# oleg-savchenko/jax_nbody_emulator_with_dj

Hardware: AMD Instinct MI355X
Metric: voxels/sec (disp+vel) on 512^3 box, ndiv=4 (higher is better)
Workload: dtype f32-equivalent: f16x3 split MFMA (3 f16 MFMAs per product, f32 accumulate)

## Files before the change

### include/nbe.h

```cpp
#ifndef NBE_H
#define NBE_H

#include <stddef.h>
#include <stdint.h>

#ifdef __cplusplus
extern "C" {
#endif

typedef struct nbe_ctx nbe_ctx;

typedef void (*nbe_progress_cb)(int done, int total, void* user);

typedef struct nbe_layer_desc {
    const char* block;
    const char* layer;
    int cout, cin, k;
    const float* weight;
    const float* bias;
    const float* style_weight;
    const float* style_bias;
    const float* dweight;
} nbe_layer_desc;

enum { NBE_F32 = 0, NBE_F16 = 1 };

const char* nbe_last_error(void);
int nbe_version(void);

int nbe_create(int device_id, nbe_ctx** out);
int nbe_destroy(nbe_ctx* ctx);
int nbe_set_stream(nbe_ctx* ctx, void* hip_stream);
int nbe_use_own_stream(nbe_ctx* ctx);
int nbe_synchronize(nbe_ctx* ctx);

int nbe_set_arch(nbe_ctx* ctx, int in_chan, int out_chan, int mid_chan, float eps, int compute_vel);

enum { NBE_PREC_F32 = 0, NBE_PREC_F16X3 = 1, NBE_PREC_F16 = 2 };
int nbe_set_precision(nbe_ctx* ctx, int precision);

enum { NBE_ERANGE = 2 };
int nbe_check_finite(nbe_ctx* ctx);
int nbe_set_input_range(nbe_ctx* ctx, float absmax);

enum { NBE_Q_GAUGE_ACTIVE = 0,
       NBE_Q_SLAB = 1,
       NBE_Q_PERIODIC_YX = 2,
       NBE_Q_PERIODIC_Z = 3,
       NBE_Q_RANGE_SHIFT = 4,
       NBE_Q_WORKSPACE_BYTES = 5,
       NBE_Q_HOST_PIPE = 6,
       NBE_Q_GRAPH_REPLAYS = 7,
       NBE_Q_PLAN_TILES = 8,
       NBE_Q_PLAN_SHORT_GB = 9 };
int nbe_query(nbe_ctx* ctx, int what, double* out);

int nbe_load_style_weights(nbe_ctx* ctx, const nbe_layer_desc* layers, int nlayers);
int nbe_load_premod_weights(nbe_ctx* ctx, const nbe_layer_desc* layers, int nlayers);

int nbe_set_cosmology(nbe_ctx* ctx, float Om, float Dz);

int nbe_forward(nbe_ctx* ctx, const void* x, int D, int H, int W, float Dz, float vel_fac,
                void* disp, void* vel);

int nbe_process_box(nbe_ctx* ctx, const void* box, const int64_t size[3], const int ndiv[3], const int pad[6],
                    float Dz, float vel_fac, void* disp, void* vel, int out_dtype,
                    nbe_progress_cb cb, void* user);

void* nbe_host_alloc(size_t bytes);
int nbe_host_free(void* p);
int nbe_host_trim(void);

int nbe_process_region(nbe_ctx* ctx, const void* box, const int64_t box_size[3], const int64_t origin[3],
                       const int64_t region[3], const int ndiv[3], const int* order, int norder,
                       float Dz, float vel_fac, void* disp, void* vel, int out_dtype,
                       const int64_t out_size[3], const int64_t out_origin[3]);

int64_t nbe_brick_halo_bytes(nbe_ctx* ctx, const int64_t brick_size[3], int which);
int nbe_brick_plan(nbe_ctx* ctx, const int64_t brick_size[3]);
int nbe_brick_encode(nbe_ctx* ctx, const void* haloed_brick, const int64_t brick_size[3], float Dz, float vel_fac,
                     void* send_lo, void* send_hi, void* skip_send_lo, void* skip_send_hi);
int nbe_brick_interior(nbe_ctx* ctx);
int nbe_brick_exchange(nbe_ctx* ctx, const void* recv_lo, const void* recv_hi, void* send2_lo, void* send2_hi);
int nbe_brick_finish(nbe_ctx* ctx, const void* recv2_lo, const void* recv2_hi, const void* skip_recv_lo, const void* skip_recv_hi,
                     void* skip_ready_event , float Dz, float vel_fac, void* disp, void* vel, int out_dtype);

int nbe_plan_tiles(const int64_t region[3], const int ndiv[3], int max_tile, int out_ndiv[3]);
int nbe_set_max_tile(nbe_ctx* ctx, int max_tile);
int nbe_plan_tiles_ctx(nbe_ctx* ctx, const int64_t region[3], const int ndiv[3], int periodic_box, int out_ndiv[3]);
int nbe_set_slab(nbe_ctx* ctx, int slab);
int nbe_set_periodic(nbe_ctx* ctx, int on);

double nbe_growth_factor(double z, double Om);
double nbe_vel_norm(double z, double Om);


int nbe_paint_mesh(const void* disp, int disp_dtype, const int64_t n[3], const double boxsize[3], const int64_t res[3],
                   int worder, int count_atomics, void* mesh, void* stats, void* stream);
int nbe_mesh_to_delta(const void* mesh, const int64_t res[3], int64_t nparticles, void* delta, void* stream);

#define NBE_PAINT_MAX_CHANNELS 4
#define NBE_FIELD_DENSITY 0
#define NBE_FIELD_MEAN 1
int nbe_quantity_range(const void* quantity, int dtype, int nchan, int64_t count, void* range, void* stream);
int nbe_paint_fields(const void* disp, int disp_dtype, const void* quantity, int quantity_dtype, int nchan,
                     const int exponents[], const void* shift, int shift_dtype, int shift_axis, double shift_scale,
                     const int64_t n[3], const double boxsize[3], const int64_t res[3], int worder, void* mesh,
                     void* qmesh, void* stats, void* stream);
int nbe_mesh_to_field(const void* mesh, const void* qmesh, int nchan, const int exponents[], const int64_t res[3],
                      int64_t nparticles, int mode, double fill, void* field, void* stats, void* stream);
int nbe_deconvolve_mas(void* field, const int64_t res[3], int worder, void* stream);
int nbe_power_spectrum(const void* a, const void* b, int64_t n, void* binmax, void* sums, void* stream);
#define NBE_PK_ANISO_MAX_N 2048
#define NBE_PK_MAX_MU 64
int nbe_power_multipoles(const void* a, const void* b, int64_t n, int los, void* binmax, void* sums, void* stream);
int nbe_power_wedges(const void* a, const void* b, int64_t n, int los, int nmu, int max_bins, void* binmax, void* sums,
                     void* stream);

#define NBE_MF_MAX_N 2048
#define NBE_MF_MAX_THRESHOLDS 1024
#define NBE_MOMENTS_WORDS 2050
int nbe_field_moments(const void* field, int64_t n, void* moments, void* stream);
int nbe_minkowski_counts(const void* field, int64_t n, const void* thresholds, int nthresholds, const void* moments,
                         void* counts, void* stream);

#define NBE_BK_MIN_N 4
#define NBE_BK_MAX_N 2048
#define NBE_BK_MAX_SHELLS 258
#define NBE_BK_MAX_EDGES 512
#define NBE_BK_PARTIALS 2048
int nbe_shell_filter(const void* spectrum, int64_t n, const void* shells, int nshells, void* filtered, void* binmax,
                     void* sums, void* stream);
int nbe_triple_sums(const void* f1, const void* f2, const void* f3, int nfields, int64_t n, void* partials, void* out,
                    void* stream);
int nbe_triangle_counts(const void* modes1, int64_t count1, const void* modes2, int64_t count2, const void* edges,
                        int nedges, void* hist, void* stream);

#define NBE_MOMENTS4_WORDS 6148
#define NBE_PDF_MAX_BINS 4096
#define NBE_ONEPOINT_MAX_VOXELS (1LL << 40)
int nbe_field_moments4(const void* field, int64_t count, void* moments, void* stream);
int nbe_field_histogram(const void* field, int64_t count, double lo, double hi, const void* edges, int nbins,
                        void* counts, void* stream);

#define NBE_LPT_MIN_N 2
#define NBE_LPT_MAX_N 2048
int nbe_zeldovich_spectrum(const void* spectrum, int64_t n, double boxsize, double scale, void* psi_spectrum,
                           void* stream);
int nbe_divergence_spectrum(const void* spectra, int64_t n, double boxsize, void* out, void* stream);
int nbe_spectrum_resize(const void* src, int64_t n_in, void* dst, int64_t n_out, int sphere, void* stream);
int nbe_spectrum_inject(const void* src, int64_t n_in, void* dst, int64_t n_out, const void* k_table,
                        const void* pk_table, int ntable, double tail_slope, double tail_intercept, double boxsize,
                        uint64_t seed, void* stream);
int nbe_gaussian_filter(void* spectrum, int64_t n, double sigma_over_L, void* stream);
int nbe_block_average(const void* src, int64_t n_in, void* dst, int64_t n_out, void* stream);
int nbe_trilinear_upsample(const void* src, int64_t n_in, void* dst, int64_t n_out, void* stream);


int nbe_test_layer(nbe_ctx* ctx, int kind, int crop, int flags, const float* x, const float* dx, int cin,
                   int D, int H, int W, const float* w, const float* dw, const float* bias, int cout,
                   const float* res, const float* dres, float* y, float* dy);
int nbe_test_layer_gauged(nbe_ctx* ctx, int flags, const float* x, const float* dx, int cin, int D, int H, int W,
                          const float* w, const float* beta, const float* bias, int cout, float* y, float* dy);
int nbe_test_layer_gauged_res(nbe_ctx* ctx, int flags, const float* x, const float* dx, int cin, int D, int H, int W,
                              const float* w, const float* beta, const float* bias, int cout, const float* res,
                              const float* dres, float* y, float* dy);
enum { NBE_PATH_SKIP_FUSED = 1,
       NBE_PATH_TWO_SOURCE = 2,
       NBE_PATH_WINO_0 = 4,
       NBE_PATH_WINO_1 = 8,
       NBE_PATH_NARROW = 16,
       NBE_PATH_UP8 = 32,
       NBE_PATH_SKIP_NODX = 64,
       NBE_PATH_TWO_SOURCE_SKIP = 128   };
int nbe_test_block(nbe_ctx* ctx, const char* block, int pad, int two_source, const float* x, const float* dx, int D, int H, int W,
                   const float* x2, const float* dx2, float* y, float* dy, float* h, float* dh, float* gauges, int* paths);
int nbe_test_modulate(nbe_ctx* ctx, const float* weight, const float* style_weight, const float* style_bias,
                      int cout, int cin, int k, float s0, float s1, float eps, int first_layer,
                      float* w_n, float* dw_tot);

int nbe_probe_begin(nbe_ctx* ctx, const int64_t origin[3], int nout);
int nbe_probe_slots(nbe_ctx* ctx);
int nbe_probe_layout(nbe_ctx* ctx, int slot, char* name, int name_cap, int dims[3], int64_t* word_offset);
int nbe_probe_read(nbe_ctx* ctx, void* words, int64_t nwords);
int nbe_probe_end(nbe_ctx* ctx);

int nbe_profile_enable(nbe_ctx* ctx, int on);
int nbe_profile_reset(nbe_ctx* ctx);
int nbe_profile_count(nbe_ctx* ctx);
int nbe_profile_entry(nbe_ctx* ctx, int i, char* name, int name_cap, double* ms, int64_t* launches, double* flops);
int64_t nbe_workspace_bytes(nbe_ctx* ctx);
int nbe_debug_phase_cycles(nbe_ctx* ctx, double* out16);

#ifdef __cplusplus
}
#endif
#endif
```

### jax_nbody_emulator_with_dj_amd/csrc/nbe_engine.cpp

```cpp
#include "nbe_engine_internal.h"

static thread_local std::string g_err;

int fail(const char* fmt, ...) {
    char buf[1024];
    va_list ap;
    va_start(ap, fmt);
    vsnprintf(buf, sizeof buf, fmt, ap);
    va_end(ap);
    g_err = buf;
    return 1;
}

namespace nbe { int api_fail(const char* msg) { g_err = msg; return 1; } }

bool is_device_ptr(const void* p) {
    hipPointerAttribute_t at;
    if (hipPointerGetAttributes(&at, p) != hipSuccess) { (void)hipGetLastError(); return false; }
    return at.type == hipMemoryTypeDevice;
}

int require_ready(nbe_ctx* c) {
    if (!c->have_weights) return fail("No parameters loaded. Call nbe_load_style_weights / nbe_load_premod_weights first.");
    if (c->style && !c->modulated) return fail("style weights are loaded but nbe_set_cosmology(Om, Dz) has not been called");
// ... 232 lines not shown
    }
    char *dd = (char*)disp, *vd = (char*)vel;
    if (!out_dev) {
        const int64_t need = out_bytes * 2;
        if (need > c->box_out_bytes) { (void)hipFree(c->box_out); HIPCHK(hipMalloc((void**)&c->box_out, need)); c->box_out_bytes = need; }
        dd = c->box_out; vd = c->box_out + out_bytes;
    }
    if (prepare_range(c, xd, (int64_t)c->in_chan * D * H * W, Dz)) return 1;
    if (c->probe.on) {
        const int oe[3] = {OD, OH, OW};
        c->probe.tile = true;
        for (int d = 0; d < 3; ++d) {
            c->probe.o[d] = c->probe.p[d];
            if (c->probe.p[d] < 0 || c->probe.p[d] + c->probe.nout > oe[d]) return fail("branch probe: the block does not fit the output of this input");
        }
    }
    if (run_subbox(c, xd, D, H, W, 0, 0, 0, D, H, W, Dz, vel_fac, dd, vd, NBE_F32, OD, OH, OW, 0, 0, 0)) return 1;
    HIPCHK(hipGetLastError());
    if (!out_dev) {
        HIPCHK(hipMemcpyAsync(disp, dd, out_bytes, hipMemcpyDeviceToHost, c->stream));
        if (c->vel) HIPCHK(hipMemcpyAsync(vel, vd, out_bytes, hipMemcpyDeviceToHost, c->stream));
    }
    if (!out_dev || !xin_dev) {
        HIPCHK(hipStreamSynchronize(c->stream));
        return check_range(c);
    }
    return 0;
}

int nbe_set_precision(nbe_ctx* c, int prec) {
    if (!c) return fail("null context");
    if (prec != PREC_F32 && prec != PREC_F16X3 && prec != PREC_F16) return fail("precision must be NBE_PREC_F32 (0), NBE_PREC_F16X3 (1) or NBE_PREC_F16 (2)");
    if (c->have_weights && prec != c->prec)
        return fail("nbe_set_precision must be called before the weights are loaded (they are packed per precision)");
    c->prec = prec;
    return 0;
}

int nbe_set_periodic(nbe_ctx* c, int on) {
    if (!c) return fail("null context");
    c->pyx_allowed = on != 0;
    return 0;
}

int nbe_set_slab(nbe_ctx* c, int slab) {
    if (!c) return fail("null context");
    if (slab > 0 && (slab & 1)) return fail("slab must be even");
    c->slab_forced = slab < 0 ? -1 : slab;
    return 0;
}

int nbe_set_max_tile(nbe_ctx* c, int max_tile) {
    if (!c) return fail("null context");
    if (max_tile < 0) return fail("max_tile must be >= 0 (0 = keep the caller's sub-box grid)");
    c->max_tile = max_tile;
    return 0;
}

int nbe_check_finite(nbe_ctx* c) {
    if (!c) return fail("null context");
    HIPCHK(hipSetDevice(c->device));
    return check_range(c);
}

int nbe_set_input_range(nbe_ctx* c, float absmax) {
    if (!c) return fail("null context");
    c->preset_absmax = (absmax >= 0.f || std::isnan(absmax)) ? absmax : -1.f;
    return 0;
}

int nbe_query(nbe_ctx* c, int what, double* out) {
    if (!c || !out) return fail("null argument");
    switch (what) {
    case NBE_Q_GAUGE_ACTIVE: *out = c->gauge_active ? 1 : 0; break;
    case NBE_Q_SLAB: *out = c->slab; break;
    case NBE_Q_PERIODIC_YX: *out = c->pyx ? 1 : 0; break;
    case NBE_Q_PERIODIC_Z: *out = c->pz ? 1 : 0; break;
    case NBE_Q_RANGE_SHIFT: *out = std::log2((double)c->act_scale); break;
    case NBE_Q_WORKSPACE_BYTES: *out = (double)c->ws_bytes; break;
    case NBE_Q_HOST_PIPE: *out = c->last_piped ? 1 : 0; break;
    case NBE_Q_GRAPH_REPLAYS: *out = (double)c->graph_replays; break;
    case NBE_Q_PLAN_TILES: *out = (double)c->plan_tiles; break;
    case NBE_Q_PLAN_SHORT_GB: *out = c->plan_short_gb; break;
    default: return fail("nbe_query: unknown item %d", what);
    }
    return 0;
}

int64_t nbe_workspace_bytes(nbe_ctx* c) { return c ? c->ws_bytes : 0; }

}
```

### jax_nbody_emulator_with_dj_amd/csrc/nbe_engine_box.cpp

```cpp
#include "nbe_engine_internal.h"

#include <sched.h>

static int host_threads() {
    static const int n = [] {
        if (const char* e = getenv("NBE_HOST_THREADS")) return std::max(1, atoi(e));
        unsigned hw = std::thread::hardware_concurrency();
        cpu_set_t set;
        if (sched_getaffinity(0, sizeof set, &set) == 0) hw = std::min<unsigned>(hw ? hw : 64, (unsigned)CPU_COUNT(&set));
        return (int)std::max(1u, std::min(hw ? hw : 4u, 16u));
    }();
    return n;
}
template <typename F>
static void parallel_for(int nt, F&& fn) {
    std::vector<std::thread> th;
    for (int i = 1; i < nt; ++i) th.emplace_back([&fn, i, nt] { fn(i, nt); });
    fn(0, nt);
    for (auto& t : th) t.join();
}
static void parallel_memcpy(void* dst, const void* src, size_t bytes) {
    const int nt = bytes < (size_t(8) << 20) ? 1 : host_threads();
    parallel_for(nt, [&](int i, int n) {
        const size_t per = ((bytes + n - 1) / n + 4095) & ~size_t(4095), b = std::min(bytes, per * i), e = std::min(bytes, b + per);
// ... 69 lines not shown
    }
    return 0;
}

int pipe_input(nbe_ctx* c, const Tensor& tin, int t0, int t1, int look, float scale) {
    auto& P = c->pipe;
    if (P.gz < t0) P.gz = t0;
    if (t1 > P.gz) {
        if (pipe_upload(c, P.gz, t1)) return 1;
        HIPCHK(hipEventRecord(c->ev_up, c->up_stream));
        HIPCHK(hipStreamWaitEvent(c->stream, c->ev_up, 0));
        const Tensor v = zview(tin, P.gz, t1 - P.gz);
        const int h = tin.pad ? 1 : 48;
        launch_gather(c->box_in, P.C, P.S0, P.S1, P.S2, P.o0 + P.gz, P.slabwise ? P.o1 : -h, P.slabwise ? P.o2 : -h, v.p, scale,
                      c->prec, c->stream);
        P.gz = t1;
    }
    return look > 0 ? pipe_upload(c, t1, t1 + look) : 0;
}

int pipe_output(nbe_ctx* c, int z, int n, int a1, int a2, int e1, int e2) {
    auto& P = c->pipe;
    if (e1 < 0) e1 = P.O1;
    if (e2 < 0) e2 = P.O2;
    HIPCHK(hipEventRecord(c->ev_down, c->stream));
    HIPCHK(hipStreamWaitEvent(c->down_stream, c->ev_down, 0));
    const int64_t plane = (int64_t)P.O1 * P.O2 * P.esz;
    const bool whole = a1 == 0 && a2 == 0 && e1 == P.O1 && e2 == P.O2;
    for (int f = 0; f < (P.hvel ? 2 : 1); ++f) {
        char* h = f ? P.hvel : P.hdisp;
        char* d = f ? P.dvel : P.ddisp;
        for (int ch = 0; ch < c->out_chan; ++ch) {
            if (whole) {
                const int64_t off = ((int64_t)ch * P.O0 + z) * plane;
                HIPCHK(hipMemcpyAsync(h + off, d + off, (size_t)n * plane, hipMemcpyDeviceToHost, c->down_stream));
            } else {
                hipMemcpy3DParms mp;
                memset(&mp, 0, sizeof mp);
                mp.srcPtr = make_hipPitchedPtr(d, (size_t)P.O2 * P.esz, (size_t)P.O2 * P.esz, (size_t)P.O1);
                mp.dstPtr = make_hipPitchedPtr(h, (size_t)P.O2 * P.esz, (size_t)P.O2 * P.esz, (size_t)P.O1);
                mp.srcPos = make_hipPos((size_t)a2 * P.esz, (size_t)a1, (size_t)ch * P.O0 + z);
                mp.dstPos = mp.srcPos;
                mp.extent = make_hipExtent((size_t)e2 * P.esz, (size_t)e1, (size_t)n);
                mp.kind = hipMemcpyDeviceToHost;
                HIPCHK(hipMemcpy3DAsync(&mp, c->down_stream));
            }
        }
    }
    return 0;
}

static int64_t workspace_need(nbe_ctx* c, int D, int H, int W, int slab, bool pyx, bool pz) {
    const int keep_slab = c->slab; const bool keep_pyx = c->pyx, keep_pz = c->pz;
    c->slab = slab; c->pyx = pyx; c->pz = pz;
    c->dry = true;
    c->arena.reset();
    Tensor tin = talloc(c, c->in_chan, D, H, W), y;
    tin.pad = c->pyx ? 1 : 0;
    HeadOut ho{};
    const int rc = c->slab > 0 ? network_stream(c, tin, ho, c->slab) : network(c, tin, &y);
    c->dry = false;
    c->slab = keep_slab; c->pyx = keep_pyx; c->pz = keep_pz;
    return rc ? -1 : c->arena.high;
}

int ensure_workspace(nbe_ctx* c, int D, int H, int W) {
    const int64_t need = workspace_need(c, D, H, W, c->slab, c->pyx, c->pz);
    if (need < 0) return 1;
    if (need > c->ws_bytes) {
        c->sst.valid = false;
        if (c->ws) { HIPCHK(hipStreamSynchronize(c->stream)); HIPCHK(hipFree(c->ws)); c->ws = nullptr; c->ws_bytes = 0; }
        HIPCHK(hipMalloc((void**)&c->ws, need));
        HIPCHK(hipMemsetAsync(c->ws, 0, need, c->stream));
        c->ws_bytes = need;
    }
    return 0;
}

int run_subbox(nbe_ctx* c, const float* box, int Db, int Hb, int Wb, int o0, int o1, int o2,
                      int D, int H, int W, float Dz, float vel_fac, void* disp, void* velo, int out_dtype,
                      int OD, int OH, int OW, int a0, int a1, int a2) {
    c->sst.valid = false;
    c->arena.reset();
    Tensor tin = talloc(c, c->in_chan, D, H, W), y;
    tin.pad = c->pyx ? 1 : 0;
    if (tin.pad) set_org(tin, 0, 48, 48);
    if (!c->pipe.active && !c->pipe.slabwise)
        launch_gather(box, c->in_chan, Db, Hb, Wb, o0, o1, o2, tin.p, Dz / 6.0f * c->act_scale, c->prec, c->stream);
    const HeadOut ho{disp, velo, out_dtype, OD, OH, OW, a0, a1, a2, Dz, vel_fac};
    if (c->slab > 0) return network_stream(c, tin, ho, c->slab);
    if (network(c, tin, &y)) return 1;
    run_head(c, y, tin, ho, 0);
    return 0;
}

void drop_graphs(nbe_ctx* c) {
    for (auto& kv : c->graphs) {
        if (kv.second.exec) (void)hipGraphExecDestroy(kv.second.exec);
        if (kv.second.graph) (void)hipGraphDestroy(kv.second.graph);
    }
    c->graphs.clear();
}

static int run_tile(nbe_ctx* c, const float* box, int Db, int Hb, int Wb, int o0, int o1, int o2,
                    int D, int H, int W, float Dz, float vel_fac, void* disp, void* velo, int out_dtype,
                    int OD, int OH, int OW, int a0, int a1, int a2) {
    const bool off = getenv("NBE_GRAPH") && atoi(getenv("NBE_GRAPH")) == 0;
    if (off || c->prof || c->prog_cb || c->pipe.active || c->pipe.slabwise || c->dry || c->probe.on)
        return run_subbox(c, box, Db, Hb, Wb, o0, o1, o2, D, H, W, Dz, vel_fac, disp, velo, out_dtype, OD, OH, OW, a0, a1, a2);
    nbe_ctx::GraphKey k;
    memset(&k, 0, sizeof k);
    k.box = box; k.disp = disp; k.velo = velo; k.ws = c->ws;
    const int geo[18] = {Db, Hb, Wb, o0, o1, o2, D, H, W, out_dtype, OD, OH, OW, a0, a1, a2, c->slab, c->prec};
    memcpy(k.geo, geo, sizeof geo);
    k.f[0] = Dz; k.f[1] = vel_fac; k.f[2] = c->act_scale;
    k.epoch = c->epoch; k.flags = (c->pyx ? 1 : 0) | (c->pz ? 2 : 0) | (c->gauge_active ? 4 : 0) | (c->fuse ? 8 : 0) | (wino_env_off() ? 16 : 0);
    nbe_ctx::GraphVal& g = c->graphs[k];
    g.used = ++c->graph_clock;
    if (!g.exec && g.seen++ == 0) {
        if (c->graphs.size() > 16) {
            auto lru = c->graphs.begin();
            for (auto it = c->graphs.begin(); it != c->graphs.end(); ++it) if (it->second.used < lru->second.used) lru = it;
            if (lru->second.exec) (void)hipGraphExecDestroy(lru->second.exec);
            if (lru->second.graph) (void)hipGraphDestroy(lru->second.graph);
            c->graphs.erase(lru);
        }
        return run_subbox(c, box, Db, Hb, Wb, o0, o1, o2, D, H, W, Dz, vel_fac, disp, velo, out_dtype, OD, OH, OW, a0, a1, a2);
    }
    if (!c->ev_g0) { HIPCHK(hipEventCreateWithFlags(&c->ev_g0, hipEventDisableTiming)); HIPCHK(hipEventCreateWithFlags(&c->ev_g1, hipEventDisableTiming)); }
    hipStream_t user = c->stream;
    if (!g.exec) {
        c->stream = c->own_stream;
        hipError_t e = hipStreamBeginCapture(c->own_stream, hipStreamCaptureModeThreadLocal);
        int rc = 0;
        if (e == hipSuccess) {
            rc = run_subbox(c, box, Db, Hb, Wb, o0, o1, o2, D, H, W, Dz, vel_fac, disp, velo, out_dtype, OD, OH, OW, a0, a1, a2);
            e = hipStreamEndCapture(c->own_stream, &g.graph);
            if (e == hipSuccess && !rc) e = hipGraphInstantiate(&g.exec, g.graph, nullptr, nullptr, 0);
        }
        c->stream = user;
        if (rc || e != hipSuccess || !g.exec) {
            (void)hipGetLastError();
            if (g.graph) { (void)hipGraphDestroy(g.graph); g.graph = nullptr; }
            g.exec = nullptr; g.seen = -1000000;
            return run_subbox(c, box, Db, Hb, Wb, o0, o1, o2, D, H, W, Dz, vel_fac, disp, velo, out_dtype, OD, OH, OW, a0, a1, a2);
        }
    }
    if (user != c->own_stream) { HIPCHK(hipEventRecord(c->ev_g0, user)); HIPCHK(hipStreamWaitEvent(c->own_stream, c->ev_g0, 0)); }
    HIPCHK(hipGraphLaunch(g.exec, c->own_stream));
    if (user != c->own_stream) { HIPCHK(hipEventRecord(c->ev_g1, c->own_stream)); HIPCHK(hipStreamWaitEvent(user, c->ev_g1, 0)); }
    ++c->graph_replays;
    return 0;
}

extern "C" {

int nbe_plan_tiles(const int64_t region[3], const int ndiv[3], int max_tile, int out_ndiv[3]) {
    if (!region || !ndiv || !out_ndiv) return fail("null argument");
    bool ok = max_tile > 0;
    for (int a = 0; a < 3 && ok; ++a) {
        if (ndiv[a] < 1 || region[a] < 1) return fail("sizes and ndiv must be positive");
        const int64_t crop = region[a] / ndiv[a];
        if (crop % 8 != 0 || crop * ndiv[a] != region[a]) ok = false;
    }
    for (int a = 0; a < 3; ++a) {
        out_ndiv[a] = ndiv[a];
        if (!ok) continue;
        const int64_t crop = region[a] / ndiv[a];
        int best = 1;
        for (int m = 1; m <= ndiv[a]; ++m)
            if (ndiv[a] % m == 0 && crop * m <= max_tile) best = m;
        out_ndiv[a] = ndiv[a] / best;
    }
    return 0;
}

}

int choose_slab(nbe_ctx* c, int D, int H, int W, int64_t budget, int64_t* need_out, bool pyx, bool pz) {
    const int forced = c->slab_forced;
    int result = -1;
    const int cand[4] = {0, 128, 64, 32};
    for (int i = 0; i < 4 && result < 0; ++i) {
        int S = cand[i];
        if (pyx && S == 0) { if (forced == 0) break; continue; }
        if (forced == 0 && S != 0) break;
        if (forced > 0) { if (i > (pyx ? 1 : 0)) break; S = forced & ~1; }
        if (!pyx && S > 0 && D - 8 <= S) continue;
        const int64_t need = workspace_need(c, D, H, W, S, pyx, pyx && pz);
        if (need >= 0 && need <= budget) { result = S; if (need_out) *need_out = need; }
    }
    return result;
}

static bool choose_schedule(nbe_ctx* c, int e0, int e1, int e2, bool spans_yx, bool whole_z, int64_t budget, bool fallback32) {
    const int D = e0 + 96;
    if (spans_yx && !check_dims_pyx(D, e1 + 2, e2 + 2)) {
        const int sl = choose_slab(c, D, e1 + 2, e2 + 2, budget, nullptr, true, whole_z);
        if (sl > 0) { c->slab = sl; c->pyx = true; c->pz = whole_z; return true; }
// ... 391 lines not shown
```

### jax_nbody_emulator_with_dj_amd/csrc/nbe_engine_internal.h

```cpp
#pragma once

#include "../../include/nbe.h"
#include "nbe_kernels.h"

#include <cmath>
#include <cstdarg>
#include <cstdio>
#include <cstdlib>
#include <cstring>
#include <algorithm>
#include <atomic>
#include <chrono>
#include <condition_variable>
#include <deque>
#include <functional>
#include <map>
#include <memory>
#include <mutex>
#include <string>
#include <thread>
#include <vector>

#pragma GCC visibility push(hidden)

using namespace nbe;

int fail(const char* fmt, ...);

#define HIPCHK(expr)                                                                        \
    do {                                                                                    \
        hipError_t e_ = (expr);                                                             \
        if (e_ != hipSuccess) return fail("%s failed: %s (%s:%d)", #expr, hipGetErrorString(e_), __FILE__, __LINE__); \
    } while (0)

static inline int roundup(int v, int m) { return (v + m - 1) / m * m; }

struct Arena {
    struct Blk { int64_t off, size; bool used; };
    std::vector<Blk> blks;
    int64_t high = 0;
    void reset() { blks.clear(); blks.push_back({0, INT64_MAX / 2, false}); high = 0; }
    int64_t alloc(int64_t bytes) {
        bytes = (bytes + 255) & ~int64_t(255);
        for (size_t i = 0; i < blks.size(); ++i) {
            if (!blks[i].used && blks[i].size >= bytes) {
                Blk rest{blks[i].off + bytes, blks[i].size - bytes, false};
                blks[i].size = bytes; blks[i].used = true;
                if (rest.size > 0) blks.insert(blks.begin() + i + 1, rest);
                if (blks[i].off + bytes > high) high = blks[i].off + bytes;
                return blks[i].off;
            }
        }
        return -1;
    }
    void release(int64_t off) {
        for (size_t i = 0; i < blks.size(); ++i) {
            if (blks[i].off == off && blks[i].used) {
                blks[i].used = false;
                if (i + 1 < blks.size() && !blks[i + 1].used) { blks[i].size += blks[i + 1].size; blks.erase(blks.begin() + i + 1); }
                if (i > 0 && !blks[i - 1].used) { blks[i - 1].size += blks[i].size; blks.erase(blks.begin() + i); }
                return;
            }
        }
    }
};

struct Layer {
    std::string block, layer;
    int cout = 0, cin = 0, k = 0, kind = 0;
    bool first = false;
    float *weight = nullptr, *sw = nullptr, *sb = nullptr;
    float *wn = nullptr, *dwn = nullptr;
    PackedW pw;
    PackedW pwn;
    float* bias0 = nullptr;
    float *alpha = nullptr, *beta = nullptr;
    const float* gout = nullptr;
    const float* a_in = nullptr;
    bool g6 = false;
    const Layer* fskip = nullptr;
    const float* b_sub = nullptr;
    float* bias_f = nullptr;
    float* dwn_f = nullptr;
};

struct Tensor { Planes p; int64_t off = -1; int pad = 0; int org[3] = {0, 0, 0}; };

struct ProfEntry { std::string name; double ms = 0; int64_t launches = 0; double flops = 0; };

struct Progress {
    struct Item { hipEvent_t ev; int done, total; };
    nbe_progress_cb cb; void* user; int device;
    std::thread th; std::mutex mu; std::condition_variable cv; std::deque<Item> q; bool stop = false;
    Progress(nbe_progress_cb cb_, void* user_, int dev) : cb(cb_), user(user_), device(dev) {
        th = std::thread([this] {
            (void)hipSetDevice(device);
            for (;;) {
                Item it;
                {
                    std::unique_lock<std::mutex> lk(mu);
                    cv.wait(lk, [this] { return stop || !q.empty(); });
                    if (q.empty()) return;
                    it = q.front(); q.pop_front();
                }
                (void)hipEventSynchronize(it.ev);
                (void)hipEventDestroy(it.ev);
                cb(it.done, it.total, user);
            }
        });
    }
    void post(hipStream_t s, int done, int total) {
        hipEvent_t ev;
        if (hipEventCreateWithFlags(&ev, hipEventDisableTiming) != hipSuccess) return;
        (void)hipEventRecord(ev, s);
        { std::lock_guard<std::mutex> lk(mu); q.push_back({ev, done, total}); }
        cv.notify_one();
    }
    ~Progress() {
        { std::lock_guard<std::mutex> lk(mu); stop = true; }
        cv.notify_one();
        if (th.joinable()) th.join();
    }
};

struct nbe_ctx {
    int device = 0;
    hipStream_t own_stream = nullptr, stream = nullptr;
    int in_chan = 3, out_chan = 3, mid = 64;
    float eps = 1e-8f;
    bool vel = true;
    bool have_weights = false, style = false, modulated = false;
    float mod_Om = NAN, mod_Dz = NAN;
    std::map<std::string, Layer> layers;
    Arena arena;
    char* ws = nullptr;
    int64_t ws_bytes = 0;
    bool dry = false;
    int slab = 0;
    int slab_forced = -1;
    bool pyx = false;
    bool pyx_allowed = true;
    bool pz = false;
    bool zx = false;
    int phase = 0;
    struct BrickIO { void *send_lo = nullptr, *send_hi = nullptr; const void *recv_lo = nullptr, *recv_hi = nullptr;
                     void *skip_send_lo = nullptr, *skip_send_hi = nullptr; const void *skip_recv_lo = nullptr, *skip_recv_hi = nullptr;
                     hipEvent_t skip_ready = nullptr; } bio;
    struct StreamState {
        bool valid = false;
        int stage = 0;
        Tensor skip0, td, tin, t, h, y1, cat1, t2;
        int D = 0, H = 0, W = 0, S = 0;
        std::vector<Arena::Blk> blks; int64_t high = 0;
        float Dz = 0.f, vel_fac = 0.f, act_scale = 1.f; const char* ws = nullptr;
    } sst;
    nbe_progress_cb prog_cb = nullptr; void* prog_user = nullptr; int prog_k = 0, prog_n = 1;
    Progress* prog = nullptr;
    int max_tile = 512;
    int prec = PREC_F32;
    bool gauge = false;
    bool gauge_active = false;
    bool fuse = false;
    bool novel_fuse = false;
    int64_t bp_size[3] = {0, 0, 0}; int bp_slab = 0; int64_t bp_need = 0;
    int plan_tiles = 0;
    double plan_short_gb = 0.0;
    int64_t plan_logged = 0;
    int* gauge_flag = nullptr;
    int* wino_flag = nullptr; bool wino_ok = false;
    float act_scale = 1.f;
    float bias_scale = 1.f;
    bool bias_dirty = true;
    float bias_max = 0.f;
    float preset_absmax = -1.f;
    bool input_finite = true;
    bool range_pending = false;
    unsigned* flags = nullptr;
    float* box_in = nullptr; int64_t box_in_bytes = 0;
    char* box_out = nullptr; int64_t box_out_bytes = 0;
    struct HostPipe {
        bool active = false, out_async = false;
        bool tiles = false;
        bool slabwise = false;
        int o1 = 0, o2 = 0;
        const float* hbox = nullptr;
        bool in_pinned = false;
        int C = 0, S0 = 0, S1 = 0, S2 = 0, o0 = 0;
        std::vector<char> up;
        int gz = 0;
        char *hdisp = nullptr, *hvel = nullptr;
        char *ddisp = nullptr, *dvel = nullptr;
        int esz = 4, O0 = 0, O1 = 0, O2 = 0;
        int nstage = 0;
    } pipe;
    bool last_piped = false;
    hipStream_t up_stream = nullptr, down_stream = nullptr;
    static constexpr int NSTAGE = 3;
    char* stage_buf[NSTAGE] = {nullptr, nullptr, nullptr}; int64_t stage_bytes = 0;
    hipEvent_t stage_free[NSTAGE] = {nullptr, nullptr, nullptr};
    hipEvent_t ev_up = nullptr, ev_down = nullptr;
    struct GraphKey {
        const void *box, *disp, *velo, *ws;
        int geo[18]; float f[3]; int epoch, flags;
        bool operator<(const GraphKey& o) const { return memcmp(this, &o, sizeof *this) < 0; }
    };
    struct GraphVal { hipGraphExec_t exec = nullptr; hipGraph_t graph = nullptr; int seen = 0; uint64_t used = 0; };
    std::map<GraphKey, GraphVal> graphs;
    uint64_t graph_clock = 0, graph_replays = 0;
    int epoch = 0;
    hipEvent_t ev_g0 = nullptr, ev_g1 = nullptr;
    struct Probe {
        bool on = false, tile = false;
        int p[3] = {0, 0, 0}, nout = 0;
        int o[3] = {0, 0, 0};
        struct Slot { std::string name; int C, n, nw, level; int64_t off; };
        std::vector<Slot> slots;
        unsigned* bits = nullptr; int64_t words = 0;
        unsigned* count = nullptr;
    } probe;
    int* paths = nullptr;
    bool prof = false;
    std::vector<ProfEntry> prof_entries;
    struct Pending { int entry; hipEvent_t a, b; };
    std::vector<Pending> pending;
    std::vector<hipEvent_t> ev_pool;
};

struct HeadOut { void* disp; void* velo; int out_dtype; int OD, OH, OW, a0, a1, a2; float Dz, vel_fac; };

static constexpr int PIPE_EDGE = 32;

static constexpr int BRICK_H1 = 6, BRICK_H2 = 10;
static constexpr int BRICK_H0 = 4;

bool is_device_ptr(const void* p);
int require_ready(nbe_ctx* c);
int prepare_range(nbe_ctx* c, const float* dev_src, int64_t n, float Dz, const float* host_src = nullptr);
int check_range(nbe_ctx* c);

int planes_for(int C, int prec);
Tensor talloc(nbe_ctx* c, int C, int D, int H, int W);
Tensor tallocp(nbe_ctx* c, int C, int D, int Hi, int Wi, int pad);
void fill_halo(nbe_ctx* c, const Tensor& t);
void tfree(nbe_ctx* c, Tensor& t);
Tensor zview(const Tensor& t, int z0, int nz);
void set_org(Tensor& t, int z, int y, int x);
bool wino_f16_layer(int prec, bool vel, int cin_pad);
bool wino_env_off();
bool up8_launch(const nbe_ctx* c, const Layer& L, bool has_dx);
int run_conv(nbe_ctx* c, const Layer& L, const ConvLaunch& cl_in, bool has_dx);
const Layer* find_layer(nbe_ctx* c, const char* block, const char* layer);
bool block_fused(const nbe_ctx* c, const Layer* L1, int nres);
bool two_source_width(const nbe_ctx* c);
Tensor alloc_hidden(nbe_ctx* c, int cmid, int nz, const Tensor& x, bool fused);
int resblock_part(nbe_ctx* c, const char* name, const Tensor& x, const Tensor& h, const Tensor& s,
                  int js, int ns, int jh, int nh, bool has_dx, bool final_act, const int* zr, const Tensor* x2 = nullptr);
int resblock(nbe_ctx* c, const char* name, const Tensor& x, bool has_dx, bool final_act, int cout, int cmid, Tensor* out,
             Tensor* hidden_out = nullptr);
int down_conv(nbe_ctx* c, const Layer& L, const Tensor& x, Tensor& o, bool probe);
int downblock(nbe_ctx* c, const char* name, const Tensor& x, Tensor* out);
int upblock(nbe_ctx* c, const char* name, const Tensor& x, const Tensor& cat, int xcrop = 0, int g0 = -1);
void crop_into(nbe_ctx* c, const Tensor& src, int crop, const Tensor& dst, int cz = -1);
int check_dims(int D, int H, int W);
int check_dims_pyx(int D, int H, int W);
void run_head(nbe_ctx* c, const Tensor& y, const Tensor& xin, const HeadOut& h, int zoff);
int network(nbe_ctx* c, const Tensor& tin, Tensor* yout);
int network_stream(nbe_ctx* c, const Tensor& tin, const HeadOut& ho, int S);

PackedW layer_geometry(int prec, int kind, int cout, int cin);
bool packs_narrow(int prec, bool vel, const Layer& L);
bool packs_wino(int prec, bool vel, const Layer& L);
bool packs_wino_skip(int prec, bool vel, bool style, const Layer& L);
bool packs_stem(int prec, const Layer& L);
int alloc_wino(PackedW& pw);
int alloc_stem(PackedW& pw);
int wino_flag_round_trip(nbe_ctx* c, const std::function<void()>& packs);
void release_layer(Layer& L);
void free_layers(nbe_ctx* c);
int pack_wino(nbe_ctx* c);

unsigned host_absmax_bits(const float* x, int64_t n);
int pipe_input(nbe_ctx* c, const Tensor& tin, int t0, int t1, int look, float scale);
int pipe_output(nbe_ctx* c, int z, int n, int a1 = 0, int a2 = 0, int e1 = -1, int e2 = -1);
int ensure_workspace(nbe_ctx* c, int D, int H, int W);
int run_subbox(nbe_ctx* c, const float* box, int Db, int Hb, int Wb, int o0, int o1, int o2,
               int D, int H, int W, float Dz, float vel_fac, void* disp, void* velo, int out_dtype,
               int OD, int OH, int OW, int a0, int a1, int a2);
void drop_graphs(nbe_ctx* c);
int64_t plan_budget(nbe_ctx* c, int64_t reserve);
int choose_slab(nbe_ctx* c, int D, int H, int W, int64_t budget, int64_t* need_out, bool pyx = false, bool pz = false);

void brick_send(nbe_ctx* c, const Tensor& t, int in, int n, void* lo, void* hi);
void brick_recv(nbe_ctx* c, const Tensor& like, const void* lo, const void* hi, int n, const Tensor& dst, int wrap);
int brick_interior(nbe_ctx* c, nbe_ctx::StreamState& st);
int brick_edges(nbe_ctx* c, nbe_ctx::StreamState& st);
int brick_level2(nbe_ctx* c, nbe_ctx::StreamState& st, Tensor* t_out);

void probe_act(nbe_ctx* c, const Layer& L, const Planes& out, int g0, const int org[3], int ez, int ey, int ex, bool periodic,
               const int* zr = nullptr);
int prof_entry(nbe_ctx* c, const std::string& name);
hipEvent_t get_event(nbe_ctx* c);
void prof_collect(nbe_ctx* c);

#pragma GCC visibility pop
```

### jax_nbody_emulator_with_dj_amd/csrc/nbe_engine_net.cpp

```cpp
#include "nbe_engine_internal.h"

int planes_for(int C, int prec) { return roundup(C, 16) / (prec == PREC_F16 ? 8 : 4); }

static Planes ws_planes(nbe_ctx* c, int G, int D, int H, int W, int64_t* off_out) {
    Planes p;
    p.G = G; p.D = D; p.H = H; p.W = W;
    p.pstride = (p.vox() + 63) & ~int64_t(63);
    const int64_t one = (int64_t)G * p.pstride * 16;
    const int64_t slack = ((int64_t)2 * H * W + 2 * W + 1024) * 16;
    const int64_t off = c->arena.alloc(one * (c->vel ? 2 : 1) + slack);
    *off_out = off;
    if (!c->dry) {
        p.x = (float*)(c->ws + off);
        p.dx = c->vel ? (float*)(c->ws + off + one) : nullptr;
    }
    return p;
}

Tensor talloc(nbe_ctx* c, int C, int D, int H, int W) {
    Tensor t;
    t.p = ws_planes(c, planes_for(C, c->prec), D, H, W, &t.off);
    const int gw = c->prec == PREC_F16 ? (C + 7) / 8 : c->prec == PREC_F16X3 ? 2 * ((C + 7) / 8) : (C + 3) / 4;
    if (!c->dry && t.off >= 0 && gw < t.p.G) {
        const size_t off = (size_t)gw * t.p.pstride * 4, bytes = (size_t)(t.p.G - gw) * t.p.pstride * 16;
        launch_zero(t.p.x + off, (int64_t)bytes, c->stream);
        if (t.p.dx) launch_zero(t.p.dx + off, (int64_t)bytes, c->stream);
    }
    return t;
}
Tensor tallocp(nbe_ctx* c, int C, int D, int Hi, int Wi, int pad) {
    Tensor t = talloc(c, C, D, Hi + 2 * pad, Wi + 2 * pad);
    t.pad = pad;
    return t;
}
static Planes inner(const Tensor& t) {
    Planes p = t.p;
    const int64_t sh = (int64_t)t.pad * (t.p.W + 1) * 4;
    if (p.x) p.x += sh;
    if (p.dx) p.dx += sh;
    return p;
}
void fill_halo(nbe_ctx* c, const Tensor& t) {
    if (t.pad > 0 && !c->dry) launch_fill_yx(t.p, t.pad, c->vel, c->stream);
}
void tfree(nbe_ctx* c, Tensor& t) { if (t.off >= 0) c->arena.release(t.off); t.off = -1; }
Tensor zview(const Tensor& t, int z0, int nz) {
    Tensor v = t;
    v.off = -1;
    const int64_t sh = (int64_t)z0 * t.p.H * t.p.W * 4;
    if (v.p.x) v.p.x += sh;
    if (v.p.dx) v.p.dx += sh;
    v.p.D = nz;
    v.org[0] += z0;
    return v;
}
static void org_conv(const Tensor& x, int nconv, int out[3]) {
    const int p = x.pad ? nconv : 0;
    out[0] = x.org[0]; out[1] = x.org[1] - p; out[2] = x.org[2] - p;
}
void set_org(Tensor& t, int z, int y, int x) { t.org[0] = z; t.org[1] = y; t.org[2] = x; }

static std::string conv_name(const PackedW& pw, bool vel, bool has_dx, bool g6 = false, bool up8 = false) {
    if (up8) return vel ? "up_h3<8 parities,vel,dx>" : "up_h3<8 parities,novel>";
    const char* m = pw.mode == MODE_FLAT3 ? "FLAT3" : pw.mode == MODE_FLAT1 ? "FLAT1" : "DOWN";
    if (pw.stem && !(vel && has_dx) && pw.mode == MODE_FLAT3) return vel ? "stem_h3<FLAT3,vel,nodx>" : "stem_h3<FLAT3,novel>";
    char b[96];
    if (g6 && prec_is_half(pw.prec)) snprintf(b, sizeof b, "%s<%s,vel,dx>", pw.prec == PREC_F16 ? "conv_h1g" : (pw.cout_t == 16 ? "conv_h3n" : "conv_h3g"), m);
    else if (g6) snprintf(b, sizeof b, "conv_mfma_g<%s,vel,dx,ni%d>", m, pw.ni);
    else if (prec_is_half(pw.prec))
        snprintf(b, sizeof b, "%s<%s,%s,%s>", pw.prec == PREC_F16 ? "conv_h1" : "conv_h3", m, vel ? "vel" : "novel", (vel && has_dx) ? "dx" : "nodx");
    else
        snprintf(b, sizeof b, "conv_mfma<%s,%s,%s,ni%d>", m, vel ? "vel" : "novel", (vel && has_dx) ? "dx" : "nodx", pw.ni);
    return b;
}

bool wino_f16_layer(int prec, bool vel, int cin_pad) { return prec == PREC_F16 && vel && cin_pad % 32 == 0 && cin_pad / 32 <= 8; }
bool wino_env_off() { return getenv("NBE_WINO") && atoi(getenv("NBE_WINO")) == 0; }
bool up8_launch(const nbe_ctx* c, const Layer& L, bool has_dx) { return prec_is_half(c->prec) && (!c->vel || has_dx) && L.pw.cin_pad <= 64; }

int run_conv(nbe_ctx* c, const Layer& L, const ConvLaunch& cl_in, bool has_dx) {
    if (c->dry) return 0;
    ConvLaunch cl = cl_in;
    const bool g6 = c->gauge_active && L.g6 && has_dx;
    const bool nov = !c->vel && c->prec == PREC_F16X3 && L.kind == 0 && L.pw.ww && c->wino_ok;
    if (c->gauge_active) { cl.gout = L.gout; cl.beta = g6 ? L.beta : nullptr; }
    if (cl.skw) {
        if (!((g6 || nov) && c->fuse && L.fskip)) return fail("internal error: fused skip requested for %s/%s", L.block.c_str(), L.layer.c_str());
        cl.bias = L.bias_f;
    }
    const PackedW& pw = (g6 && L.kind == 0 && L.pwn.w) ? L.pwn : L.pw;
    cl.wino = (g6 || nov) && c->wino_ok && &pw == &L.pw && pw.ww && (!cl.skw || cl.skw->ww) && (c->prec == PREC_F16 || !(cl.flags & F_RES)) &&
              (cl.Dv & 1) == 0 && cl.in_off == 0 && cl.osz == 1 && !wino_env_off();
    if (c->paths)
        *c->paths |= (cl.skw ? NBE_PATH_SKIP_FUSED : 0) | (cl.skw && (cl.flags & F_SKIP_NODX) ? NBE_PATH_SKIP_NODX : 0) |
                     (cl.csplit_ch ? NBE_PATH_TWO_SOURCE : 0) | (cl.skw && cl.sk_split_ch ? NBE_PATH_TWO_SOURCE_SKIP : 0) |
                     (cl.wino ? (L.layer == "conv_1" ? NBE_PATH_WINO_1 : NBE_PATH_WINO_0) : 0) |
                     (&pw == &L.pwn ? NBE_PATH_NARROW : 0) | (cl.set < 0 ? NBE_PATH_UP8 : 0);
    int pe = -1; hipEvent_t ea = nullptr, eb = nullptr;
    if (c->prof) {
        std::string pn = cl.wino ? std::string(c->prec == PREC_F16 ? "conv_h1w<FLAT3,vel,dx>" : c->vel ? "conv_h3w<FLAT3,vel,dx>" : "conv_h3w<FLAT3,novel>")
                                 : conv_name(pw, c->vel, has_dx, g6, cl.set < 0);
        static const bool per_layer = getenv("NBE_PROF_LAYERS") && atoi(getenv("NBE_PROF_LAYERS")) == 1;
        if (per_layer) pn += " " + L.block + "/" + L.layer;
        pe = prof_entry(c, pn);
        ea = get_event(c); eb = get_event(c);
        (void)hipEventRecord(ea, c->stream);
    }
    if (launch_conv(pw, cl, c->vel, has_dx, c->stream))
        return fail("internal error: no kernel for layer %s/%s (mode %d, gauged %d, input tangent %d, crop offset %ld, output stride %d)",
                    L.block.c_str(), L.layer.c_str(), L.pw.mode, (int)g6, (int)has_dx, (long)cl.in_off, cl.osz);
    if (c->prof) {
        (void)hipEventRecord(eb, c->stream);
        c->pending.push_back({pe, ea, eb});
        const double nout = (double)cl.Dv * cl.Hv * cl.Wv * (cl.set < 0 ? 8.0 : 1.0);
        const int taps = L.kind == 0 ? 27 : L.kind == 2 ? 8 : 1;
        const double gemms = c->vel ? ((has_dx && !g6) ? 3.0 : 2.0) : 1.0;
        c->prof_entries[pe].flops += 2.0 * nout * L.cout * L.cin * taps * gemms;
        if (cl.skw) c->prof_entries[pe].flops += 2.0 * nout * L.cout * L.fskip->cin * (!c->vel ? 1.0 : (cl.flags & F_SKIP_NODX) ? 2.0 : 3.0);
        c->prof_entries[pe].launches += 1;
        if (c->pending.size() > 4096) prof_collect(c);
    }
    return 0;
}

const Layer* find_layer(nbe_ctx* c, const char* block, const char* layer) {
    auto it = c->layers.find(std::string(block) + "/" + layer);
    return it == c->layers.end() ? nullptr : &it->second;
}


static bool wino_only_fuse(const nbe_ctx* c) { return !c->vel || c->prec == PREC_F16; }
bool block_fused(const nbe_ctx* c, const Layer* L1, int nres) {
    return c->fuse && L1->fskip != nullptr && (!wino_only_fuse(c) || (!wino_env_off() && (nres & 1) == 0));
}

bool two_source_width(const nbe_ctx* c) { return c->mid % (c->prec == PREC_F16 ? 32 : 16) == 0; }

Tensor alloc_hidden(nbe_ctx* c, int cmid, int nz, const Tensor& x, bool fused) {
    const int pad = x.pad, sy = pad ? 0 : 2;
    if (fused && !pad) return talloc(c, cmid, nz, x.p.H, x.p.W);
    return tallocp(c, cmid, nz, x.p.H - 2 * pad - sy, x.p.W - 2 * pad - sy, pad);
}

int resblock_part(nbe_ctx* c, const char* name, const Tensor& x, const Tensor& h, const Tensor& s,
                         int js, int ns, int jh, int nh, bool has_dx, bool final_act, const int* zr, const Tensor* x2) {
    const Layer *Ls = find_layer(c, name, "skip"), *L0 = find_layer(c, name, "conv_0"), *L1 = find_layer(c, name, "conv_1");
    if (!Ls || !L0 || !L1) return fail("missing layers of block %s", name);
    const int H = x.p.H, W = x.p.W, pad = x.pad;
    const bool fused = block_fused(c, L1, ns);
    if (fused && (h.p.H != H || h.p.W != W)) return fail("internal: hidden tensor of fused block %s lacks the input's pitch", name);
    if (x2 && (!fused || x2->p.H != H || x2->p.W != W || x2->pad != pad)) return fail("internal: two-source input of block %s", name);
    const Tensor sv = zview(s, js, ns), hv = zview(h, jh, nh);
    const Tensor xs = zview(x, js, ns + 4);
    const int64_t sk_off = (2L * H + (pad ? pad : 2)) * W + (pad ? pad : 2);
    if (!fused) {
        ConvLaunch cl; cl.in = xs.p; cl.in_off = sk_off;
        cl.Dv = ns; cl.Hv = s.p.H - 2 * pad; cl.Wv = s.p.W - 2 * pad; cl.out = inner(sv); cl.flags = 0;
        if (run_conv(c, *Ls, cl, has_dx)) return 1;
    }
    int og[3];
    {
        ConvLaunch cl; cl.in = zview(x, jh, nh + 2).p; cl.Dv = nh; cl.Hv = H - 2; cl.Wv = W - 2; cl.out = inner(hv); cl.flags = F_ACT;
        if (x2) { cl.in2 = zview(*x2, jh, nh + 2).p; cl.csplit_ch = c->mid; }
        if (run_conv(c, *L0, cl, has_dx)) return 1;
        org_conv(x, 1, og); og[0] += jh;
        const int zh[3] = {zr ? zr[0] : 0, zr ? zr[1] + 2 : 0, zr ? zr[2] : 0};
        probe_act(c, *L0, cl.out, 0, og, cl.Dv, cl.Hv, cl.Wv, pad != 0, zr ? zh : nullptr);
    }
    fill_halo(c, hv);
    {
        ConvLaunch cl; cl.in = zview(h, js, ns + 2).p; cl.Dv = ns; cl.Hv = s.p.H - 2 * pad; cl.Wv = s.p.W - 2 * pad; cl.out = inner(sv);
        if (fused) { cl.sk = xs.p; cl.sk_off = sk_off; cl.skw = L1->pwn.w ? &Ls->pwn : &Ls->pw; cl.flags = (final_act ? F_ACT : 0) | (has_dx ? 0 : F_SKIP_NODX);
                     if (x2) { cl.sk2 = zview(*x2, js, ns + 4).p; cl.sk_split_ch = c->mid; } }
        else { cl.res = inner(sv); cl.flags = F_RES | (final_act ? F_ACT : 0); }
        if (run_conv(c, *L1, cl, true)) return 1;
        org_conv(x, 2, og); og[0] += js;
        if (final_act) probe_act(c, *L1, cl.out, 0, og, cl.Dv, cl.Hv, cl.Wv, pad != 0, zr);
    }
    fill_halo(c, sv);
    return 0;
}

int resblock(nbe_ctx* c, const char* name, const Tensor& x, bool has_dx, bool final_act, int cout, int cmid, Tensor* out,
                    Tensor* hidden_out) {
    const Layer* L1 = find_layer(c, name, "conv_1");
    if (!L1) return fail("missing layers of block %s", name);
    const int D = x.p.D, pad = x.pad;
    const int sy = pad ? 0 : 2;
    Tensor s = tallocp(c, cout, D - 4, x.p.H - 2 * pad - 2 * sy, x.p.W - 2 * pad - 2 * sy, pad);
    Tensor h = alloc_hidden(c, cmid, D - 2, x, block_fused(c, L1, D - 4));
    if (s.off < 0 || h.off < 0) return fail("workspace exhausted in block %s", name);
    if (resblock_part(c, name, x, h, s, 0, D - 4, 0, D - 2, has_dx, final_act, nullptr)) return 1;
    tfree(c, h);
    if (hidden_out) *hidden_out = h;
    int og[3];
    org_conv(x, 2, og);
    set_org(s, og[0], og[1], og[2]);
    *out = s;
    return 0;
}

static void carry_planes(nbe_ctx* c, const Tensor& t, int src, int dst, int n) {
    if (c->dry || n <= 0) return;
    launch_crop(zview(t, src, n).p, 0, zview(t, dst, n).p, 0, c->vel, c->stream, 0);
}

int down_conv(nbe_ctx* c, const Layer& L, const Tensor& x, Tensor& o, bool probe) {
    ConvLaunch cl; cl.in = inner(x); cl.Dv = o.p.D; cl.Hv = o.p.H; cl.Wv = o.p.W; cl.out = o.p; cl.flags = F_ACT;
    if (run_conv(c, L, cl, true)) return 1;
    set_org(o, x.org[0] / 2, x.org[1] / 2, x.org[2] / 2);
    if (probe) probe_act(c, L, cl.out, 0, o.org, cl.Dv, cl.Hv, cl.Wv, x.pad != 0);
    return 0;
}

int downblock(nbe_ctx* c, const char* name, const Tensor& x, Tensor* out) {
    const Layer* L = find_layer(c, name, "conv_0");
    if (!L) return fail("missing layer %s/conv_0", name);
    Tensor o = talloc(c, c->mid, x.p.D / 2, x.p.H / 2, x.p.W / 2);
    if (o.off < 0) return fail("workspace exhausted in %s", name);
    if (down_conv(c, *L, x, o, true)) return 1;
    *out = o;
    return 0;
}

static int mid_planes(const nbe_ctx* c) { return c->mid / (c->prec == PREC_F16 ? 8 : 4); }

int upblock(nbe_ctx* c, const char* name, const Tensor& x, const Tensor& cat, int xcrop, int g0) {
    const Layer* L = find_layer(c, name, "conv_0");
    if (!L) return fail("missing layer %s/conv_0", name);
    xcrop += x.pad;
    const int Hx = x.p.H - 2 * xcrop, Wx = x.p.W - 2 * xcrop;
    if (cat.p.D != 2 * x.p.D || cat.p.H - 2 * cat.pad != 2 * Hx || cat.p.W - 2 * cat.pad != 2 * Wx)
        return fail("internal: concat geometry mismatch in %s", name);
    const bool up8 = up8_launch(c, *L, true);
    const int out_g0 = g0 >= 0 ? g0 : mid_planes(c);
    for (int p = 0; p < (up8 ? 1 : 8); ++p) {
        ConvLaunch cl; cl.in = x.p; cl.in_off = ((int64_t)xcrop * x.p.W + xcrop);
        cl.Dv = x.p.D; cl.Hv = Hx; cl.Wv = Wx; cl.out = inner(cat);
        cl.out_g0 = out_g0; cl.osz = 2; cl.oz = (p >> 2) & 1; cl.oy = (p >> 1) & 1; cl.ox = p & 1;
        cl.flags = F_ACT; cl.set = up8 ? -1 : p;
        if (run_conv(c, *L, cl, true)) return 1;
    }
    const int xc = xcrop - x.pad;
    const int og[3] = {2 * x.org[0], 2 * (x.org[1] + xc), 2 * (x.org[2] + xc)};
    probe_act(c, *L, inner(cat), out_g0, og, 2 * x.p.D, 2 * Hx, 2 * Wx, cat.pad != 0);
    return 0;
}

void crop_into(nbe_ctx* c, const Tensor& src, int crop, const Tensor& dst, int cz) {
    if (c->dry) return;
    Planes s = src.p; s.G = mid_planes(c);
    launch_crop(s, crop, dst.p, 0, c->vel, c->stream, cz);
}

int check_dims(int D, int H, int W) {
    const int v[3] = {D, H, W};
    for (int i = 0; i < 3; ++i)
        if (v[i] < 104 || v[i] % 8 != 0)
            return fail("input spatial size %d unsupported: each of (D,H,W) must be >= 104 and a multiple of 8 "
                        "(all-VALID U-Net with three 2x levels, receptive-field crop 48)", v[i]);
    return 0;
}

void run_head(nbe_ctx* c, const Tensor& y, const Tensor& xin, const HeadOut& h, int zoff) {
    if (c->dry) return;
    const float inv_s = 1.0f / c->act_scale;
    HeadScale hs;
    hs.k_disp = 6.0f * inv_s; hs.k_dy = h.vel_fac * 6.0f * inv_s; hs.k_x0 = h.vel_fac * 6.0f / h.Dz * inv_s;
    hs.bad = c->flags ? (int*)(c->flags + 1) : nullptr;
    launch_head(y.p, xin.p, 48, c->out_chan, hs, c->vel, h.disp, h.velo, h.out_dtype, h.OD, h.OH, h.OW,
                h.a0 + zoff, h.a1, h.a2, c->prec, c->stream, y.pad);
}

static int stream_encode(nbe_ctx* c, const Tensor& tin, const HeadOut& ho, int S, Tensor* skip0_out, Tensor* td_out) {
    const int m = c->mid, pad = tin.pad;
    const int D = tin.p.D, H = tin.p.H, W = tin.p.W;
    const int Hi = H - 2 * pad, Wi = W - 2 * pad;
    const int Y = D - 8;
    const bool zx = pad && c->zx;
    const bool pz = pad && (c->pz || zx);
    const int zlo = pz ? (zx ? 44 : 40) : 0, zhi = pz ? (zx ? Y - 44 : Y - 40) : Y;
    Tensor skip0 = pad ? tallocp(c, m, Y - 80, Hi, Wi, pad) : talloc(c, m, Y - 80, H - 88, W - 88);
    Tensor td = pad ? talloc(c, m, pz ? (D - 96) / 2 : Y / 2, Hi / 2, Wi / 2) : talloc(c, m, Y / 2, (H - 8) / 2, (W - 8) / 2);
    if (skip0.off < 0 || td.off < 0) return fail("workspace exhausted (level 0)");
    const Layer* Ld = find_layer(c, "down_l0", "conv_0");
    if (!Ld) return fail("missing layer down_l0/conv_0");
    const int sy = pad ? 0 : 2;
    const Layer* L00 = find_layer(c, "conv_l00", "conv_1");
    if (!L00) return fail("missing layer conv_l00/conv_1");
    Tensor h0 = alloc_hidden(c, m, S + 6, tin, block_fused(c, L00, S + 4)), a = tallocp(c, m, S + 4, Hi - 2 * sy, Wi - 2 * sy, pad);
    const Layer *L01 = find_layer(c, "conv_l01", "conv_1"), *Lr00 = find_layer(c, "conv_r00", "conv_1"), *Lr01 = find_layer(c, "conv_r01", "conv_1");
    if (!L01 || !Lr00 || !Lr01) return fail("missing conv_1 layers of the level-0 blocks");
    Tensor h1 = alloc_hidden(c, m, S + 2, a, block_fused(c, L01, S));
    Tensor y0r = pz ? Tensor() : tallocp(c, m, S, Hi - 4 * sy, Wi - 4 * sy, pad);
    if (h0.off < 0 || a.off < 0 || h1.off < 0 || (!pz && y0r.off < 0)) return fail("workspace exhausted (level-0 encoder slabs)");
    const int zr00[3] = {zlo, zhi + 4, pz ? D - 96 : 0}, zr01[3] = {zlo, zhi, pz ? D - 96 : 0};
    for (int z = zlo, n = 0; z < zhi; z += n) {
        n = std::min(((c->pipe.active || c->pipe.slabwise) && z == zlo) ? std::min(S, PIPE_EDGE) : S, zhi - z);
        const int n_next = std::min(S, zhi - (z + n));
        const bool first = z == zlo;
        Tensor y0 = pz ? zview(skip0, z - 40, n) : zview(y0r, 0, n);
        if ((c->pipe.active || c->pipe.slabwise) && !c->dry && pipe_input(c, tin, z, z + n + 8, n_next, ho.Dz / 6.0f * c->act_scale)) return 1;
        { int og[3]; org_conv(zview(tin, z, n + 8), 2, og); set_org(a, og[0], og[1], og[2]);
          org_conv(a, 2, og); set_org(y0, og[0], og[1], og[2]); }
        if (first) {
            if (resblock_part(c, "conv_l00", zview(tin, z, n + 8), h0, a, 0, n + 4, 0, n + 6, false, true, zr00)) return 1;
            if (resblock_part(c, "conv_l01", a, h1, y0, 0, n, 0, n + 2, true, true, zr01)) return 1;
        } else {
            if (resblock_part(c, "conv_l00", zview(tin, z, n + 8), h0, a, 4, n, 6, n, false, true, zr00)) return 1;
            if (resblock_part(c, "conv_l01", a, h1, y0, 0, n, 2, n, true, true, zr01)) return 1;
        }
        if (z + n < zhi) {
            carry_planes(c, h0, n, 0, 6);
            carry_planes(c, a, n, 0, 4);
            carry_planes(c, h1, n, 0, 2);
        }
        const int i0 = std::max(0, 40 - z), i1 = std::min(n, Y - 40 - z);
        if (!pz && i1 > i0) crop_into(c, y0, pad ? 0 : 40, zview(skip0, z + i0 - 40, i1 - i0), i0);
        {
            const int d0 = pz ? std::max(z, 44) : z, d1 = pz ? std::min(z + n, Y - 44) : z + n;
            if (d1 > d0) {
                const Tensor tv = zview(td, (d0 - (pz ? 44 : 0)) / 2, (d1 - d0) / 2);
                Tensor yv = zview(y0, d0 - z, d1 - d0);
                ConvLaunch cl; cl.in = inner(yv); cl.Dv = tv.p.D; cl.Hv = tv.p.H; cl.Wv = tv.p.W; cl.out = tv.p; cl.flags = F_ACT;
                if (run_conv(c, *Ld, cl, true)) return 1;
                const int og[3] = {yv.org[0] / 2, yv.org[1] / 2, yv.org[2] / 2};
                const int zd[3] = {22, 22 + (D - 96) / 2, pz ? (D - 96) / 2 : 0};
                probe_act(c, *Ld, cl.out, 0, og, cl.Dv, cl.Hv, cl.Wv, pad != 0, zd);
            }
        }
    }
    tfree(c, h0); tfree(c, a); tfree(c, h1);
    if (!pz) tfree(c, y0r);
    set_org(skip0, 0, pad ? 4 : 0, pad ? 4 : 0);
    set_org(td, pz ? 22 : 0, pad ? 22 : 0, pad ? 22 : 0);
    *skip0_out = skip0; *td_out = td;
    return 0;
}

static int stream_level1(nbe_ctx* c, int pad, bool pz, Tensor td, Tensor* cat1_out, Tensor* t_out) {
    const int m = c->mid;
    Tensor t = td;
    if (pad) {
        t = tallocp(c, m, td.p.D + (pz ? 44 : 0), td.p.H, td.p.W, 1);
        if (t.off < 0) return fail("workspace exhausted (level 1 input)");
        if (!c->dry) launch_wrap_pad(td.p, t.p, 1, c->vel, c->stream, pz ? 22 : 0);
        set_org(t, pz ? td.org[0] - 22 : td.org[0], td.org[1], td.org[2]);
        tfree(c, td);
    }

    Tensor y1, cat1;
    if (resblock(c, "conv_l1", t, true, true, m, m, &y1)) return 1;
    tfree(c, t);
    if (pad) {
        cat1 = tallocp(c, 2 * m, y1.p.D - 32, y1.p.H - 2, y1.p.W - 2, 1);
        if (cat1.off < 0) return fail("workspace exhausted (cat1)");
        crop_into(c, y1, 0, cat1, 16);
        set_org(cat1, y1.org[0], y1.org[1] - 16, y1.org[2] - 16);
        Tensor t2 = talloc(c, m, y1.p.D / 2, (y1.p.H - 2) / 2, (y1.p.W - 2) / 2);
        const Layer* Ld1 = find_layer(c, "down_l1", "conv_0");
        if (t2.off < 0 || !Ld1) return fail("workspace exhausted or missing layer (down_l1)");
        if (down_conv(c, *Ld1, y1, t2, true)) return 1;
        t = talloc(c, m, t2.p.D, t2.p.H + 20, t2.p.W + 20);
        if (t.off < 0) return fail("workspace exhausted (level 2 input)");
        if (!c->dry) launch_wrap_pad(t2.p, t.p, 10, c->vel, c->stream, 0);
        set_org(t, t2.org[0], t2.org[1] - 10, t2.org[2] - 10);
        tfree(c, t2);
    } else {
        cat1 = talloc(c, 2 * m, y1.p.D - 32, y1.p.H - 32, y1.p.W - 32);
        if (cat1.off < 0) return fail("workspace exhausted (cat1)");
        crop_into(c, y1, 16, cat1);
        if (downblock(c, "down_l1", y1, &t)) return 1;
    }
    tfree(c, y1);
    *cat1_out = cat1; *t_out = t;
    return 0;
}

static int lower_levels(nbe_ctx* c, Tensor t, Tensor cat1, Tensor* r_out) {
    const int m = c->mid;
    Tensor y2, cat2, r;
    if (resblock(c, "conv_l2", t, true, true, m, m, &y2)) return 1;
    tfree(c, t);
    cat2 = talloc(c, 2 * m, y2.p.D - 8, y2.p.H - 8, y2.p.W - 8);
    if (cat2.off < 0) return fail("workspace exhausted (cat2)");
    crop_into(c, y2, 4, cat2);
    if (downblock(c, "down_l2", y2, &t)) return 1;
    tfree(c, y2);

    if (resblock(c, "conv_c", t, true, true, m, m, &r)) return 1;
    tfree(c, t);

    if (upblock(c, "up_r2", r, cat2)) return 1;
    tfree(c, r);
    if (resblock(c, "conv_r2", cat2, true, true, m, 2 * m, &r)) return 1;
    tfree(c, cat2);

    if (upblock(c, "up_r1", r, cat1, cat1.pad ? 2 : 0)) return 1;
    fill_halo(c, cat1);
    tfree(c, r);
    if (resblock(c, "conv_r1", cat1, true, true, m, 2 * m, r_out)) return 1;
    tfree(c, cat1);
    return 0;
}

int network(nbe_ctx* c, const Tensor& tin, Tensor* yout) {
    const int m = c->mid;
    Tensor a, y0, t, cat0, cat1, r;
    if (resblock(c, "conv_l00", tin, false, true, m, m, &a)) return 1;
    if (resblock(c, "conv_l01", a, true, true, m, m, &y0)) return 1;
    tfree(c, a);
    cat0 = talloc(c, 2 * m, y0.p.D - 80, y0.p.H - 80, y0.p.W - 80);
    if (cat0.off < 0) return fail("workspace exhausted (cat0)");
    crop_into(c, y0, 40, cat0);
    if (downblock(c, "down_l0", y0, &t)) return 1;
    tfree(c, y0);

    if (stream_level1(c, 0, false, t, &cat1, &t)) return 1;
    if (lower_levels(c, t, cat1, &r)) return 1;

    if (upblock(c, "up_r0", r, cat0)) return 1;
    tfree(c, r);
    if (resblock(c, "conv_r00", cat0, true, true, m, 2 * m, &r)) return 1;
    tfree(c, cat0);

    if (resblock(c, "conv_r01", r, true, false, c->out_chan, m, yout)) return 1;
    tfree(c, r);
    return 0;
}

static int stream_tail(nbe_ctx* c, const Tensor& tin, const HeadOut& ho, int S, Tensor skip0, Tensor cat1, Tensor t) {
    const int m = c->mid, pad = tin.pad;
    const int sy = pad ? 0 : 2;
    const Layer *Lr00 = find_layer(c, "conv_r00", "conv_1"), *Lr01 = find_layer(c, "conv_r01", "conv_1");
    if (!Lr00 || !Lr01) return fail("missing conv_1 layers of the level-0 blocks");
    Tensor r;
    if (lower_levels(c, t, cat1, &r)) return 1;
    if (2 * r.p.D != skip0.p.D || 2 * (r.p.H - 2 * r.pad) != skip0.p.H - 2 * pad || 2 * (r.p.W - 2 * r.pad) != skip0.p.W - 2 * pad)
        return fail("internal: level-0 concat geometry mismatch");

    if (pad && c->zx && !c->dry && c->bio.skip_recv_lo) {
        if (c->bio.skip_ready) HIPCHK(hipStreamWaitEvent(c->stream, c->bio.skip_ready, 0));
        brick_recv(c, skip0, c->bio.skip_recv_lo, c->bio.skip_recv_hi, BRICK_H0, skip0, 0);
    }
    const int Yo = skip0.p.D - 8;
    const int Hs = skip0.p.H - 2 * pad, Ws = skip0.p.W - 2 * pad;
    const bool two = block_fused(c, Lr00, S + 4) && two_source_width(c);
    Tensor cat = tallocp(c, two ? m : 2 * m, S + 8, Hs, Ws, pad), hq = alloc_hidden(c, 2 * m, S + 6, cat, block_fused(c, Lr00, S + 4));
    Tensor q = tallocp(c, m, S + 4, Hs - 2 * sy, Ws - 2 * sy, pad), hy = alloc_hidden(c, m, S + 2, q, block_fused(c, Lr01, S));
    Tensor y = tallocp(c, c->out_chan, S, Hs - 4 * sy, Ws - 4 * sy, pad);
    if (cat.off < 0 || hq.off < 0 || q.off < 0 || hy.off < 0 || y.off < 0) return fail("workspace exhausted (level-0 decoder slabs)");
    for (int z = 0, n = 0; z < Yo; z += n) {
        n = std::min(S, Yo - z);
        if (c->pipe.active && c->pipe.out_async && Yo - z > PIPE_EDGE && Yo - z - n < PIPE_EDGE)
            n = Yo - z - PIPE_EDGE;
        const bool first = z == 0;
        const int c0 = first ? 0 : 8, cn = first ? n + 8 : n;
        set_org(cat, skip0.org[0] + z, skip0.org[1], skip0.org[2]);
        { int og[3]; org_conv(cat, 2, og); set_org(q, og[0], og[1], og[2]); }
        if (!two && !c->dry) launch_crop(zview(skip0, z + c0, cn).p, 0, zview(cat, c0, cn).p, 0, c->vel, c->stream, 0);
        if (upblock(c, "up_r0", zview(r, (z + c0) / 2, cn / 2), zview(cat, c0, cn), 0, two ? 0 : -1)) return 1;
        fill_halo(c, zview(cat, c0, cn));
        const Tensor sk = two ? zview(skip0, z, std::min(S + 8, skip0.p.D - z)) : cat;
        const Tensor* up2 = two ? &cat : nullptr;
        if (first) {
            if (resblock_part(c, "conv_r00", sk, hq, q, 0, n + 4, 0, n + 6, true, true, nullptr, up2)) return 1;
            if (resblock_part(c, "conv_r01", q, hy, y, 0, n, 0, n + 2, true, false, nullptr)) return 1;
        } else {
            if (resblock_part(c, "conv_r00", sk, hq, q, 4, n, 6, n, true, true, nullptr, up2)) return 1;
            if (resblock_part(c, "conv_r01", q, hy, y, 0, n, 2, n, true, false, nullptr)) return 1;
        }
        if (z + n < Yo) {
            carry_planes(c, cat, n, 0, 8);
            carry_planes(c, hq, n, 0, 6);
            carry_planes(c, q, n, 0, 4);
            carry_planes(c, hy, n, 0, 2);
        }
        run_head(c, zview(y, 0, n), zview(tin, z, n + 96), ho, z);
        if (c->pipe.active && c->pipe.out_async && !c->dry && pipe_output(c, z, n)) return 1;
        if (c->prog && !c->dry && z + n < Yo)
            c->prog->post(c->pipe.active && c->pipe.out_async ? c->down_stream : c->stream,
                          c->prog_k * 1000 + (int)(1000L * (z + n) / Yo), c->prog_n * 1000);
    }
    tfree(c, cat); tfree(c, hq); tfree(c, q); tfree(c, hy); tfree(c, y);
    tfree(c, r); tfree(c, skip0);
    return 0;
}

static void stash_arena(nbe_ctx* c) { c->sst.blks = c->arena.blks; c->sst.high = c->arena.high; }

int network_stream(nbe_ctx* c, const Tensor& tin, const HeadOut& ho, int S) {
    auto& st = c->sst;
    const int pad = tin.pad;
    const bool zx = pad && c->zx;
    if (c->phase >= 2) {
        if (!st.valid || st.stage != c->phase - 1) return fail("brick calls out of order (encode, interior, exchange, finish) or the context was used in between");
        c->arena.blks = st.blks; c->arena.high = st.high;
    }
    if (c->phase <= 1) {
        if (stream_encode(c, tin, ho, S, &st.skip0, &st.td)) return 1;
        st.tin = tin; st.S = S;
        if (c->phase == 1) {
            brick_send(c, st.td, 0, BRICK_H1, c->bio.send_lo, c->bio.send_hi);
            brick_send(c, st.skip0, BRICK_H0, BRICK_H0, c->bio.skip_send_lo, c->bio.skip_send_hi);
            st.valid = true; st.stage = 1; stash_arena(c);
            return 0;
        }
    }
    if (!zx) {
        Tensor cat1, t;
        if (stream_level1(c, pad, pad && c->pz, st.td, &cat1, &t)) return 1;
        return stream_tail(c, tin, ho, S, st.skip0, cat1, t);
    }
    if (c->phase == 0 || c->phase == 2) {
        if (brick_interior(c, st)) return 1;
        if (c->phase == 2) { st.stage = 2; stash_arena(c); return 0; }
    }
    if (c->phase == 0 || c->phase == 3) {
        if (brick_edges(c, st)) return 1;
        if (c->phase == 3) { st.stage = 3; stash_arena(c); return 0; }
    }
    Tensor t;
    if (brick_level2(c, st, &t)) return 1;
    st.valid = false;
    return stream_tail(c, st.tin, ho, st.S, st.skip0, st.cat1, t);
}

int check_dims_pyx(int D, int H, int W) {
    if (D < 104 || D % 8 != 0) return fail("input depth %d unsupported: must be >= 104 and a multiple of 8", D);
    const int v[2] = {H - 2, W - 2};
    for (int i = 0; i < 2; ++i)
        if (v[i] < 48 || v[i] % 8 != 0) return fail("periodic extent %d unsupported: must be >= 48 and a multiple of 8", v[i]);
    return 0;
}
// ... 1 lines not shown
```

### jax_nbody_emulator_with_dj_amd/csrc/nbe_kernels.h

```cpp
#pragma once
#include <hip/hip_runtime.h>
#include <stdint.h>

namespace nbe {

struct Planes {
    float* x = nullptr;
    float* dx = nullptr;
    int64_t pstride = 0;
    int G = 0;
    int D = 0, H = 0, W = 0;
    int64_t vox() const { return (int64_t)D * H * W; }
};

enum Precision { PREC_F32 = 0, PREC_F16X3 = 1, PREC_F16 = 2 };
inline constexpr bool prec_is_half(int prec) { return prec == PREC_F16X3 || prec == PREC_F16; }
inline constexpr int prec_parts(int prec) { return prec == PREC_F16X3 ? 2 : 1; }
constexpr float H3_SCALE = 2048.0f, H3_INV = 1.0f / 2048.0f;
constexpr int H3_RANGE_UP = 6;

constexpr int NBE_MAX_GROUPS = 64;

enum ConvMode { MODE_FLAT3 = 0, MODE_FLAT1 = 1, MODE_DOWN = 2 };
enum ConvFlags { F_ACT = 1, F_RES = 2, F_SKIP_NODX = 4 };

constexpr int TILE_VOX = 256;
inline constexpr int mode_taps(int mode) { return mode == MODE_FLAT3 ? 3 : 1; }
inline constexpr int mode_nseg(int mode) { return mode == MODE_FLAT3 ? 9 : (mode == MODE_DOWN ? 8 : 1); }
inline constexpr int mode_ck(int mode) { return mode == MODE_FLAT3 ? 8 : 16; }
inline constexpr int prec_ck(int prec, int mode) { return prec_is_half(prec) ? 16 : mode_ck(mode); }

struct PackedW {
    float* w = nullptr;
    float* dw = nullptr;
    float* bias = nullptr;
    int prec = PREC_F32;
    int mode = 0, ni = 2;
    int cout_t = 64;
    int cin = 0, cout = 0;
    int cin_pad = 0;
    int ctiles = 0;
    int64_t floats = 0;
    int nsets = 1;
    float* ww = nullptr;
    float* stem = nullptr;
};

struct ConvLaunch {
    Planes in;
    int64_t in_off = 0;
    int Dv = 0, Hv = 0, Wv = 0;
    Planes out;
    int out_g0 = 0;
    int osz = 1, oz = 0, oy = 0, ox = 0;
    Planes res;
    int flags = 0;
    int set = 0;
    const float* gout = nullptr;
    const float* beta = nullptr;
    const float* bias = nullptr;
    Planes in2;
    int csplit_ch = 0;
    Planes sk, sk2;
    int sk_split_ch = 0;
    int64_t sk_off = 0;
    const PackedW* skw = nullptr;
    bool wino = false;
};

int launch_conv(const PackedW& pw, const ConvLaunch& L, bool vel, bool has_dx, hipStream_t s);

void launch_modulate(const float* weight, const float* style_weight, const float* style_bias,
                     int cout, int cin, int k3, float s0, float s1, float eps, int first_layer,
                     float* w_n, float* dw_tot , hipStream_t s,
                     const float* a_in = nullptr, float* beta_out = nullptr, const float* b_sub = nullptr);
void launch_style_alpha(const float* style_weight, const float* style_bias, int cin, float s0, float s1,
                        float* alpha, int* flag, hipStream_t s);
void launch_pack(const float* w_oidhw, int cout, int cin, int kind, const PackedW& pw, float* dst, hipStream_t s);

void launch_pack_h3w(const float* w_oidhw, int cout, int cin, int cin_pad, int ctiles, float* dst, int* flag, hipStream_t s,
                     int prec = PREC_F16X3);
void launch_pack_h3w_skip(const float* w_oidhw, int cout, int cin, const PackedW& pw, float* dst, int* flag, hipStream_t s);

void launch_gather(const float* box, int C, int Db, int Hb, int Wb, int a0, int a1, int a2,
                   const Planes& dst, float scale, int prec, hipStream_t s);
void launch_to_planes(const float* src, int C, const Planes& dst, bool tangent, float scale, int prec, hipStream_t s);
void launch_from_planes(const Planes& src, bool tangent, int C, float* dst, int prec, hipStream_t s);
void launch_crop(const Planes& src, int c, const Planes& dst, int g0, bool vel, hipStream_t s, int cz = -1);
struct HeadScale { float k_disp = 6.f, k_dy = 0.f, k_x0 = 0.f; int* bad = nullptr; };
void launch_head(const Planes& y, const Planes& xin, int c0, int C, const HeadScale& hs, bool vel,
                 void* disp, void* velo, int out_dtype, int Db, int Hb, int Wb, int a0, int a1, int a2,
                 int prec, hipStream_t s, int pad = 0);
void launch_absmax(const float* src, int64_t n, unsigned* out_bits, hipStream_t s);
void launch_zero(void* dst, int64_t bytes, hipStream_t s);
void launch_scale(const float* src, float* dst, int n, float f, hipStream_t s, const float* src2 = nullptr);

void launch_fill_yx(const Planes& t, int pad, bool vel, hipStream_t s);
void launch_wrap_pad(const Planes& src, const Planes& dst, int pad, bool vel, hipStream_t s, int padz = 0);

void launch_tag_word(unsigned* dst, unsigned v, const unsigned* expect_at, unsigned* flag, unsigned bit, hipStream_t s);

struct ProbeLaunch {
    const float* x; int64_t pstride; int H, W, g0, prec, C;
    int ext[3], org[3], per[3];
    int zlo, zhi, zper;
    int o[3], n, nw;
    unsigned* bits; unsigned* count;
};
void launch_probe_signs(const ProbeLaunch& a, hipStream_t s);

void h3q_read_stamps(double* out16, hipStream_t s);

}
```

### jax_nbody_emulator_with_dj_amd/csrc/nbe_kernels.hip

```cpp

#include "nbe_kernels_internal.h"
#include <algorithm>
#include <cstdint>
#include <cstdio>
#include <cstdlib>

namespace nbe {

#define LDS_AS NBE_LDS_AS
#define GLB_AS NBE_GLB_AS

extern __shared__ __attribute__((aligned(16))) f32x4 lds_dyn[];

template <int MODE, bool VEL, bool HAS_DX, int NI, bool G6 = false>
__global__ __launch_bounds__(256, 2) void conv_mfma_kernel(ConvKArgs a) {
    constexpr int CK = mode_ck(MODE), GL = CK / 4, TAPS = mode_taps(MODE);
    constexpr int COUT_T = 32 * NI;
    constexpr int XV = (MODE == MODE_FLAT3) ? 320 : 256;
    constexpr int WP = TAPS * GL * COUT_T;
    constexpr int XP = GL * XV;
    constexpr bool DX = VEL && HAS_DX;
    constexpr bool DWT = VEL && !G6;
    static_assert(!G6 || (DX && MODE == MODE_FLAT3), "gauged form: 3x3x3 layers with an input tangent");
    constexpr int OFF_W = 0, OFF_DW = WP, OFF_X = OFF_DW + (DWT ? WP : 0), OFF_DXX = OFF_X + XP;
// ... 40 lines not shown
            const int n = wave + 4 * t;
            if (n < NIW) {
                dma16(a.w + wbase + (long)(n * 64 + lane) * 4, buf + OFF_W + n * 64);
            } else if (DWT && n < NW_TOT) {
                const int m = n - NIW;
                dma16(a.dw + wbase + (long)(m * 64 + lane) * 4, buf + OFF_DW + m * 64);
            } else if (n < NINSTR) {
                const bool tang = DX && n >= NW_TOT + NIX;
                const int m = n - NW_TOT - (tang ? NIX : 0);
                const int gl = (m * 64) / XV;
                const int vl = (m * 64) % XV + lane;
                long v;
                if (MODE == MODE_DOWN) v = (long)inbase[vl] + segoff;
                else {
                    v = q0 + a.in_off + segoff + vl;
                    if (v > a.P - 1) v = a.P - 1;
                }
                const long off = ((long)(chunk * GL + gl) * a.in_pstride + v) * 4;
                dma16((tang ? a.dx : a.x) + off, buf + (tang ? OFF_DXX : OFF_X) + m * 64);
            }
        }
    };

    f32x16 accy[NI][2];
    f32x16 accd[NI][2];
#pragma unroll
    for (int it = 0; it < NI; ++it)
#pragma unroll
        for (int jt = 0; jt < 2; ++jt)
#pragma unroll
            for (int e = 0; e < 16; ++e) { accy[it][jt][e] = 0.f; accd[it][jt][e] = 0.f; }

    auto compute = [&](int b) {
        const f32x4* buf = lds + b * BUF;
#pragma unroll
        for (int tap = 0; tap < TAPS; ++tap) {
#pragma unroll
            for (int kg = 0; kg < CK / 8; ++kg) {
                f32x4 wv[NI], dwv[NI], xv[2], dxv[2];
#pragma unroll
                for (int it = 0; it < NI; ++it) {
                    const int o = (tap * GL + 2 * kg + lh) * COUT_T + 32 * it + li;
                    wv[it] = buf[OFF_W + o];
                    if (DWT) dwv[it] = buf[OFF_DW + o];
                }
#pragma unroll
                for (int jt = 0; jt < 2; ++jt) {
                    const int o = (2 * kg + lh) * XV + wave * 64 + 32 * jt + li + (MODE == MODE_FLAT3 ? tap : 0);
                    xv[jt] = buf[OFF_X + o];
                    if (DX) dxv[jt] = buf[OFF_DXX + o];
                }
#pragma unroll
                for (int r = 0; r < 4; ++r) {
#pragma unroll
                    for (int it = 0; it < NI; ++it) {
#pragma unroll
                        for (int jt = 0; jt < 2; ++jt) {
                            accy[it][jt] = __builtin_amdgcn_mfma_f32_32x32x2f32(wv[it][r], xv[jt][r], accy[it][jt], 0, 0, 0);
                            if (DWT) accd[it][jt] = __builtin_amdgcn_mfma_f32_32x32x2f32(dwv[it][r], xv[jt][r], accd[it][jt], 0, 0, 0);
                            if (DX) accd[it][jt] = __builtin_amdgcn_mfma_f32_32x32x2f32(wv[it][r], dxv[jt][r], accd[it][jt], 0, 0, 0);
                        }
                    }
                }
            }
        }
    };

    issue(0, 0);
    __syncthreads();
    for (int s = 0; s < nstage; ++s) {
        if (s + 1 < nstage) issue(s + 1, (s + 1) & 1);
        compute(s & 1);
        __syncthreads();
    }

    const bool act = a.flags & F_ACT, res = a.flags & F_RES;
#pragma unroll
    for (int jt = 0; jt < 2; ++jt) {
        const long q = q0 + wave * 64 + 32 * jt + li;
        bool valid = q < a.Q;
        long o;
        if (MODE == MODE_DOWN) {
            o = q;
        } else {
            const int z = (int)(q / HW), rem = (int)(q - (long)z * HW);
            const int yy = rem / a.W, xx = rem - yy * a.W;
            valid = valid && xx < a.Wv && yy < a.Hv && z < a.Dv;
            o = ((long)(z * a.osz + a.oz) * a.Ho + (yy * a.osz + a.oy)) * a.Wo + (xx * a.osz + a.ox);
        }
        if (!valid) continue;
#pragma unroll
        for (int it = 0; it < NI; ++it) {
#pragma unroll
            for (int k = 0; k < 4; ++k) {
                const int cgl = 8 * it + 2 * k + lh;
                const int cg = ct * (COUT_T / 4) + cgl;
                if (cg >= a.cout_groups) continue;
                const f32x4 bv = *(const f32x4*)(a.bias + cg * 4);
                f32x4 v, dv;
#pragma unroll
                for (int e = 0; e < 4; ++e) { v[e] = accy[it][jt][4 * k + e] + bv[e]; dv[e] = accd[it][jt][4 * k + e]; }
                if (G6) {
                    const f32x4 be = *(const f32x4*)(a.beta + cg * 4);
#pragma unroll
                    for (int e = 0; e < 4; ++e) dv[e] += be[e] * accy[it][jt][4 * k + e];
                }
                if (res) {
                    const long ro = ((long)cg * a.res_pstride + o) * 4;
                    const f32x4 rv = *(const f32x4*)(a.r + ro);
                    v += rv;
                    if (VEL) { const f32x4 drv = *(const f32x4*)(a.dr + ro); dv += drv; }
                }
                if (act) {
#pragma unroll
                    for (int e = 0; e < 4; ++e) {
                        if (VEL) dv[e] = v[e] > 0.f ? dv[e] : 0.01f * dv[e];
                        v[e] = v[e] >= 0.f ? v[e] : 0.01f * v[e];
                    }
                }
                if (VEL && a.gout) {
                    const f32x4 gv = *(const f32x4*)(a.gout + cg * 4);
#pragma unroll
                    for (int e = 0; e < 4; ++e) dv[e] += gv[e] * v[e];
                }
                const long oo = ((long)(a.out_g0 + cg) * a.out_pstride + o) * 4;
                *(f32x4*)(a.y + oo) = v;
                if (VEL) *(f32x4*)(a.dy + oo) = dv;
            }
        }
    }
}

template <int MODE, bool VEL, bool HAS_DX, int NI, bool G6 = false>
static void launch_conv_t(const ConvKArgs& ka, int ctiles, hipStream_t s) {
    constexpr int CK = mode_ck(MODE), GL = CK / 4, TAPS = mode_taps(MODE);
    constexpr int XV = (MODE == MODE_FLAT3) ? 320 : 256;
    constexpr int WP = TAPS * GL * 32 * NI, XP = GL * XV;
    constexpr int BUF = WP * ((VEL && !G6) ? 2 : 1) + XP * ((VEL && HAS_DX) ? 2 : 1);
    constexpr size_t smem = (size_t)2 * BUF * 16 + 256 * sizeof(int);
    auto kern = conv_mfma_kernel<MODE, VEL, HAS_DX, NI, G6>;
    ensure_lds_limit((const void*)kern, smem);
    dim3 grid(ka.ntiles, ctiles, 1), block(256, 1, 1);
    hipLaunchKernelGGL(kern, grid, block, smem, s, ka);
}

int launch_conv(const PackedW& pw, const ConvLaunch& L, bool vel, bool has_dx, hipStream_t s) {
    ConvKArgs ka;
    ka.x = L.in.x; ka.dx = L.in.dx; ka.in_pstride = L.in.pstride;
    ka.D = L.in.D; ka.H = L.in.H; ka.W = L.in.W; ka.P = L.in.vox(); ka.in_off = L.in_off;
    ka.Dv = L.Dv; ka.Hv = L.Hv; ka.Wv = L.Wv;
    if (pw.mode == MODE_DOWN) ka.Q = (long)L.Dv * L.Hv * L.Wv;
    else ka.Q = ((long)(L.Dv - 1) * L.in.H + (L.Hv - 1)) * L.in.W + L.Wv;
    ka.y = L.out.x; ka.dy = L.out.dx; ka.out_pstride = L.out.pstride; ka.out_g0 = L.out_g0;
    ka.Ho = L.out.H; ka.Wo = L.out.W; ka.osz = L.osz; ka.oz = L.oz; ka.oy = L.oy; ka.ox = L.ox;
    ka.r = L.res.x; ka.dr = L.res.dx; ka.res_pstride = L.res.pstride;
    ka.bias = L.bias ? L.bias : pw.bias;
    const int set = L.set < 0 ? 0 : L.set;
    ka.up8 = L.set < 0 ? 1 : 0; ka.set_stride = (long)pw.floats * 4;
    ka.stem_w = pw.stem;
    ka.ww = L.wino ? pw.ww : nullptr;
    ka.wws = (L.wino && L.skw) ? L.skw->ww : nullptr; ka.wws_set_floats = L.skw ? L.skw->floats : 0;
    ka.w = pw.w + (size_t)set * pw.floats;
    ka.dw = pw.dw ? pw.dw + (size_t)set * pw.floats : nullptr;
    ka.nchunk = pw.cin_pad / prec_ck(pw.prec, pw.mode);
    ka.cout_groups = prec_is_half(pw.prec) ? (pw.cout + 7) / 8 : (pw.cout + 3) / 4;
    ka.flags = L.flags;
    ka.gout = L.gout; ka.beta = L.beta;
    ka.x2 = L.in2.x; ka.dx2 = L.in2.dx; ka.in2_pstride = L.in2.pstride;
    if (L.csplit_ch % 16 != 0 || L.sk_split_ch % 16 != 0) return 1;
    ka.csplit = L.csplit_ch > 0 ? L.csplit_ch / 16 : (1 << 30);
    ka.xs = ka.dxs = ka.xs2 = ka.dxs2 = nullptr; ka.s_pstride = ka.s2_pstride = 0; ka.s_csplit = 1 << 30;
    ka.ws = ka.dws = nullptr; ka.nskip = 0; ka.dws_delta = 0;
    if (L.skw) {
        if (L.sk.H != L.in.H || L.sk.W != L.in.W) return 1;
        const int64_t o = (L.sk_off - L.sk.W - 1) * 4;
        ka.xs = L.sk.x + o; ka.dxs = (L.flags & F_SKIP_NODX) ? ka.xs : L.sk.dx + o; ka.s_pstride = L.sk.pstride;
        if (L.sk_split_ch > 0) { ka.xs2 = L.sk2.x + o; ka.dxs2 = L.sk2.dx + o; ka.s2_pstride = L.sk2.pstride; ka.s_csplit = L.sk_split_ch / 16; }
        ka.ws = L.skw->w; ka.dws = L.skw->dw; ka.nskip = L.skw->cin_pad / 16;
    }
    ka.ntiles = (int)((ka.Q + TILE_VOX - 1) / TILE_VOX);
    if (prec_is_half(pw.prec)) return launch_conv_h3(pw, ka, vel, has_dx, s);
    const int ct = pw.ctiles;
    if (ka.beta) {
        if (!(pw.mode == MODE_FLAT3 && vel && has_dx)) return 1;
        if (pw.ni == 2) launch_conv_t<MODE_FLAT3, true, true, 2, true>(ka, ct, s);
        else launch_conv_t<MODE_FLAT3, true, true, 1, true>(ka, ct, s);
        return 0;
    }
#define NBE_DISPATCH(MODE)                                                                   \
    if (vel) {                                                                               \
        if (has_dx) { if (pw.ni == 2) launch_conv_t<MODE, true, true, 2>(ka, ct, s);        \
                      else launch_conv_t<MODE, true, true, 1>(ka, ct, s); }                 \
        else        { if (pw.ni == 2) launch_conv_t<MODE, true, false, 2>(ka, ct, s);       \
                      else launch_conv_t<MODE, true, false, 1>(ka, ct, s); }                \
    } else {                                                                                 \
        if (pw.ni == 2) launch_conv_t<MODE, false, false, 2>(ka, ct, s);                     \
        else launch_conv_t<MODE, false, false, 1>(ka, ct, s);                                \
    }
    if (pw.mode == MODE_FLAT3) { NBE_DISPATCH(MODE_FLAT3) }
    else if (pw.mode == MODE_FLAT1) { NBE_DISPATCH(MODE_FLAT1) }
    else { NBE_DISPATCH(MODE_DOWN) }
#undef NBE_DISPATCH
    return 0;
}


__device__ __forceinline__ double block_sum(double v, double* scratch) {
#pragma unroll
    for (int off = 32; off > 0; off >>= 1) v += __shfl_down(v, off, 64);
    const int lane = threadIdx.x & 63, wave = threadIdx.x >> 6;
    __syncthreads();
    if (lane == 0) scratch[wave] = v;
    __syncthreads();
    double t = 0.0;
    for (int i = 0; i < (int)(blockDim.x >> 6); ++i) t += scratch[i];
    return t;
}

__global__ __launch_bounds__(256) void modulate_kernel(const float* __restrict__ weight,
                                                       const float* __restrict__ sw,
                                                       const float* __restrict__ sb,
                                                       int cin, int k3, float s0, float s1, float eps,
                                                       int first_layer, float* __restrict__ w_n,
                                                       float* __restrict__ dw_tot, const float* __restrict__ a_in,
                                                       float* __restrict__ beta_out, const float* __restrict__ b_sub) {
    __shared__ double scratch[4];
    const int co = blockIdx.x;
    const int n = cin * k3;
    const float* wr = weight + (size_t)co * n;
    double sww = 0.0, swd = 0.0;
    for (int e = threadIdx.x; e < n; e += blockDim.x) {
        const int ci = e / k3;
        const float smod = sw[2 * ci] * s0 + sw[2 * ci + 1] * s1 + sb[ci];
        const float w = wr[e] * smod;
        const float dws = wr[e] * sw[2 * ci + 1];
        sww += (double)w * w;
        swd += (double)w * dws;
    }
    sww = block_sum(sww, scratch);
    swd = block_sum(swd, scratch);
    const float norm = sqrtf((float)sww + eps);
    const float dnorm = -(float)swd / (norm * norm * norm);
    const float inv_dz = 1.0f / (s1 + 1.0f);
    if (beta_out && threadIdx.x == 0) beta_out[co] = dnorm * norm;
    for (int e = threadIdx.x; e < n; e += blockDim.x) {
        const int ci = e / k3;
        const float smod = sw[2 * ci] * s0 + sw[2 * ci + 1] * s1 + sb[ci];
        const float w = wr[e] * smod;
        const float dws = wr[e] * sw[2 * ci + 1];
        const float wn = w / norm;
        w_n[(size_t)co * n + e] = wn;
        if (dw_tot) {
            float d = dws / norm + w * dnorm;
            if (first_layer) d += wn * inv_dz;
            if (a_in) d -= wn * a_in[ci];
            if (b_sub) d -= wn * b_sub[co];
            dw_tot[(size_t)co * n + e] = d;
        }
    }
}

void launch_modulate(const float* weight, const float* style_weight, const float* style_bias,
                     int cout, int cin, int k3, float s0, float s1, float eps, int first_layer,
                     float* w_n, float* dw_tot, hipStream_t s, const float* a_in, float* beta_out, const float* b_sub) {
// ... 347 lines not shown
```

### jax_nbody_emulator_with_dj_amd/csrc/nbe_kernels_h3.hip

```cpp

#include "nbe_kernels_internal.h"
#include <cstdlib>
#include <cstdio>
#include <algorithm>

#ifndef NBE_DBG
#define NBE_DBG 0
#endif

namespace nbe {

extern __shared__ __attribute__((aligned(16))) f32x4 lds_h3[];

__device__ __forceinline__ void split4(const f32x4 v, half4& hi, half4& lo) {
#pragma unroll
    for (int e = 0; e < 4; ++e) {
        hi[e] = (_Float16)v[e];
        lo[e] = (_Float16)__builtin_fmaf((float)hi[e], -H3_SCALE, v[e] * H3_SCALE);
    }
}
__device__ __forceinline__ f32x4 join4(const half4 hi, const half4 lo) {
    f32x4 v;
#pragma unroll
    for (int e = 0; e < 4; ++e) v[e] = (float)hi[e] + (float)lo[e] * H3_INV;
// ... 182 lines not shown

    f32x16 ym[2], yc[2], dm[2], dc[2];
#pragma unroll
    for (int jt = 0; jt < 2; ++jt)
#pragma unroll
        for (int e = 0; e < 16; ++e) { ym[jt][e] = 0.f; yc[jt][e] = 0.f; dm[jt][e] = 0.f; dc[jt][e] = 0.f; }

    struct Ops { half8 wh, wl, dwh, dwl, xh[2], xl[2], dxh[2], dxl[2]; };
    auto load_ops = [&](const half8* wb, const half8* xb, Ops& o) {
        const int wo = (PARTS * lh) * 64 + 32 * it + li;
        o.wh = wb[wo];
        if (SPLIT) o.wl = wb[wo + 64];
        if (VEL) { o.dwh = wb[OFF_DW + wo]; if (SPLIT) o.dwl = wb[OFF_DW + wo + 64]; }
#pragma unroll
        for (int jt = 0; jt < 2; ++jt) {
            const int xo = (PARTS * lh) * XV + jq * 64 + 32 * jt + li;
            o.xh[jt] = xb[xo];
            if (SPLIT) o.xl[jt] = xb[xo + XV];
            if (DX) { o.dxh[jt] = xb[OFF_DXX + xo]; if (SPLIT) o.dxl[jt] = xb[OFF_DXX + xo + XV]; }
        }
    };
    auto mfma1 = [&](const Ops& o, int i) {
        const int jt = i / 9, k = i % 9;
        if (k == 0) ym[jt] = __builtin_amdgcn_mfma_f32_32x32x16_f16(o.wh, o.xh[jt], ym[jt], 0, 0, 0);
        if (SPLIT && k == 1) yc[jt] = __builtin_amdgcn_mfma_f32_32x32x16_f16(o.wh, o.xl[jt], yc[jt], 0, 0, 0);
        if (SPLIT && k == 2) yc[jt] = __builtin_amdgcn_mfma_f32_32x32x16_f16(o.wl, o.xh[jt], yc[jt], 0, 0, 0);
        if (VEL) {
            if (k == 3) dm[jt] = __builtin_amdgcn_mfma_f32_32x32x16_f16(o.dwh, o.xh[jt], dm[jt], 0, 0, 0);
            if (SPLIT && k == 4) dc[jt] = __builtin_amdgcn_mfma_f32_32x32x16_f16(o.dwh, o.xl[jt], dc[jt], 0, 0, 0);
            if (SPLIT && k == 5) dc[jt] = __builtin_amdgcn_mfma_f32_32x32x16_f16(o.dwl, o.xh[jt], dc[jt], 0, 0, 0);
        }
        if (DX) {
            if (k == 6) dm[jt] = __builtin_amdgcn_mfma_f32_32x32x16_f16(o.wh, o.dxh[jt], dm[jt], 0, 0, 0);
            if (SPLIT && k == 7) dc[jt] = __builtin_amdgcn_mfma_f32_32x32x16_f16(o.wh, o.dxl[jt], dc[jt], 0, 0, 0);
            if (SPLIT && k == 8) dc[jt] = __builtin_amdgcn_mfma_f32_32x32x16_f16(o.wl, o.dxh[jt], dc[jt], 0, 0, 0);
        }
    };

    {
        const long x0 = seg_offset(0);
#pragma unroll
        for (int t = 0; t < NXS; ++t) dma_x(t, x0, 0);
#pragma unroll
        for (int t = 0; t < NWS; ++t) dma_w(t, 0);
        wait_all();
        barrier();
    }

    int ring = 0;
    for (int s = 0; s < nstage; ++s) {
        const bool pw = s + 1 < nstage, px = s + 1 < nstage;
        const long xoff2 = px ? seg_offset(s + 1) : 0;
        const int ring2 = ring ^ 1;
        const half8* wb = (const half8*)(lds + (s & 1) * WB);
        const half8* xb = (const half8*)(lds + XRING + ring * XB);
        Ops o0, o1;
        load_ops(wb, xb, o0);
        __builtin_amdgcn_sched_barrier(0);
#pragma unroll
        for (int i = 0; i < 18; ++i) {
            mfma1(o0, i);
            if (i & 1) {
                const int t = i >> 1;
                if (t < NWS) { if (pw) dma_w(t, s + 1); }
                else if (t - NWS < NXS) { if (px) dma_x(t - NWS, xoff2, ring2); }
                __builtin_amdgcn_sched_barrier(0);
            }
        }
        __builtin_amdgcn_sched_barrier(0);
        __builtin_amdgcn_sched_barrier(0);
        wait_all();
        barrier();
        ring = ring == 1 ? 0 : ring + 1;
    }

    long o[2];
    bool ok[2];
#pragma unroll
    for (int jt = 0; jt < 2; ++jt) {
        const long q = q0 + jq * 64 + 32 * jt + li;
        ok[jt] = q < a.Q;
        if (MODE == MODE_DOWN) {
            o[jt] = q;
        } else {
            const int z = (int)(q / HW), rem = (int)(q - (long)z * HW);
            const int yy = rem / a.W, xx = rem - yy * a.W;
            ok[jt] = ok[jt] && xx < a.Wv && yy < a.Hv && z < a.Dv;
            o[jt] = ((long)(z * a.osz + a.oz) * a.Ho + (yy * a.osz + a.oy)) * a.Wo + (xx * a.osz + a.ox);
        }
        if (!ok[jt]) o[jt] = 0;
    }
    h3_store2<VEL, SPLIT>(a, ct, it, lh, o, ok, ym, yc, dm, dc);
}

constexpr int UP_XV = 256;
constexpr int UP_MAXCH = 4;
template <bool SPLIT> struct UpGeom {
    static constexpr int UN = SPLIT ? 4 : 2;
    static constexpr int XC = 2 * UN * UP_XV;
    static constexpr int WS = 2 * 2 * UN * 64;
    static constexpr int WBASE = UP_MAXCH * XC;
    static constexpr int LDS_UNITS = WBASE + 2 * WS;
};

template <bool SPLIT, bool VEL = true>
__global__ __launch_bounds__(512, 2) void up_h3_kernel(ConvKArgs a) {
    constexpr int UN = UpGeom<SPLIT>::UN, UP_XC = UpGeom<SPLIT>::XC, UP_WS = UpGeom<SPLIT>::WS, UP_WBASE = UpGeom<SPLIT>::WBASE;
    constexpr int PS = SPLIT ? 2 : 1;
    f32x4* lds = lds_h3;
    const half8* L8 = (const half8*)lds_h3;
    const int tid = threadIdx.x;
    const int lane = tid & 63;
    const int wave = __builtin_amdgcn_readfirstlane(tid >> 6);
    const int li = lane & 31, lh = lane >> 5;
    const int it = wave & 1, jq = wave >> 1;
    const int tile = xcd_tile(blockIdx.x, a.ntiles);
    const int ct = blockIdx.y;
    const long q0 = (long)tile * UP_XV;
    const int nchunk = a.nchunk, nstage = 2 * 4 * nchunk;
    const long HW = (long)a.H * a.W;

    for (int c = 0; c < nchunk; ++c) {
#pragma unroll
        for (int k = 0; k < (VEL ? UN : UN / 2); ++k) {
            const int n = wave + 8 * k;
            const int t = n / (4 * UN), u = (n >> 2) % UN, qd = n & 3;
            const long v = q0 + a.in_off + qd * 64 + lane;
            const char* src = (const char*)(t ? a.dx : a.x) + (((long)c * UN + u) * a.in_pstride + v) * 16;
            dma16((const float*)src, lds + c * UP_XC + (t * UN + u) * UP_XV + qd * 64);
        }
    }
    auto dma_w = [&](int st) {
        const int c = st % nchunk, pp = (st / nchunk) & 3;
#pragma unroll
        for (int k = 0; k < UN / 2; ++k) {
            const int n = wave + 8 * k;
            const int par = n / (2 * UN), d = (n / UN) & 1, m = n % UN;
            if (!VEL && d) continue;
            const char* src = (const char*)(d ? a.dw : a.w) + (long)(2 * pp + par) * a.set_stride +
                              (((long)ct * nchunk + c) * (UN * 64) + m * 64 + lane) * 16;
            dma16((const float*)src, lds + UP_WBASE + (st & 1) * UP_WS + n * 64);
        }
    };
    dma_w(0);
    asm volatile("s_waitcnt vmcnt(0)" ::: "memory");
    __syncthreads();

    f32x16 ym[2], yc[2], dm[2], dc[2];
    auto zero_acc = [&]() {
#pragma unroll
        for (int jt = 0; jt < 2; ++jt)
#pragma unroll
            for (int e = 0; e < 16; ++e) { ym[jt][e] = 0.f; yc[jt][e] = 0.f; dm[jt][e] = 0.f; dc[jt][e] = 0.f; }
    };
    zero_acc();

    for (int st = 0; st < nstage; ++st) {
        const int c = st % nchunk, pp = (st / nchunk) & 3, half = st / (4 * nchunk);
        if (st + 1 < nstage) dma_w(st + 1);
        const half8* wb = L8 + UP_WBASE + (st & 1) * UP_WS;
        const half8* xb = L8 + c * UP_XC;
        const int xo = (PS * lh) * UP_XV + half * 128 + jq * 32 + li;
        const half8 xh = xb[xo];
        half8 dxh = xh, xl = xh, dxl = xh;
        if (VEL) dxh = xb[UN * UP_XV + xo];
        if (SPLIT) { xl = xb[xo + UP_XV]; if (VEL) dxl = xb[UN * UP_XV + xo + UP_XV]; }
// ... 1340 lines not shown
            if (!uok) unit = a.cout_groups - 1;
            const f32x4 bv = *(const f32x4*)(Lvec + unit * 8 + 4 * kh);
            const f32x4 gv = *(const f32x4*)(Lvec + 64 + unit * 8 + 4 * kh);
#pragma unroll
            for (int nt = 0; nt < 2; ++nt) {
                const int t = 2 * mt + nt;
                f32x4 v, dv;
#pragma unroll
                for (int e = 0; e < 4; ++e) {
                    v[e] = ym[t][e] + (SPLIT ? yc[t][e] * H3_INV : 0.f) + bv[e];
                    dv[e] = dm[t][e] + (SPLIT ? dc[t][e] * H3_INV : 0.f);
                }
                if (act) {
#pragma unroll
                    for (int e = 0; e < 4; ++e) {
                        dv[e] = v[e] > 0.f ? dv[e] : 0.01f * dv[e];
                        v[e] = v[e] >= 0.f ? v[e] : 0.01f * v[e];
                    }
                }
                if (gauge) {
#pragma unroll
                    for (int e = 0; e < 4; ++e) dv[e] += gv[e] * v[e];
                }
                if (!SPLIT) {
                    if (uok && ook[nt]) {
                        const long ob = ((long)(a.out_g0 + unit) * a.out_pstride + o[nt]) * 16 + 8 * kh;
                        half4 h;
#pragma unroll
                        for (int e = 0; e < 4; ++e) h[e] = (_Float16)v[e];
                        *(half4*)((char*)a.y + ob) = h;
                        if (VEL) {
#pragma unroll
                            for (int e = 0; e < 4; ++e) h[e] = (_Float16)dv[e];
                            *(half4*)((char*)a.dy + ob) = h;
                        }
                    }
                } else
                if (uok && ook[nt]) {
                    const long ob = ((long)(a.out_g0 + 2 * unit) * a.out_pstride + o[nt]) * 16 + 8 * kh;
                    const long ol = ob + a.out_pstride * 16;
                    half4 hi, lo;
                    split4(v, hi, lo);
                    *(half4*)((char*)a.y + ob) = hi;
                    *(half4*)((char*)a.y + ol) = lo;
                    if (VEL) {
                        split4(dv, hi, lo);
                        *(half4*)((char*)a.dy + ob) = hi;
                        *(half4*)((char*)a.dy + ol) = lo;
                    }
                }
            }
        }
    }
}

template <bool VEL, bool SPLIT = true>
static int launch_stem(ConvKArgs ka, hipStream_t s) {
    ka.tny = (ka.Hv + ST_ROWS - 1) / ST_ROWS;
    ka.tnx = (ka.Wv + ST_COLS - 1) / ST_COLS;
    const long nt = (long)ka.Dv * ka.tny * ka.tnx;
    if (nt <= 0 || nt >= (1L << 31) || ka.cout_groups > 8 || ka.nchunk != 1) return 1;
    ka.ntiles = (int)nt;
    const int grid = (int)std::min<long>(nt, 512);
    static_assert(2 * ST_LDS <= 160 * 1024, "two workgroups per CU");
    ensure_lds_limit((const void*)stem_h3_kernel<VEL, SPLIT>, ST_LDS);
    hipLaunchKernelGGL((stem_h3_kernel<VEL, SPLIT>), dim3(grid), dim3(256), ST_LDS, s, ka);
    return 0;
}

__global__ __launch_bounds__(256) void pack_stem_kernel(const float* __restrict__ w, int cout, int cin, _Float16* __restrict__ dst, int parts) {
    const int idx = blockIdx.x * blockDim.x + threadIdx.x;
    if (idx >= parts * 3 * 4 * 64 * 8) return;
    const int j = idx & 7, co = (idx >> 3) & 63, qq = (idx >> 9) & 3, sp = idx >> 11, st = sp % 3, part = sp / 3;
    const int k = 32 * st + 8 * qq + j, tap = k / 3, ch = k - 3 * tap;
    float v = 0.f;
    if (k < 81 && ch < cin && co < cout) v = w[((size_t)co * cin + ch) * 27 + tap];
    const _Float16 hi = (_Float16)v;
    dst[idx] = part == 0 ? hi : (_Float16)((v - (float)hi) * H3_SCALE);
}

int launch_conv_h3(const PackedW& pw, const ConvKArgs& ka, bool vel, bool has_dx, hipStream_t s) {
    const int ct = pw.ctiles;
    const bool split = pw.prec == PREC_F16X3;
    if (ka.stem_w && !(vel && has_dx) && pw.mode == MODE_FLAT3 && ka.in_off == 0 && ka.osz == 1 &&
        !(ka.flags & F_RES) && ka.nskip == 0 && !ka.beta) {
        if (split) return vel ? launch_stem<true>(ka, s) : launch_stem<false>(ka, s);
        return vel ? launch_stem<true, false>(ka, s) : launch_stem<false, false>(ka, s);
    }
    if ((ka.nskip > 0 || ka.csplit < ka.nchunk) && !(ka.beta && split)) {
        if (split && !vel && ka.ww && pw.mode == MODE_FLAT3 && ka.in_off == 0 && ka.osz == 1)
            return launch_h3w(ka, ka.ww, ka.wws, ka.wws_set_floats, ct, s, true);
        if (!split && vel && has_dx && ka.beta && ka.ww && pw.mode == MODE_FLAT3 && ka.in_off == 0 && ka.osz == 1)
            return launch_h3w(ka, ka.ww, ka.wws, ka.wws_set_floats, ct, s, false, true);
        return 1;
    }
    if (ka.beta) {
        if (!(pw.mode == MODE_FLAT3 && vel && has_dx && ka.in_off == 0 && ka.osz == 1)) return 1;
        if (split) {
            if (pw.cout_t == 16) {
                if (launch_h3nz(ka, ct, pw.cout, s) == 0) return 0;
                return launch_h3g<true>(ka, ct, s);
            }
            if (ka.ww && launch_h3w(ka, ka.ww, ka.wws, ka.wws_set_floats, ct, s) == 0) return 0;
            return launch_h3g<false>(ka, ct, s);
        }
        if (ka.ww && launch_h3w(ka, ka.ww, ka.wws, ka.wws_set_floats, ct, s, false, true) == 0) return 0;
        return launch_h2q<false, true>(ka, ct, s);
    }
    if (pw.mode == MODE_FLAT3) {
        if (!(ka.in_off == 0 && ka.osz == 1)) return 1;
        if (split && vel && has_dx) return launch_h3q(ka, ct, s);
        if (split && !vel && ka.ww && launch_h3w(ka, ka.ww, ka.wws, ka.wws_set_floats, ct, s, true) == 0) return 0;
        if (split && !vel) return launch_h2q<true>(ka, ct, s);
        if (!split && vel && has_dx) return launch_h2q<false>(ka, ct, s);
        if (!vel) launch_h3p_t<false, false, false>(ka, ct, s);
        else if (split) launch_h3p_t<true, false, true>(ka, ct, s);
        else launch_h3p_t<true, false, false>(ka, ct, s);
        return 0;
    }
    if (pw.mode == MODE_FLAT1) {
        if (ka.up8) {
            if (vel && has_dx) return split ? launch_up_h3<true>(ka, ct, s) : launch_up_h3<false>(ka, ct, s);
            if (!vel) return split ? launch_up_h3<true, false>(ka, ct, s) : launch_up_h3<false, false>(ka, ct, s);
            return 1;
        }
        return split ? launch_h3_vd<MODE_FLAT1, true>(ka, ct, vel, has_dx, s) : launch_h3_vd<MODE_FLAT1, false>(ka, ct, vel, has_dx, s);
    }
    return split ? launch_h3_vd<MODE_DOWN, true>(ka, ct, vel, has_dx, s) : launch_h3_vd<MODE_DOWN, false>(ka, ct, vel, has_dx, s);
}

__global__ __launch_bounds__(256) void pack_h3_kernel(const float* __restrict__ w, int cout, int cin, int kind,
                                                      int mode, int nchunk, long halves_per_set, int nsets,
                                                      int parts, int cout_t, _Float16* __restrict__ dst,
                                                      float wscale = 0.f, int* __restrict__ flag = nullptr, int f16w = 0) {
    const long idx = (long)blockIdx.x * blockDim.x + threadIdx.x;
    if (idx >= halves_per_set * nsets) return;
    const int TAPS = mode_taps(mode), nseg = mode_nseg(mode);
    const int nstage = nseg * nchunk;
    long r = idx;
    const int j = (int)(r % 8); r /= 8;
    const int co = (int)(r % cout_t); r /= cout_t;
    const int un = 2 * parts;
    const int u = (int)(r % un); r /= un;
    const int tap = (int)(r % TAPS); r /= TAPS;
    const int stage = (int)(r % nstage); r /= nstage;
    const long per_set_ct = halves_per_set / ((long)nstage * TAPS * un * cout_t * 8);
    const int ct = (int)(r % per_set_ct); r /= per_set_ct;
    const int set = (int)r;
    const int chunk = stage / nseg, seg = stage - chunk * nseg;
    const int h = u / parts, part = u - h * parts;
    const int ci = f16w ? chunk * 32 + 8 * u + j : chunk * 16 + 8 * h + j;
    const int oc = ct * cout_t + co;
    int k, kz, ky, kx;
    if (kind == 0) { k = 3; kz = seg / 3; ky = seg % 3; kx = tap; }
    else if (kind == 1) { k = 1; kz = ky = kx = 0; }
    else if (kind == 2) { k = 2; kz = seg >> 2; ky = (seg >> 1) & 1; kx = seg & 1; }
    else { k = 2; kz = 1 - ((set >> 2) & 1); ky = 1 - ((set >> 1) & 1); kx = 1 - (set & 1); }
    float v = 0.f;
    if (oc < cout && ci < cin) v = w[(((size_t)oc * cin + ci) * k + kz) * k * k + ky * k + kx];
    if (wscale != 0.f) {
        v *= wscale;
        if (!(fabsf(v) <= 60000.f)) { atomicOr(flag, 1); v = 0.f; }
        const _Float16 h = (_Float16)v;
        dst[idx] = (part == 0 || f16w) ? h : (_Float16)(v - (float)h);
        return;
    }
// ... 146 lines not shown
```

### jax_nbody_emulator_with_dj_amd/csrc/nbe_kernels_internal.h

```cpp
#pragma once
#include "nbe_kernels.h"
#include <mutex>
#include <set>
#include <utility>

namespace nbe {

typedef float f32x4 __attribute__((ext_vector_type(4)));
typedef float f32x16 __attribute__((ext_vector_type(16)));
typedef _Float16 half8 __attribute__((ext_vector_type(8)));
typedef _Float16 half4 __attribute__((ext_vector_type(4)));

#define NBE_LDS_AS __attribute__((address_space(3)))
#define NBE_GLB_AS __attribute__((address_space(1)))

struct ConvGroupSrc { const char* x; const char* dx; const char* w; long psb; };

struct ConvKArgs {
    const float* x; const float* dx; long in_pstride;
    int D, H, W; long P; long in_off;
    int Dv, Hv, Wv; long Q;
    float* y; float* dy; long out_pstride; int out_g0;
    int Ho, Wo; int osz, oz, oy, ox;
    const float* r; const float* dr; long res_pstride;
    const float* bias; const float* w; const float* dw;
    int nchunk; int cout_groups; int flags; int ntiles;
    int tny, tnx;
    int zrun;
    const float* gout;
    const float* beta;
    const float* x2; const float* dx2; long in2_pstride; int csplit;
    const float* xs; const float* dxs; long s_pstride; const float* xs2; const float* dxs2; long s2_pstride; int s_csplit;
    const float* ws; const float* dws; int nskip;
    long dws_delta;
    int up8; long set_stride;
    const float* wws; long wws_set_floats;
    const float* ww;
    const float* stem_w;
    ConvGroupSrc gs[NBE_MAX_GROUPS];
};

__device__ __forceinline__ void dma16(const float* src, f32x4* dst_wave_base) {
    __builtin_amdgcn_global_load_lds((const NBE_GLB_AS void*)src, (NBE_LDS_AS void*)dst_wave_base, 16, 0, 0);
}

inline void ensure_lds_limit(const void* kernel, size_t bytes) {
    static std::mutex mu;
    static std::set<std::pair<const void*, int>> done;
    int dev = 0;
    (void)hipGetDevice(&dev);
    std::lock_guard<std::mutex> lock(mu);
    if (done.insert({kernel, dev}).second)
        (void)hipFuncSetAttribute(kernel, hipFuncAttributeMaxDynamicSharedMemorySize, (int)bytes);
}

__device__ __forceinline__ int xcd_tile(int b, int nt) {
    const int qd = nt >> 3, rm = nt & 7, xcd = b & 7;
    return (xcd < rm ? xcd * (qd + 1) : rm * (qd + 1) + (xcd - rm) * qd) + (b >> 3);
}

int launch_conv_h3(const PackedW& pw, const ConvKArgs& ka, bool vel, bool has_dx, hipStream_t s);
void launch_pack_h3(const float* w_oidhw, int cout, int cin, int kind, const PackedW& pw, float* dst, hipStream_t s);
void launch_gather_h8(const float* box, int C, int Db, int Hb, int Wb, int a0, int a1, int a2,
                      float* dst, const Planes& geom, float scale, int parts, hipStream_t s);
void launch_from_planes_h8(const float* src, const Planes& geom, int C, float* dst, int parts, hipStream_t s);
void launch_head_h8(const Planes& y, const Planes& xin, int c0, int C, const HeadScale& hs, bool vel,
                    void* disp, void* velo, int out_dtype, int Db, int Hb, int Wb, int a0, int a1, int a2,
                    int parts, hipStream_t s, int pad = 0);

}
```

### jax_nbody_emulator_with_dj_amd/csrc/nbe_kernels_wino.h

```cpp

#ifndef NBE_EPI_MAX
#define NBE_EPI_MAX 1
#endif
#ifndef NBE_WINO_ZROW
#define NBE_WINO_ZROW 1
#endif
#ifndef NBE_WINO_ITEMREG
#define NBE_WINO_ITEMREG 1
#endif
#ifndef NBE_WINO_LOU
#define NBE_WINO_LOU (NBE_XF_F32 ? 0 : 1)
#endif
constexpr int NBE_MAX_WSTAGES = 32;
constexpr int NBE_MAX_WSKIP = 16;
constexpr float WINO_WSCALE = 16384.0f;
constexpr float WINO_WSCALE_F16 = 256.0f;

struct WinoSrc { const char* xa; const char* xb; long dxd; const char* w; long psb; float sb; int pad_; };

struct WinoKArgs {
    int H, W, Dv, Hv, Wv, Ho, Wo;
    int nchunk, cout_groups, flags, ntiles, tny, tnx;
    int zblock;
    float* y; float* dy; long out_pstride; int out_g0;
    const float* bias; const float* gout; const float* beta;
    const float* r; const float* dr; long res_pstride;
    float inv_scale;
    int nskip;
    long dws_delta;
    WinoSrc st[NBE_MAX_WSTAGES + NBE_MAX_WSKIP];
};

template <bool SKIP, bool NOVEL, bool F16 = false>
__global__ __launch_bounds__(512, 2) void conv_h3w_kernel(WinoKArgs a) {
    static_assert(!(F16 && NOVEL), "the float16 form has no displacement-only variant");
    typedef HGGeom<false> G;
    constexpr int NW = 8, CT = 64, TAPU = G::TAPU, WGU = G::WG, XBASE = G::XBASE, MT = 4, NT = 2, NTILE = 8;
    constexpr int ZROW = G::LDS_UNITS;
    f32x4* lds = lds_h3;
    const half8* L8 = (const half8*)lds_h3;
    half8* L8w = (half8*)lds_h3;
    const int tid = threadIdx.x;
    const int lane = tid & 63;
    const int wave = __builtin_amdgcn_readfirstlane(tid >> 6);
    const int c = lane & 15, q = lane >> 4, kh = q & 1, ks = q >> 1;

    const int nct = (a.cout_groups + 7) / 8;
    const int vt = xcd_tile(blockIdx.x, a.ntiles * nct);
    const int tile = vt / nct, ct = vt - tile * nct;
    const int npair = a.Dv >> 1;
    int zp, ty, tx;
    {
        const int zb = a.zblock;
        const int full = (npair / zb) * zb;
        const int per_blk = zb * a.tny * a.tnx;
        if (tile < (npair / zb) * per_blk) {
            const int blk = tile / per_blk, r = tile - blk * per_blk;
            const int zi = r % zb, tyx = r / zb;
            zp = blk * zb + zi; ty = tyx / a.tnx; tx = tyx - ty * a.tnx;
        } else {
            const int r = tile - (npair / zb) * per_blk, rem = npair - full;
            const int zi = r % rem, tyx = r / rem;
            zp = full + zi; ty = tyx / a.tnx; tx = tyx - ty * a.tnx;
        }
    }
    const int y0 = ty * (NOVEL ? 2 * HP_ROWS : HP_ROWS), x0 = tx * HP_COLS, z0 = 2 * zp;
    const int nst = 4 * a.nchunk;

    const long to = (((long)z0 * a.H + y0) * a.W + x0) * 16;
    const long wcm = (long)ct * nst * WGU * 16, wcs = (long)ct * a.nskip * TAPU * 16;

    struct Nxt { const char *xa, *xb, *w0; long dxd, psb; float sb; } nx;
    auto set_next = [&](int s) {
        const WinoSrc e = a.st[s];
        nx.xa = e.xa + to; nx.xb = e.xb + to; nx.dxd = e.dxd; nx.psb = e.psb; nx.w0 = e.w + (SKIP && s >= nst ? wcs : wcm); nx.sb = e.sb;
    };
    unsigned lane16 = (unsigned)lane << 4;
    asm volatile("" : "+v"(lane16));
    auto dma_w = [&](int buf, int t) {
        const int n = wave + NW * t;
        unsigned l16 = (unsigned)lane;
        if (NBE_WINO_ZROW && !F16) l16 = lane16;
        else asm volatile("v_lshlrev_b32 %0, 4, %0" : "+v"(l16));
        if (n < G::NWI) dma16s(nx.w0 + (long)n * 1024, l16, lds + buf * WGU + n * 64);
    };
    auto dma_raw = [&](int buf) {
        unsigned l16 = (unsigned)lane;
        asm volatile("v_lshlrev_b32 %0, 4, %0" : "+v"(l16));
        dma16s(nx.w0 + (wave < 4 ? 0 : a.dws_delta) + (long)(wave & 3) * 1024, l16, lds + buf * WGU + wave * 64);
#pragma unroll
        for (int t = 0; t < 6; ++t) {
            const int tensor = t / 3, n = wave + NW * (t % 3), pl = n / 6, k = n - 6 * pl;
            const int u = k * 64 + lane;
            const int uu = u < HP_PL ? u : HP_PL - 1;
            const int row = (uu * 241) >> 13, col = uu - row * HP_RS;
            if (u < HP_PL)
                dma16s(nx.xa + (tensor ? nx.dxd : 0) + (long)pl * nx.psb, (unsigned)(row * a.W + col) * 16u,
                       lds + XBASE + buf * HQ_XB + tensor * HQ_XT + pl * HQ_PP + k * 64);
        }
    };
    constexpr bool ITEMREG = NBE_WINO_ITEMREG && !F16;
    int it_uu[3] = {0, 0, 0};
    unsigned it_go[3] = {0u, 0u, 0u};
    if (ITEMREG) {
#pragma unroll
        for (int j = 0; j < 3; ++j) {
            const int u = ((wave + NW * j) % 6) * 64 + lane;
            it_uu[j] = u < HP_PL ? u : HP_PL - 1;
            const int row = (it_uu[j] * 241) >> 13, col = it_uu[j] - row * HP_RS;
            it_go[j] = (unsigned)(row * a.W + col) * 16u;
        }
#pragma unroll
        for (int j = 0; j < 3; ++j) asm volatile("" : "+v"(it_uu[j]), "+v"(it_go[j]));
    }
    auto item_unit = [&](int j, bool& valid) {
        if (ITEMREG) {
            valid = lane < HP_PL - ((wave + NW * j) % 6) * 64;
            return it_uu[j];
        }
        int l = lane;
        asm volatile("" : "+v"(l));
        const int u = ((wave + NW * j) % 6) * 64 + l;
        valid = u < HP_PL;
        return valid ? u : HP_PL - 1;
    };
    auto item_goff_j = [&](int j) {
        if (ITEMREG) return it_go[j];
        bool v;
        const int uu = item_unit(j, v);
        const int row = (uu * 241) >> 13, col = uu - row * HP_RS;
        return (unsigned)(row * a.W + col) * 16u;
    };
    typedef unsigned int u32x4 __attribute__((ext_vector_type(4)));
    struct Stg { half8 ah, al, bh, bl; float sb; };
    auto st_load = [&](int j, Stg& g) {
        const int n = wave + NW * j;
        const long po = ((n / 12) ? nx.dxd : 0) + (long)(((n % 12) / 6) * 2) * nx.psb;
        const char* pa = nx.xa + po;
        const char* pb = nx.xb + po;
        const unsigned go = item_goff_j(j);
        const __amdgpu_buffer_rsrc_t ra = __builtin_amdgcn_make_buffer_rsrc((void*)pa, 0, 0xffffffffu, 0x00027000);
        const __amdgpu_buffer_rsrc_t rb = __builtin_amdgcn_make_buffer_rsrc((void*)pb, 0, 0xffffffffu, 0x00027000);
        const unsigned pso = (unsigned)nx.psb;
        auto ld = [&](half8& d, __amdgpu_buffer_rsrc_t r, unsigned so) {
            const u32x4 v = __builtin_amdgcn_raw_buffer_load_b128(r, go, so, 0);
            d = __builtin_bit_cast(half8, v);
        };
        ld(g.ah, ra, 0); ld(g.al, ra, pso); ld(g.bh, rb, 0); ld(g.bl, rb, pso);
        g.sb = nx.sb;
    };
#if NBE_XF_F32
    struct Xf { u32x4 HI, LO; float t0, t1; unsigned h; };
    auto xf_step = [&](const Stg& g, Xf& x, int k) {
        const int r = k >> 2, m = k & 3;
        const unsigned AH = __builtin_bit_cast(u32x4, g.ah)[r], AL = __builtin_bit_cast(u32x4, g.al)[r];
        const unsigned BH = __builtin_bit_cast(u32x4, g.bh)[r], BL = __builtin_bit_cast(u32x4, g.bl)[r];
        const float inv = H3_INV, sinv = g.sb * H3_INV, sb = g.sb, k2048 = H3_SCALE;
        if (m == 0) {
            asm("v_fma_mix_f32 %0, %1, %2, %3 op_sel:[0,0,0] op_sel_hi:[1,0,1]" : "=v"(x.t0) : "v"(AL), "s"(inv), "v"(AH));
            asm("v_fma_mix_f32 %0, %1, %2, %0 op_sel:[0,0,0] op_sel_hi:[1,0,0]" : "+v"(x.t0) : "v"(BL), "s"(sinv));
            asm("v_fma_mix_f32 %0, %1, %2, %0 op_sel:[0,0,0] op_sel_hi:[1,0,0]" : "+v"(x.t0) : "v"(BH), "s"(sb));
        } else if (m == 1) {
            asm("v_fma_mix_f32 %0, %1, %2, %3 op_sel:[1,0,1] op_sel_hi:[1,0,1]" : "=v"(x.t1) : "v"(AL), "s"(inv), "v"(AH));
            asm("v_fma_mix_f32 %0, %1, %2, %0 op_sel:[1,0,0] op_sel_hi:[1,0,0]" : "+v"(x.t1) : "v"(BL), "s"(sinv));
            asm("v_fma_mix_f32 %0, %1, %2, %0 op_sel:[1,0,0] op_sel_hi:[1,0,0]" : "+v"(x.t1) : "v"(BH), "s"(sb));
        } else if (m == 2) {
            asm("v_cvt_pk_f16_f32 %0, %1, %2" : "=v"(x.h) : "v"(x.t0), "v"(x.t1));
            asm("v_fma_mix_f32 %0, %1, -1.0, %0 op_sel:[0,0,0] op_sel_hi:[1,0,0]" : "+v"(x.t0) : "v"(x.h));
            asm("v_fma_mix_f32 %0, %1, -1.0, %0 op_sel:[1,0,0] op_sel_hi:[1,0,0]" : "+v"(x.t1) : "v"(x.h));
        } else {
            unsigned l;
            asm("v_fma_mixlo_f16 %0, %1, %2, 0 op_sel_hi:[0,0,0]" : "=v"(l) : "v"(x.t0), "s"(k2048));
            asm("v_fma_mixhi_f16 %0, %1, %2, 0 op_sel_hi:[0,0,0]" : "+v"(l) : "v"(x.t1), "s"(k2048));
            x.HI[r] = x.h; x.LO[r] = l;
        }
    };
#else
    struct Xf { u32x4 HI, LO; unsigned s, bb, e1, e2, l1; };
    auto xf_step = [&](const Stg& g, Xf& x, int k) {
        const int r = k >> 2, m = k & 3;
        const unsigned AH = __builtin_bit_cast(u32x4, g.ah)[r], AL = __builtin_bit_cast(u32x4, g.al)[r];
        const unsigned BH = __builtin_bit_cast(u32x4, g.bh)[r], BL = __builtin_bit_cast(u32x4, g.bl)[r];
        const unsigned sbp = g.sb < 0.f ? 0xBC00BC00u : 0x3C003C00u, k2048 = 0x68006800u;
        if (F16) {
            if (m == 0) asm("v_pk_fma_f16 %0, %1, %2, %3" : "=v"(x.s) : "v"(BH), "s"(sbp), "v"(AH));
            else if (m == 1) asm("v_pk_fma_f16 %0, %1, %2, %3" : "=v"(x.l1) : "v"(BL), "s"(sbp), "v"(AL));
            else if (m == 3) { x.HI[r] = x.s; x.LO[r] = x.l1; }
            (void)k2048;
        } else
        if (m == 0) {
            asm("v_pk_fma_f16 %0, %1, %2, %3" : "=v"(x.s) : "v"(BH), "s"(sbp), "v"(AH));
            asm("v_pk_add_f16 %0, %1, %2 neg_lo:[0,1] neg_hi:[0,1]" : "=v"(x.bb) : "v"(x.s), "v"(AH));
        } else if (m == 1) {
            asm("v_pk_add_f16 %0, %1, %2 neg_lo:[0,1] neg_hi:[0,1]" : "=v"(x.e1) : "v"(x.s), "v"(x.bb));
            asm("v_pk_fma_f16 %0, %1, %2, %3 neg_lo:[0,0,1] neg_hi:[0,0,1]" : "=v"(x.e2) : "v"(BH), "s"(sbp), "v"(x.bb));
        } else if (m == 2) {
            asm("v_pk_add_f16 %0, %1, %2 neg_lo:[0,1] neg_hi:[0,1]" : "=v"(x.e1) : "v"(AH), "v"(x.e1));
            asm("v_pk_fma_f16 %0, %1, %2, %3" : "=v"(x.l1) : "v"(BL), "s"(sbp), "v"(AL));
        } else {
            unsigned err, l;
            asm("v_pk_add_f16 %0, %1, %2" : "=v"(err) : "v"(x.e1), "v"(x.e2));
#if NBE_WINO_LOU
            const unsigned kinv = 0x10001000u;
            asm("v_pk_fma_f16 %0, %1, %2, %3" : "=v"(l) : "v"(x.l1), "s"(kinv), "v"(err));
            (void)k2048;
#else
            asm("v_pk_fma_f16 %0, %1, %2, %3" : "=v"(l) : "v"(err), "s"(k2048), "v"(x.l1));
#endif
            x.HI[r] = x.s; x.LO[r] = l;
        }
    };
#endif
    auto st_write = [&](int j, int buf, const Xf& x) {
        bool valid;
// ... 33 lines not shown
    };
    auto LB = [&](half8 (&r)[NT], int idx) {
#pragma unroll
        for (int nt = 0; nt < NT; ++nt) r[nt] = L8[idx + 16 * nt];
    };
    const _Float16 kInv = (_Float16)H3_INV;
#define SNAKE(i) ((((i) >> 1) & 1) ? ((i) ^ 1) : (i))
    auto nohook = [](int) {};
    auto MM8h = [&](f32x4 (&acc)[NTILE], const half8 (&A)[MT], const half8 (&B)[NT], int slot, int nb, bool px, bool zsel,
                    bool hooked, auto&& hook) {
#pragma unroll
        for (int i = 0; i < NTILE; ++i) {
            const int t = SNAKE(i);
            if (zsel && (i % NT) == 0) mmz(acc[t], A[t / NT], B[t % NT]); else
            mm(acc[t], A[t / NT], B[t % NT]);
            if (hooked) { hook(i); __builtin_amdgcn_sched_barrier(0); }
            if (slot >= 0 && (i % 4) == 3) {
                if (px) dma_w(nb, slot + i / 4);
                __builtin_amdgcn_sched_barrier(0);
            }
        }
    };
    auto MM8 = [&](f32x4 (&acc)[NTILE], const half8 (&A)[MT], const half8 (&B)[NT], int slot, int nb, bool px, bool zsel = false) {
        MM8h(acc, A, B, slot, nb, px, zsel, false, nohook);
    };
    auto MM8s = [&](f32x4 (&acc)[NTILE], half8 (&P)[MT], const half8 (&A)[MT], const half8 (&B)[NT], int slot, int nb, bool px) {
        P[0] = A[0] * kInv;
#pragma unroll
        for (int i = 0; i < NTILE; ++i) {
            const int t = SNAKE(i);
            if ((i % NT) == 0) { if (t / NT + 1 < MT) P[t / NT + 1] = A[t / NT + 1] * kInv; mmz(acc[t], P[t / NT], B[t % NT]); }
            else mm(acc[t], P[t / NT], B[t % NT]);
            if (slot >= 0 && (i % 4) == 3) {
                if (px) dma_w(nb, slot + i / 4);
                __builtin_amdgcn_sched_barrier(0);
            }
        }
    };
#define NBE_SB __builtin_amdgcn_sched_barrier(0)
    half8 wh[MT], wl[MT], wp[MT], xh[NT], xl[NT], dxh[NT], dxl[NT];
    auto pair = [&](f32x4 (&Y)[NTILE], f32x4 (&DY)[NTILE], int slot0, int nb, bool px, int wa, int xp,
                    auto&& preXl, auto&& preW, auto&& preXh, auto&& mid, bool hooked, auto&& hook, auto&& after3) {
        if (F16) {
            LB(dxh, xp + HQ_XT); LA(wl, wa + CT + aP);
            NBE_SB; MM8h(Y, wh, xh, slot0, nb, px, false, hooked, [&](int t) { hook(t); }); NBE_SB;
            LB(dxl, xp + HQ_XT + HQ_PP);
            NBE_SB; MM8h(Y, wl, xl, slot0 < 0 ? -1 : slot0 + 2, nb, px, false, hooked, [&](int t) { hook(8 + t); }); NBE_SB;
            after3();
            mid();
            preXl(); preXh();
            NBE_SB; MM8(DY, wh, dxh, slot0 < 0 ? -1 : slot0 + 4, nb, px); NBE_SB;
            preW();
            NBE_SB; MM8(DY, wl, dxl, -1, nb, px); NBE_SB;
            return;
        }
        LB(dxh, xp + HQ_XT);
#if NBE_WINO_LOU
        NBE_SB; MM8(Y, wh, xl, slot0, nb, px); NBE_SB;
#else
        NBE_SB; MM8s(Y, wp, wh, xl, slot0, nb, px); NBE_SB;
#endif
        LB(dxl, xp + HQ_XT + HQ_PP);
        NBE_SB; MM8h(Y, wh, xh, slot0 < 0 ? -1 : slot0 + 2, nb, px, false, hooked, [&](int t) { hook(t); }); NBE_SB;
        LA(wl, wa + CT + aP);
        NBE_SB; MM8h(DY, wh, dxh, slot0 < 0 ? -1 : slot0 + 4, nb, px, false, hooked, [&](int t) { hook(8 + t); }); NBE_SB;
        after3();
        mid();
#if NBE_WINO_LOU
        NBE_SB; MM8(DY, wh, dxl, -1, nb, px); NBE_SB;
#else
        NBE_SB; MM8(DY, wp, dxl, -1, nb, px); NBE_SB;
#endif
        preXl(); preW();
        NBE_SB; MM8(Y, wl, xh, -1, nb, px); NBE_SB;
        preXh();
        NBE_SB; MM8(DY, wl, dxh, -1, nb, px); NBE_SB;
    };

    constexpr int SH4 = HP_RS + 1, SH5 = HP_RS + 2, SH7 = 2 * HP_RS + 1;
    auto stage = [&](f32x4 (&Y)[NTILE], f32x4 (&DY)[NTILE], int s, auto nxt) {
        constexpr int NXT = decltype(nxt)::value;
        constexpr bool px = NXT == 1;
        const bool pre = px && s + 1 != 2 * a.nchunk;
        if (NXT) set_next(s + 1);
        int par = s & 1;
        asm volatile("" : "+s"(par));
        int nb = 1 - par;
        asm volatile("" : "+s"(nb));
        const int wb = par * WGU, xb = XBASE + par * HQ_XB;
        const int wbn = nb * WGU, xbn = XBASE + nb * HQ_XB;
        Stg g;
        Xf xf;
        auto hk = [&](int k) { xf_step(g, xf, k); };
        auto none = [] {};
        if (NXT == 2) dma_raw(nb);
        if (px) st_load(0, g);
        pair(Y, DY, 0, nb, px, wb, xb + bP1,
             [&] { LB(xl, xb + 2 + bP32 + HQ_PP); }, [&] { LA(wh, wb + 2 * TAPU + aP); }, [&] { LB(xh, xb + 2 + bP32); },
             none, false, nohook, none);
        half8 a1[MT], a2[MT], b1x[NT], b1d[NT];
        const int aS = wb + 4 * TAPU + (2 * kh + (F16 ? ks : 0)) * CT + c;
        const int bS = xb + (2 * kh + ks) * HQ_PP + rowp * HP_RS + c + SH4;
        pair(Y, DY, -1, nb, px, wb + 2 * TAPU, xb + 2 + bP32,
             [&] { LB(b1x, bS); }, [&] { LA(a1, aS); }, [&] { LB(b1d, bS + HQ_XT); }, none,
             px, hk, [&] { if (px) { st_write(0, nb, xf); st_load(1, g); } });
        const half8 zero = {0, 0, 0, 0, 0, 0, 0, 0};
        if (F16) {
            NBE_SB; MM8(Y, a1, b1x, -1, 0, false); NBE_SB;
            LB(xl, xb + SH5 + bP32 + HQ_PP); LB(xh, xb + SH5 + bP32); LA(wh, wb + 5 * TAPU + aP);
            NBE_SB; MM8(DY, a1, b1d, -1, 0, false); NBE_SB;
        } else {
#if NBE_WINO_LOU
        NBE_SB; MM8(Y, a1, b1x, -1, 0, false); NBE_SB;
#else
        {
            const _Float16 m1 = ks ? kInv : (_Float16)1.0f;
#pragma unroll
            for (int mt = 0; mt < MT; ++mt) a1[mt] = a1[mt] * m1;
        }
        NBE_SB; MM8(Y, a1, b1x, -1, 0, false, true); NBE_SB;
#endif
#if NBE_WINO_ZROW
        LA(a2, ks ? ZROW + c : aS + CT);
#else
        LA(a2, aS + CT);
#endif
        LB(xl, xb + SH5 + bP32 + HQ_PP);
        NBE_SB; MM8(DY, a1, b1d, -1, 0, false); NBE_SB;
        LB(xh, xb + SH5 + bP32); LA(wh, wb + 5 * TAPU + aP);
#if NBE_WINO_ZROW
        NBE_SB; MM8(Y, a2, b1x, -1, 0, false); NBE_SB;
#else
#pragma unroll
        for (int mt = 0; mt < MT; ++mt) a2[mt] = ks ? zero : a2[mt];
        NBE_SB; MM8(Y, a2, b1x, -1, 0, false, true); NBE_SB;
#endif
        MM8(DY, a2, b1d, -1, 0, false); NBE_SB;
        }
        pair(Y, DY, -1, nb, px, wb + 5 * TAPU, xb + SH5 + bP32,
             [&] { LB(xl, xb + SH7 + bP1 + HQ_PP); }, [&] { LA(wh, wb + 7 * TAPU + aP); }, [&] { LB(xh, xb + SH7 + bP1); },
             none, px, hk, [&] { if (px) { st_write(1, nb, xf); st_load(2, g); } });
        pair(Y, DY, -1, nb, px, wb + 7 * TAPU, xb + SH7 + bP1,
             [&] { if (pre) LB(xl, xbn + bP1 + HQ_PP); }, [&] { if (pre) LA(wh, wbn + aP); }, [&] { if (pre) LB(xh, xbn + bP1); },
             [&] { asm volatile("s_waitcnt vmcnt(0) lgkmcnt(0)\n\ts_barrier" ::: "memory"); },
             px, hk, [&] { if (px) st_write(2, nb, xf); });
    };

    auto raw_stage = [&](f32x4 (&Y)[NTILE], f32x4 (&DY)[NTILE], int s, bool px) {
        if (px) set_next(s + 1);
        int par = s & 1;
        asm volatile("" : "+s"(par));
        int nb = 1 - par;
        asm volatile("" : "+s"(nb));
        const int wb = par * WGU, xb = XBASE + par * HQ_XB;
        if (px) dma_raw(nb);
        half8 a1[MT], a2[MT], d1[MT], d2[MT], bx[NT], bd[NT];
        const half8 zero = {0, 0, 0, 0, 0, 0, 0, 0};
        const _Float16 m1 = ks ? kInv : (_Float16)1.0f;
        const int aS = wb + (2 * kh) * CT + c;
        const int bS = xb + (2 * kh + ks) * HQ_PP + rowp * HP_RS + c + SH4;
        if (F16) {
            const int aF = wb + (2 * kh + ks) * CT + c;
            LA(a1, aF); LB(bx, bS); LB(bd, bS + HQ_XT); LA(d1, aF + TAPU);
            NBE_SB; MM8(Y, a1, bx, -1, 0, false); NBE_SB;
            MM8(DY, a1, bd, -1, 0, false); NBE_SB;
            MM8(DY, d1, bx, -1, 0, false); NBE_SB;
            asm volatile("s_waitcnt vmcnt(0) lgkmcnt(0)\n\ts_barrier" ::: "memory");
            return;
        }
        LA(a1, aS); LB(bx, bS); LA(a2, aS + CT); LB(bd, bS + HQ_XT);
#pragma unroll
        for (int mt = 0; mt < MT; ++mt) a1[mt] = a1[mt] * m1;
        NBE_SB; MM8(Y, a1, bx, -1, 0, false, true); NBE_SB;
        if (!NOVEL) LA(d1, aS + TAPU);
#pragma unroll
        for (int mt = 0; mt < MT; ++mt) a2[mt] = ks ? zero : a2[mt];
        NBE_SB; MM8(Y, a2, bx, -1, 0, false, true); NBE_SB;
        if (!NOVEL) LA(d2, aS + TAPU + CT);
        if (NOVEL || !(a.flags & F_SKIP_NODX)) {
            NBE_SB; MM8(DY, a1, bd, -1, 0, false); NBE_SB;
            MM8(DY, a2, bd, -1, 0, false); NBE_SB;
        }
        if (!NOVEL) {
#pragma unroll
            for (int mt = 0; mt < MT; ++mt) { d1[mt] = d1[mt] * m1; d2[mt] = ks ? zero : d2[mt]; }
            NBE_SB; MM8(DY, d1, bx, -1, 0, false, true); NBE_SB;
            MM8(DY, d2, bx, -1, 0, false, true); NBE_SB;
        }
        asm volatile("s_waitcnt vmcnt(0) lgkmcnt(0)\n\ts_barrier" ::: "memory");
    };

    {
        if (NBE_WINO_ZROW && !F16 && tid < 64) L8w[ZROW + tid] = half8{0, 0, 0, 0, 0, 0, 0, 0};
        set_next(0);
#pragma unroll
        for (int k = 0; k < G::NWS; ++k) dma_w(0, k);
        {
            Stg g0, g1, g2;
            st_load(0, g0); st_load(1, g1); st_load(2, g2);
            st_store(0, 0, g0); st_store(1, 0, g1); st_store(2, 0, g2);
        }
        asm volatile("s_waitcnt vmcnt(0) lgkmcnt(0)" ::: "memory");
        __syncthreads();
        LA(wh, aP); LB(xl, XBASE + bP1 + HQ_PP); LB(xh, XBASE + bP1);
    }

    auto butterfly = [&] {
            asm volatile("s_nop 15\n\ts_nop 15" ::: "memory");
#pragma unroll
            for (int t = 0; t < NTILE; ++t) {
                f32x4 p, m;
#pragma unroll
                for (int e = 0; e < 4; ++e) { p[e] = acc_read(YA[t][e]); m[e] = acc_read(YB[t][e]); }
                YA[t] = p + m; YB[t] = p - m;
                asm volatile("" : "+a"(YA[t]), "+a"(YB[t]));
                __builtin_amdgcn_sched_barrier(0);
#pragma unroll
                for (int e = 0; e < 4; ++e) { p[e] = acc_read(DA[t][e]); m[e] = acc_read(DB[t][e]); }
                DA[t] = p + m; DB[t] = p - m;
                asm volatile("" : "+a"(DA[t]), "+a"(DB[t]));
                __builtin_amdgcn_sched_barrier(0);
            }
            asm volatile("s_nop 7" ::: "memory");
            LA(wh, aP); LB(xl, XBASE + bP1 + HQ_PP); LB(xh, XBASE + bP1);
    };
    const int npairs = 2 * a.nchunk;
    for (int s2 = 0; s2 + 1 < npairs; ++s2) {
        if (s2 == a.nchunk) butterfly();
        stage(YA, DA, 2 * s2, std::integral_constant<int, 1>());
        stage(YB, DB, 2 * s2 + 1, std::integral_constant<int, 1>());
    }
    if (npairs - 1 == a.nchunk) butterfly();
    stage(YA, DA, 2 * npairs - 2, std::integral_constant<int, 1>());
    stage(YB, DB, 2 * npairs - 1, std::integral_constant<int, SKIP ? 2 : 0>());
    if (SKIP) {
        for (int sc = 0; sc < a.nskip; ++sc) {
            raw_stage(YA, DA, nst + 2 * sc, true);
            raw_stage(YB, DB, nst + 2 * sc + 1, sc + 1 < a.nskip);
        }
    }
#undef NBE_SB
#undef SNAKE
    asm volatile("s_nop 15\n\ts_nop 15" ::: "memory");

    const bool act = a.flags & F_ACT, gauge = !NOVEL && a.gout != nullptr;
    f32x4 bv[MT], be[MT], gv[MT];
    int unit[MT];
    bool uok[MT];
#pragma unroll
    for (int mt = 0; mt < MT; ++mt) {
        unit[mt] = ct * (CT / 8) + 2 * mt + ks;
        uok[mt] = unit[mt] < a.cout_groups;
        if (!uok[mt]) unit[mt] = a.cout_groups - 1;
        bv[mt] = *(const f32x4*)(a.bias + unit[mt] * 8 + 4 * kh);
        be[mt] = f32x4{0.f, 0.f, 0.f, 0.f};
        if (!NOVEL) be[mt] = *(const f32x4*)(a.beta + unit[mt] * 8 + 4 * kh);
        gv[mt] = f32x4{0.f, 0.f, 0.f, 0.f};
        if (!NOVEL && gauge) gv[mt] = *(const f32x4*)(a.gout + unit[mt] * 8 + 4 * kh);
    }
#pragma unroll
    for (int mt = 0; mt < MT; ++mt) asm volatile("" : "+v"(bv[mt]), "+v"(be[mt]), "+v"(gv[mt]));
    long ob_mt[MT];
#pragma unroll
    for (int mt = 0; mt < MT; ++mt) ob_mt[mt] = (long)(a.out_g0 + (F16 ? 1 : 2) * unit[mt]) * a.out_pstride * 16 + 8 * kh;
    const long ol_off = a.out_pstride * 16;
    auto epilogue = [&](f32x4 (&Y)[NTILE], f32x4 (&DY)[NTILE], int z) {
        int o[NT];
        bool ook[NT], ook2[NT];
#pragma unroll
        for (int nt = 0; nt < NT; ++nt) {
            const int yy = y0 + rowp, xx = x0 + 16 * nt + c;
            ook[nt] = yy < a.Hv && xx < a.Wv;
            ook2[nt] = NOVEL && yy + HP_ROWS < a.Hv && xx < a.Wv;
            o[nt] = ook[nt] ? (z * a.Ho + yy) * a.Wo + xx : z * a.Ho * a.Wo;
        }
        half4 r0[F16 ? NTILE : 1], r1[F16 ? NTILE : 1];
        const bool res = F16 && (a.flags & F_RES);
// ... 54 lines not shown
                    }
                    const long ob = ob_mt[mt] + (long)o[nt] * 16;
                    const long ol = ob + ol_off;
                    const long r8 = (long)HP_ROWS * a.Wo * 16;
                    half4 hi, lo;
                    if (uok[mt] && ook[nt]) {
                        split4(v, hi, lo);
                        *(half4*)((char*)a.y + ob) = hi;
                        *(half4*)((char*)a.y + ol) = lo;
                    }
                    if (uok[mt] && ook2[nt]) {
                        split4(dv, hi, lo);
                        *(half4*)((char*)a.y + ob + r8) = hi;
                        *(half4*)((char*)a.y + ol + r8) = lo;
                    }
                } else
                if (uok[mt] && ook[nt]) {
                    const long ob = ob_mt[mt] + (long)o[nt] * 16;
                    const long ol = ob + ol_off;
                    half4 hi, lo;
                    split4(v, hi, lo);
                    *(half4*)((char*)a.y + ob) = hi;
                    *(half4*)((char*)a.y + ol) = lo;
                    split4(dv, hi, lo);
                    *(half4*)((char*)a.dy + ob) = hi;
                    *(half4*)((char*)a.dy + ol) = lo;
                }
            }
        }
    };
    epilogue(YA, DA, z0);
    epilogue(YB, DB, z0 + 1);
}

__global__ __launch_bounds__(256) void pack_h3w_kernel(const float* __restrict__ w, int cout, int cin, int nchunk, long total,
                                                       _Float16* __restrict__ dst, int* __restrict__ flag, int f16) {
    const long idx = (long)blockIdx.x * blockDim.x + threadIdx.x;
    if (idx >= total) return;
    long r = idx;
    const int j = (int)(r % 8); r /= 8;
    const int co = (int)(r % 64); r /= 64;
    const int u = (int)(r % 4); r /= 4;
    const int tap = (int)(r % 9); r /= 9;
    const int stage = (int)(r % (4 * nchunk)); r /= 4 * nchunk;
    const int ct = (int)r;
    const int chunk = stage >> 2, xi = stage & 3;
    const int h = u >> 1, part = u & 1;
    const int ci = f16 ? chunk * 32 + 8 * u + j : chunk * 16 + 8 * h + j, oc = ct * 64 + co;
    float v = 0.f;
    if (oc < cout && ci < cin) {
        const float* p = w + (((size_t)oc * cin + ci) * 3) * 9 + tap;
        const float w0 = p[0], w1 = p[9], w2 = p[18];
        v = xi == 0 ? w0 : xi == 1 ? 0.5f * (w0 + w1 + w2) : xi == 2 ? 0.5f * (w0 - w1 + w2) : -w2;
    }
    v *= f16 ? WINO_WSCALE_F16 : WINO_WSCALE;
    if (!(fabsf(v) <= 60000.f)) { atomicOr(flag, 1); v = 0.f; }
    const _Float16 hi = (_Float16)v;
    dst[idx] = (part == 0 || f16) ? hi : (_Float16)(v - (float)hi);
}

void launch_pack_h3w(const float* w_oidhw, int cout, int cin, int cin_pad, int ctiles, float* dst, int* flag, hipStream_t s, int prec) {
    const bool f16 = prec == PREC_F16;
    const int nchunk = cin_pad / (f16 ? 32 : 16);
    const long total = (long)ctiles * 4 * nchunk * 9 * 4 * 64 * 8;
    hipLaunchKernelGGL(pack_h3w_kernel, dim3((unsigned)((total + 255) / 256)), dim3(256), 0, s, w_oidhw, cout, cin, nchunk, total,
                       (_Float16*)dst, flag, f16 ? 1 : 0);
}

static int launch_h3w(const ConvKArgs& ka_in, const float* ww, const float* wws, long wws_set_floats, int ctiles, hipStream_t s,
                      bool novel = false, bool f16 = false) {
    typedef HGGeom<false> G;
    constexpr size_t smem = (size_t)(G::LDS_UNITS + 64) * 16;
    static_assert(smem <= 160 * 1024, "LDS budget of one CU");
    ConvKArgs ka = ka_in;
    if (f16) {
        if (novel || (ka.nchunk & 1) || (ka.csplit < ka.nchunk && (ka.csplit & 1))) return 1;
        if (ka.nskip > 0 && ((ka.nskip & 1) || (ka.s_csplit < ka.nskip && (ka.s_csplit & 1)) || (ka.flags & F_SKIP_NODX))) return 1;
        ka.nchunk /= 2; if (ka.csplit < (1 << 29)) ka.csplit /= 2;
        ka.nskip /= 2; if (ka.s_csplit < (1 << 29)) ka.s_csplit /= 2;
    }
    if (!ww || (!f16 && (ka.flags & F_RES)) || (ka.Dv & 1) || 4 * ka.nchunk > NBE_MAX_WSTAGES || (!novel && !ka.beta)) return 1;
    if (ka.nskip > 0 && (!wws || 2 * ka.nskip > NBE_MAX_WSKIP)) return 1;
    if (ctiles != (ka.cout_groups + 7) / 8) return 1;
    if (std::max(ka.in_pstride, ka.csplit < ka.nchunk ? ka.in2_pstride : 0L) * 16 + 16L * (HP_ROWS + 2) * ka.W >= (1L << 32) - (1L << 20)) return 1;
    WinoKArgs wa;
    wa.H = ka.H; wa.W = ka.W; wa.Dv = ka.Dv; wa.Hv = ka.Hv; wa.Wv = ka.Wv; wa.Ho = ka.Ho; wa.Wo = ka.Wo;
    wa.nchunk = ka.nchunk; wa.cout_groups = ka.cout_groups; wa.flags = ka.flags;
    const int trows = novel ? 2 * HP_ROWS : HP_ROWS;
    wa.tny = (ka.Hv + trows - 1) / trows;
    wa.tnx = (ka.Wv + HP_COLS - 1) / HP_COLS;
    wa.ntiles = (ka.Dv / 2) * wa.tny * wa.tnx;
    wa.y = ka.y; wa.dy = ka.dy; wa.out_pstride = ka.out_pstride; wa.out_g0 = ka.out_g0;
    wa.bias = ka.bias; wa.gout = novel ? nullptr : ka.gout; wa.beta = novel ? nullptr : ka.beta;
    const long rows8 = (long)HP_ROWS * ka.W * 16;
    wa.inv_scale = 1.0f / (f16 ? WINO_WSCALE_F16 : WINO_WSCALE);
    wa.r = ka.r; wa.dr = ka.dr; wa.res_pstride = ka.res_pstride;
    wa.zblock = std::min(8, ka.Dv / 2);
    wa.nskip = ka.nskip; wa.dws_delta = wws_set_floats * 4;
    static const int XI[2][2] = {{1, 2}, {0, 3}};
    static const int PA[4] = {0, 1, 2, 1}, PB[4] = {2, 2, 1, 3};
    static const float SB[4] = {-1.f, 1.f, -1.f, -1.f};
    const long plane = (long)ka.H * ka.W * 16;
    for (int ph = 0; ph < 2; ++ph)
        for (int chunk = 0; chunk < ka.nchunk; ++chunk)
            for (int ab = 0; ab < 2; ++ab) {
                const int xi = XI[ph][ab];
                const bool second = chunk >= ka.csplit;
                const long ps = second ? ka.in2_pstride : ka.in_pstride;
                const char* x = (const char*)(second ? ka.x2 : ka.x);
                const char* dx = (const char*)(second ? ka.dx2 : ka.dx);
                const long off = (long)(second ? chunk - ka.csplit : chunk) * 4 * ps * 16;
                WinoSrc& e = wa.st[(ph * ka.nchunk + chunk) * 2 + ab];
                e.xa = x + off + PA[xi] * plane; e.xb = x + off + PB[xi] * plane; e.dxd = novel ? rows8 : dx - x;
                e.w = (const char*)ww + (long)(chunk * 4 + xi) * G::WG * 16; e.psb = ps * 16; e.sb = SB[xi]; e.pad_ = 0;
            }
    for (int sc = 0; sc < ka.nskip; ++sc)
        for (int ab = 0; ab < 2; ++ab) {
            const bool second = sc >= ka.s_csplit;
            const long ps = second ? ka.s2_pstride : ka.s_pstride;
            const char* x = (const char*)(second ? ka.xs2 : ka.xs);
            const char* dx = (const char*)(second ? ka.dxs2 : ka.dxs);
            const long off = (long)(second ? sc - ka.s_csplit : sc) * 4 * ps * 16 + ab * plane;
            WinoSrc& e = wa.st[4 * ka.nchunk + 2 * sc + ab];
            e.xa = x + off; e.xb = e.xa; e.dxd = novel ? rows8 : dx - x; e.w = (const char*)wws + (long)sc * G::TAPU * 16; e.psb = ps * 16; e.sb = 0.f; e.pad_ = 0;
        }
    const bool skip = ka.nskip > 0;
    if (novel) wa.dws_delta = 0;
    auto kern = f16 ? (skip ? conv_h3w_kernel<true, false, true> : conv_h3w_kernel<false, false, true>)
              : novel ? (skip ? conv_h3w_kernel<true, true> : conv_h3w_kernel<false, true>)
              : (skip ? conv_h3w_kernel<true, false> : conv_h3w_kernel<false, false>);
    ensure_lds_limit((const void*)kern, smem);
    dim3 grid(wa.ntiles * ctiles, 1, 1), block(512, 1, 1);
    hipLaunchKernelGGL(kern, grid, block, smem, s, wa);
    return 0;
}
```

### jax_nbody_emulator_with_dj_amd/engine.py

```python

import ctypes as C

import numpy as np

from . import _lib
from ._lib import LayerDesc, NBEError, NBERangeError, check

try:
    import torch
except Exception:
    torch = None

BLOCKS = ('conv_l00', 'conv_l01', 'down_l0', 'conv_l1', 'down_l1', 'conv_l2', 'down_l2', 'conv_c',
          'up_r2', 'conv_r2', 'up_r1', 'conv_r1', 'up_r0', 'conv_r00', 'conv_r01')


def _is_torch(x):
    return torch is not None and isinstance(x, torch.Tensor)


def _f32(a):
    return np.ascontiguousarray(np.asarray(a, dtype=np.float32))


# ... 63 lines not shown
        except Exception:
            pass

    def load_params(self, params, premodulated):
        if params is None:
            raise ValueError("No parameters loaded. Use load_params=True in create_emulator.")
        tree = params['params'] if 'params' in params else params
        descs, keep = [], []
        for b in BLOCKS:
            if b not in tree:
                raise NBEError("parameter tree is missing block %s" % b)
            for l, lp in tree[b].items():
                w = _f32(lp['weight'])
                bias = _f32(lp['bias'])
                d = LayerDesc()
                d.block, d.layer = b.encode(), l.encode()
                d.cout, d.cin, d.k = int(w.shape[0]), int(w.shape[1]), int(w.shape[2])
                d.weight, d.bias = w.ctypes.data, bias.ctypes.data
                keep += [w, bias]
                if premodulated:
                    if 'style_weight' in lp:
                        raise NBEError("%s/%s holds style parameters but a premodulated model was requested" % (b, l))
                    if self.compute_vel:
                        if 'dweight' not in lp:
                            raise NBEError("%s/%s: premodulated velocity parameters need 'dweight'" % (b, l))
                        dw = _f32(lp['dweight'])
                        d.dweight = dw.ctypes.data
                        keep.append(dw)
                else:
                    if 'style_weight' not in lp:
                        raise NBEError("%s/%s has no style parameters; pass premodulated weights to the "
                                       "NBodyEmulator[Vel]Core models instead" % (b, l))
                    sw, sb = _f32(lp['style_weight']), _f32(lp['style_bias'])
                    d.style_weight, d.style_bias = sw.ctypes.data, sb.ctypes.data
                    keep += [sw, sb]
                descs.append(d)
        arr = (LayerDesc * len(descs))(*descs)
        fn = self._l.nbe_load_premod_weights if premodulated else self._l.nbe_load_style_weights
        check(fn(self._h, arr, len(descs)))
        self._keep = keep
        self.loaded = params_fingerprint(params)
        self.premodulated = bool(premodulated)

    def invalidate(self):
        self.loaded = None

    def ensure_params(self, params, premodulated):
        if params is None:
            raise ValueError("No parameters loaded. Use load_params=True in create_emulator.")
        if self.loaded != params_fingerprint(params) or self.premodulated != bool(premodulated):
            self.load_params(params, premodulated)

    def set_cosmology(self, Om, Dz):
        check(self._l.nbe_set_cosmology(self._h, float(Om), float(Dz)))

    def set_stream(self, stream_ptr):
        check(self._l.nbe_set_stream(self._h, C.c_void_p(stream_ptr) if stream_ptr else None))
        self._stream_ptr = int(stream_ptr or 0)

    def use_own_stream(self):
        check(self._l.nbe_use_own_stream(self._h))
        self._stream_ptr = None

    def set_max_tile(self, max_tile):
        check(self._l.nbe_set_max_tile(self._h, int(max_tile)))
        self.max_tile = int(max_tile)

    def set_slab(self, slab):
        check(self._l.nbe_set_slab(self._h, int(slab)))

    def set_periodic(self, on):
        check(self._l.nbe_set_periodic(self._h, 1 if on else 0))

    def plan_tiles(self, region, ndiv, periodic_box=True):
        out = (C.c_int * 3)()
        check(self._l.nbe_plan_tiles_ctx(self._h, (C.c_int64 * 3)(*[int(r) for r in region]),
                                         (C.c_int * 3)(*[int(n) for n in ndiv]), 1 if periodic_box else 0, out))
        return tuple(out)

    def synchronize(self):
        check(self._l.nbe_synchronize(self._h))

    QUERY = {"gauge_active": 0, "slab": 1, "periodic_yx": 2, "periodic_z": 3, "range_shift": 4, "workspace_bytes": 5,
             "host_pipe": 6, "graph_replays": 7, "plan_tiles": 8, "plan_short_gb": 9}

    def query(self, what):
        out = C.c_double()
        check(self._l.nbe_query(self._h, self.QUERY[what], C.byref(out)))
        return out.value

    def check_finite(self):
        check(self._l.nbe_check_finite(self._h))

    def set_input_range(self, absmax):
        check(self._l.nbe_set_input_range(self._h, -1.0 if absmax is None else float(absmax)))

    def _follow_torch_stream(self, t=None):
        if t is not None and (t.device.index or 0) != self.device:
            raise NBEError("tensor lives on cuda:%d but this engine was created for cuda:%d"
                           % (t.device.index or 0, self.device))
        sp = int(torch.cuda.current_stream(self.device).cuda_stream)
        if getattr(self, '_stream_ptr', None) != sp:
            self.set_stream(sp)

    def forward(self, x, Dz, vel_fac=0.0):
        Cc, D, H, W = x.shape
        if Cc != self.in_chan:
            raise NBEError("input has %d channels, model expects %d" % (Cc, self.in_chan))
        oshape = (self.out_chan, D - 96, H - 96, W - 96)
        if min(oshape) <= 0:
            raise NBEError("input %s is smaller than the receptive field (needs > 96 per axis)" % (tuple(x.shape),))
        if _is_torch(x):
            self._follow_torch_stream(x)
            x = x.contiguous().float()
            disp = torch.empty(oshape, dtype=torch.float32, device=x.device)
            vel = torch.empty(oshape, dtype=torch.float32, device=x.device) if self.compute_vel else None
        else:
            x = _f32(x)
            disp = np.empty(oshape, np.float32)
            vel = np.empty(oshape, np.float32) if self.compute_vel else None
        check(self._l.nbe_forward(self._h, _ptr(x), D, H, W, float(Dz), float(vel_fac), _ptr(disp), _ptr(vel)))
        if _is_torch(x):
            self.check_finite()
        return (disp, vel) if self.compute_vel else disp

    def process_box(self, box, size, ndiv, padding, Dz, vel_fac=0.0, out_dtype=np.float32, progress=None,
                    out=None, check_finite=True):
        size = tuple(int(s) for s in size)
        if tuple(box.shape) != (self.in_chan,) + size:
            raise NBEError("input_box shape %s does not match (in_chan,)+size = %s" % (tuple(box.shape), (self.in_chan,) + size))
        half = np.dtype(out_dtype) == np.float16
        if not half and np.dtype(out_dtype) != np.float32:
            raise NBEError("output dtype %s unsupported (float32 / float16)" % np.dtype(out_dtype))
        oshape = (self.out_chan,) + size
        if _is_torch(box):
            self._follow_torch_stream(box)
            box = box.contiguous().float()
            tdt = torch.float16 if half else torch.float32
            if out is not None:
                disp, vel = out
            else:
                disp = torch.zeros(oshape, dtype=tdt, device=box.device)
                vel = torch.zeros(oshape, dtype=tdt, device=box.device) if self.compute_vel else None
        else:
            box = _f32(box)
            disp = _lib.pinned_empty(oshape, np.float16 if half else np.float32)
            vel = _lib.pinned_empty(oshape, disp.dtype) if self.compute_vel else None
        sz = (C.c_int64 * 3)(*size)
        nd = (C.c_int * 3)(*[int(n) for n in ndiv])
        pd = (C.c_int * 6)(*[int(p) for pp in padding for p in pp])
        cb = _lib.PROGRESS_CB(progress) if progress is not None else C.cast(None, _lib.PROGRESS_CB)
        check(self._l.nbe_process_box(self._h, _ptr(box), sz, nd, pd, float(Dz), float(vel_fac), _ptr(disp),
                                      _ptr(vel), 1 if half else 0, cb, None))
        if _is_torch(box) and check_finite:
            self.check_finite()
        return (disp, vel) if self.compute_vel else disp

    def process_region(self, box, origin, region, ndiv, Dz, vel_fac, disp, vel, out_origin=(0, 0, 0), order=None):
        self._follow_torch_stream(box)
        i64 = lambda t: (C.c_int64 * 3)(*[int(v) for v in t])
        half = disp.element_size() == 2
        nd = (C.c_int * 3)(*[int(n) for n in ndiv])
        if order is not None:
            oarr = (C.c_int * len(order))(*[int(o) for o in order])
            if len(order) == 0:
                return
        else:
# ... 7 lines not shown
    def brick_halo_bytes(self, bshape, which=1):
        n = int(self._l.nbe_brick_halo_bytes(self._h, (C.c_int64 * 3)(*[int(v) for v in bshape]), int(which)))
        if n < 0:
            raise NBEError("nbe_brick_halo_bytes failed")
        return n

    def brick_plan(self, bshape):
        return int(self._l.nbe_brick_plan(self._h, (C.c_int64 * 3)(*[int(v) for v in bshape])))

    def _check_faces(self, bshape, which, *faces):
        n = self.brick_halo_bytes(bshape, which)
        for t in faces:
            if not t.is_cuda or t.numel() * t.element_size() < n:
                raise NBEError("brick exchange buffers must be CUDA tensors of at least %d bytes" % n)

    def brick_encode(self, haloed, bshape, Dz, vel_fac, send_lo, send_hi, skip_send_lo, skip_send_hi):
        self._follow_torch_stream(haloed)
        b = tuple(int(v) for v in bshape)
        self._brick = b
        want = (self.in_chan, b[0] + 2 * self.RAW_HALO, b[1], b[2])
        if tuple(haloed.shape) != want or haloed.dtype != torch.float32 or not haloed.is_contiguous():
            raise NBEError("haloed brick must be a contiguous float32 (C, b0 + 8, S1, S2) = %s tensor; got %s %s"
                           % (want, tuple(haloed.shape), haloed.dtype))
        self._check_faces(b, 1, send_lo, send_hi)
        self._check_faces(b, 3, skip_send_lo, skip_send_hi)
        check(self._l.nbe_brick_encode(self._h, _ptr(haloed), (C.c_int64 * 3)(*b), float(Dz), float(vel_fac),
                                       _ptr(send_lo), _ptr(send_hi), _ptr(skip_send_lo), _ptr(skip_send_hi)))

    def brick_interior(self):
        check(self._l.nbe_brick_interior(self._h))

    def brick_exchange(self, recv_lo, recv_hi, send2_lo, send2_hi):
        self._check_faces(self._brick, 1, recv_lo, recv_hi)
        self._check_faces(self._brick, 2, send2_lo, send2_hi)
        check(self._l.nbe_brick_exchange(self._h, _ptr(recv_lo), _ptr(recv_hi), _ptr(send2_lo), _ptr(send2_hi)))

    def brick_finish(self, recv2_lo, recv2_hi, skip_recv_lo, skip_recv_hi, Dz, vel_fac, disp, vel, skip_ready=None):
        self._follow_torch_stream(disp)
        half = disp.element_size() == 2
        self._check_faces(self._brick, 2, recv2_lo, recv2_hi)
        self._check_faces(self._brick, 3, skip_recv_lo, skip_recv_hi)
        ev = C.c_void_p(skip_ready.cuda_event) if skip_ready is not None else None
        check(self._l.nbe_brick_finish(self._h, _ptr(recv2_lo), _ptr(recv2_hi), _ptr(skip_recv_lo), _ptr(skip_recv_hi), ev,
                                       float(Dz), float(vel_fac), _ptr(disp), _ptr(vel), 1 if half else 0))

    def test_layer(self, kind, x, w, bias, dx=None, dw=None, crop=0, act=False, res=None, dres=None):
        kinds = {'conv3': 0, 'skip': 1, 'down': 2, 'up': 3}
        k = kinds[kind]
        x = _f32(x); w = _f32(w); bias = _f32(bias)
        cin, D, H, W = x.shape
        cout = w.shape[0]
        if k == 0: osp = (D - 2, H - 2, W - 2)
        elif k == 1: osp = (D - 2 * crop, H - 2 * crop, W - 2 * crop)
        elif k == 2: osp = (D // 2, H // 2, W // 2)
        else: osp = (2 * D, 2 * H, 2 * W)
        vel = dw is not None
        dx = None if dx is None else _f32(dx)
        dw = None if dw is None else _f32(dw)
        res = None if res is None else _f32(res)
        dres = None if dres is None else _f32(dres)
        y = np.empty((cout,) + osp, np.float32)
        dy = np.empty_like(y) if vel else None
        flags = (1 if act else 0) | (2 if res is not None else 0)
        check(self._l.nbe_test_layer(self._h, k, int(crop), flags, _ptr(x), _ptr(dx), cin, D, H, W, _ptr(w), _ptr(dw),
                                     _ptr(bias), cout, _ptr(res), _ptr(dres), _ptr(y), _ptr(dy)))
        return (y, dy) if vel else y

    def test_layer_gauged(self, x, dx, w, beta, bias, act=False, res=None, dres=None):
        x, dx, w, beta, bias = _f32(x), _f32(dx), _f32(w), _f32(beta), _f32(bias)
        cin, D, H, W = x.shape
        cout = w.shape[0]
        y = np.empty((cout, D - 2, H - 2, W - 2), np.float32)
        dy = np.empty_like(y)
        if res is not None:
            res, dres = _f32(res), _f32(dres)
            check(self._l.nbe_test_layer_gauged_res(self._h, (1 if act else 0) | 2, _ptr(x), _ptr(dx), cin, D, H, W, _ptr(w),
                                                    _ptr(beta), _ptr(bias), cout, _ptr(res), _ptr(dres), _ptr(y), _ptr(dy)))
            return y, dy
        check(self._l.nbe_test_layer_gauged(self._h, 1 if act else 0, _ptr(x), _ptr(dx), cin, D, H, W, _ptr(w), _ptr(beta),
                                            _ptr(bias), cout, _ptr(y), _ptr(dy)))
        return y, dy

    PATHS = {"skip_fused": 1, "two_source": 2, "wino_0": 4, "wino_1": 8, "narrow": 16, "up8": 32, "skip_nodx": 64,
             "two_source_skip": 128}

    def test_block(self, block, x, dx=None, x2=None, dx2=None, pad=0, two_source=False):
        x = _f32(x)
        dx, x2, dx2 = (None if a is None else _f32(a) for a in (dx, x2, dx2))
        m, vel = self.mid_chan, self.compute_vel
        _, D, H, W = x.shape
        res = block.startswith('conv_')
        if res:
            cout = self.out_chan if block == 'conv_r01' else m
            cmid = 2 * m if block in ('conv_r2', 'conv_r1', 'conv_r00') else m
            sy = 0 if pad else 2
            y = np.empty((cout, D - 4, H - 2 * sy, W - 2 * sy), np.float32)
            h = np.empty((cmid, D - 2, H - sy, W - sy), np.float32)
        elif block.startswith('down_'):
            y, h = np.empty((m, D // 2, H // 2, W // 2), np.float32), None
        else:
            y, h = np.empty((m if x2 is None else 2 * m, 2 * D, 2 * H, 2 * W), np.float32), None
        dy = np.empty_like(y) if vel else None
        dh = np.empty_like(h) if (vel and h is not None) else None
        g = np.zeros((3, 2 * m), np.float32)
        word = C.c_int(0)
        check(self._l.nbe_test_block(self._h, block.encode(), int(pad), 1 if two_source else 0, _ptr(x), _ptr(dx), D, H, W,
                                     _ptr(x2), _ptr(dx2), _ptr(y), _ptr(dy), _ptr(h), _ptr(dh), _ptr(g), C.byref(word)))
        cin = x.shape[0] if (x2 is None or not res) else 2 * m
        return {"y": y, "dy": dy, "h": h, "dh": dh, "gauge_in": g[0, :cin], "gauge_hidden": None if h is None else g[1, :h.shape[0]],
                "gauge_out": g[2, :(m if not res else y.shape[0])],
                "paths": {k for k, b in self.PATHS.items() if word.value & b}}

    def test_modulate(self, weight, style_weight, style_bias, s, first_layer, eps=1e-8, vel=True):
        weight, sw, sb = _f32(weight), _f32(style_weight), _f32(style_bias)
        cout, cin, k = weight.shape[:3]
        wn = np.empty_like(weight)
        dw = np.empty_like(weight) if vel else None
        check(self._l.nbe_test_modulate(self._h, _ptr(weight), _ptr(sw), _ptr(sb), cout, cin, k, float(s[0]),
                                        float(s[1]), float(eps), 1 if first_layer else 0, _ptr(wn), _ptr(dw)))
        return (wn, dw) if vel else wn

    def probe_begin(self, origin, nout=8):
        o = (C.c_int64 * 3)(*[int(v) for v in origin])
        check(self._l.nbe_probe_begin(self._h, o, int(nout)))

    def probe_read(self):
        out, total, lay = {}, 0, []
        for i in range(self._l.nbe_probe_slots(self._h)):
            name = C.create_string_buffer(64)
            dims, off = (C.c_int * 3)(), C.c_int64()
            check(self._l.nbe_probe_layout(self._h, i, name, 64, dims, C.byref(off)))
            lay.append((name.value.decode(), dims[0], dims[1], dims[2], off.value))
            total = max(total, off.value + dims[0] * dims[1] * dims[1] * dims[2])
        words = np.empty(total, dtype=np.uint32)
        check(self._l.nbe_probe_read(self._h, words.ctypes.data_as(C.c_void_p), total))
        for name, c, n, nw, off in lay:
            w = words[off:off + c * n * n * nw].reshape(c, n, n, nw)
            bits = np.unpackbits(w.view(np.uint8), axis=-1, bitorder='little')
            out[name] = bits[..., :n].astype(bool)
        return out

    def probe_end(self):
        check(self._l.nbe_probe_end(self._h))

    def profile_enable(self, on=True):
        check(self._l.nbe_profile_enable(self._h, 1 if on else 0))

    def profile_reset(self):
        check(self._l.nbe_profile_reset(self._h))

    def profile_read(self):
        n = self._l.nbe_profile_count(self._h)
        out = []
        for i in range(n):
            name = C.create_string_buffer(128)
            ms, la, fl = C.c_double(), C.c_int64(), C.c_double()
            check(self._l.nbe_profile_entry(self._h, i, name, 128, C.byref(ms), C.byref(la), C.byref(fl)))
            out.append({'kernel': name.value.decode(), 'ms': ms.value, 'launches': la.value, 'flops': fl.value})
        return out

    def workspace_bytes(self):
        return int(self._l.nbe_workspace_bytes(self._h))

    def debug_phase_cycles(self):
        out = (C.c_double * 16)()
        check(self._l.nbe_debug_phase_cycles(self._h, out))
        return list(out)
# ... 1 lines not shown
```

Baseline: 98.43 million.

## Read periodic yx halo by index wrap in Winograd loads instead of fill kernels

```diff
diff --git a/include/nbe.h b/include/nbe.h
--- a/include/nbe.h
+++ b/include/nbe.h
@@ -52,6 +52,7 @@
        NBE_Q_HOST_PIPE = 6,
        NBE_Q_GRAPH_REPLAYS = 7,
        NBE_Q_PLAN_TILES = 8,
+       NBE_Q_HALO_FILLS = 10,
        NBE_Q_PLAN_SHORT_GB = 9 };
 int nbe_query(nbe_ctx* ctx, int what, double* out);
 
@@ -172,7 +173,8 @@
        NBE_PATH_NARROW = 16,
        NBE_PATH_UP8 = 32,
        NBE_PATH_SKIP_NODX = 64,
-       NBE_PATH_TWO_SOURCE_SKIP = 128   };
+       NBE_PATH_TWO_SOURCE_SKIP = 128,
+       NBE_PATH_WRAP_LOAD = 256         };
 int nbe_test_block(nbe_ctx* ctx, const char* block, int pad, int two_source, const float* x, const float* dx, int D, int H, int W,
                    const float* x2, const float* dx2, float* y, float* dy, float* h, float* dh, float* gauges, int* paths);
 int nbe_test_modulate(nbe_ctx* ctx, const float* weight, const float* style_weight, const float* style_bias,
diff --git a/jax_nbody_emulator_with_dj_amd/csrc/nbe_engine.cpp b/jax_nbody_emulator_with_dj_amd/csrc/nbe_engine.cpp
--- a/jax_nbody_emulator_with_dj_amd/csrc/nbe_engine.cpp
+++ b/jax_nbody_emulator_with_dj_amd/csrc/nbe_engine.cpp
@@ -338,6 +338,7 @@
     case NBE_Q_GRAPH_REPLAYS: *out = (double)c->graph_replays; break;
     case NBE_Q_PLAN_TILES: *out = (double)c->plan_tiles; break;
     case NBE_Q_PLAN_SHORT_GB: *out = c->plan_short_gb; break;
+    case NBE_Q_HALO_FILLS: *out = (double)c->halo_fills; break;
     default: return fail("nbe_query: unknown item %d", what);
     }
     return 0;
diff --git a/jax_nbody_emulator_with_dj_amd/csrc/nbe_engine_box.cpp b/jax_nbody_emulator_with_dj_amd/csrc/nbe_engine_box.cpp
--- a/jax_nbody_emulator_with_dj_amd/csrc/nbe_engine_box.cpp
+++ b/jax_nbody_emulator_with_dj_amd/csrc/nbe_engine_box.cpp
@@ -175,6 +175,7 @@
                       int OD, int OH, int OW, int a0, int a1, int a2) {
     c->sst.valid = false;
     c->arena.reset();
+    if (!c->dry) c->halo_fills = 0;
     Tensor tin = talloc(c, c->in_chan, D, H, W), y;
     tin.pad = c->pyx ? 1 : 0;
     if (tin.pad) set_org(tin, 0, 48, 48);
@@ -207,7 +208,7 @@
     const int geo[18] = {Db, Hb, Wb, o0, o1, o2, D, H, W, out_dtype, OD, OH, OW, a0, a1, a2, c->slab, c->prec};
     memcpy(k.geo, geo, sizeof geo);
     k.f[0] = Dz; k.f[1] = vel_fac; k.f[2] = c->act_scale;
-    k.epoch = c->epoch; k.flags = (c->pyx ? 1 : 0) | (c->pz ? 2 : 0) | (c->gauge_active ? 4 : 0) | (c->fuse ? 8 : 0) | (wino_env_off() ? 16 : 0);
+    k.epoch = c->epoch; k.flags = (c->pyx ? 1 : 0) | (c->pz ? 2 : 0) | (c->gauge_active ? 4 : 0) | (c->fuse ? 8 : 0) | (wino_env_off() ? 16 : 0) | (wrap_env_on() ? 32 : 0);
     nbe_ctx::GraphVal& g = c->graphs[k];
     g.used = ++c->graph_clock;
     if (!g.exec && g.seen++ == 0) {
diff --git a/jax_nbody_emulator_with_dj_amd/csrc/nbe_engine_internal.h b/jax_nbody_emulator_with_dj_amd/csrc/nbe_engine_internal.h
--- a/jax_nbody_emulator_with_dj_amd/csrc/nbe_engine_internal.h
+++ b/jax_nbody_emulator_with_dj_amd/csrc/nbe_engine_internal.h
@@ -84,7 +84,7 @@
     float* dwn_f = nullptr;
 };
 
-struct Tensor { Planes p; int64_t off = -1; int pad = 0; int org[3] = {0, 0, 0}; };
+struct Tensor { Planes p; int64_t off = -1; int pad = 0; int org[3] = {0, 0, 0}; bool halo = true; };
 
 struct ProfEntry { std::string name; double ms = 0; int64_t launches = 0; double flops = 0; };
 
@@ -219,6 +219,7 @@
         unsigned* count = nullptr;
     } probe;
     int* paths = nullptr;
+    int64_t halo_fills = 0;
     bool prof = false;
     std::vector<ProfEntry> prof_entries;
     struct Pending { int entry; hipEvent_t a, b; };
@@ -239,14 +240,16 @@
 int check_range(nbe_ctx* c);
 
 int planes_for(int C, int prec);
-Tensor talloc(nbe_ctx* c, int C, int D, int H, int W);
-Tensor tallocp(nbe_ctx* c, int C, int D, int Hi, int Wi, int pad);
+Tensor talloc(nbe_ctx* c, int C, int D, int H, int W, bool zero_tail = true);
+Tensor tallocp(nbe_ctx* c, int C, int D, int Hi, int Wi, int pad, bool zero_tail = true);
 void fill_halo(nbe_ctx* c, const Tensor& t);
 void tfree(nbe_ctx* c, Tensor& t);
 Tensor zview(const Tensor& t, int z0, int nz);
 void set_org(Tensor& t, int z, int y, int x);
 bool wino_f16_layer(int prec, bool vel, int cin_pad);
 bool wino_env_off();
+bool wrap_env_on();
+bool wrap_mode(const nbe_ctx* c);
 bool up8_launch(const nbe_ctx* c, const Layer& L, bool has_dx);
 int run_conv(nbe_ctx* c, const Layer& L, const ConvLaunch& cl_in, bool has_dx);
 const Layer* find_layer(nbe_ctx* c, const char* block, const char* layer);
@@ -256,8 +259,8 @@
 int resblock_part(nbe_ctx* c, const char* name, const Tensor& x, const Tensor& h, const Tensor& s,
                   int js, int ns, int jh, int nh, bool has_dx, bool final_act, const int* zr, const Tensor* x2 = nullptr);
 int resblock(nbe_ctx* c, const char* name, const Tensor& x, bool has_dx, bool final_act, int cout, int cmid, Tensor* out,
-             Tensor* hidden_out = nullptr);
-int down_conv(nbe_ctx* c, const Layer& L, const Tensor& x, Tensor& o, bool probe);
+             Tensor* hidden_out = nullptr, bool out_halo = true, const int* zr = nullptr);
+int down_conv(nbe_ctx* c, const Layer& L, const Tensor& x, Tensor& o, bool probe, const int* zr = nullptr);
 int downblock(nbe_ctx* c, const char* name, const Tensor& x, Tensor* out);
 int upblock(nbe_ctx* c, const char* name, const Tensor& x, const Tensor& cat, int xcrop = 0, int g0 = -1);
 void crop_into(nbe_ctx* c, const Tensor& src, int crop, const Tensor& dst, int cz = -1);
diff --git a/jax_nbody_emulator_with_dj_amd/csrc/nbe_engine_net.cpp b/jax_nbody_emulator_with_dj_amd/csrc/nbe_engine_net.cpp
--- a/jax_nbody_emulator_with_dj_amd/csrc/nbe_engine_net.cpp
+++ b/jax_nbody_emulator_with_dj_amd/csrc/nbe_engine_net.cpp
@@ -17,19 +17,19 @@
     return p;
 }
 
-Tensor talloc(nbe_ctx* c, int C, int D, int H, int W) {
+Tensor talloc(nbe_ctx* c, int C, int D, int H, int W, bool zero_tail) {
     Tensor t;
     t.p = ws_planes(c, planes_for(C, c->prec), D, H, W, &t.off);
     const int gw = c->prec == PREC_F16 ? (C + 7) / 8 : c->prec == PREC_F16X3 ? 2 * ((C + 7) / 8) : (C + 3) / 4;
-    if (!c->dry && t.off >= 0 && gw < t.p.G) {
+    if (!c->dry && zero_tail && t.off >= 0 && gw < t.p.G) {
         const size_t off = (size_t)gw * t.p.pstride * 4, bytes = (size_t)(t.p.G - gw) * t.p.pstride * 16;
         launch_zero(t.p.x + off, (int64_t)bytes, c->stream);
         if (t.p.dx) launch_zero(t.p.dx + off, (int64_t)bytes, c->stream);
     }
     return t;
 }
-Tensor tallocp(nbe_ctx* c, int C, int D, int Hi, int Wi, int pad) {
-    Tensor t = talloc(c, C, D, Hi + 2 * pad, Wi + 2 * pad);
+Tensor tallocp(nbe_ctx* c, int C, int D, int Hi, int Wi, int pad, bool zero_tail) {
+    Tensor t = talloc(c, C, D, Hi + 2 * pad, Wi + 2 * pad, zero_tail);
     t.pad = pad;
     return t;
 }
@@ -40,8 +40,12 @@
     if (p.dx) p.dx += sh;
     return p;
 }
+static void fill_planes(nbe_ctx* c, const Planes& p, int pad) {
+    launch_fill_yx(p, pad, c->vel, c->stream);
+    ++c->halo_fills;
+}
 void fill_halo(nbe_ctx* c, const Tensor& t) {
-    if (t.pad > 0 && !c->dry) launch_fill_yx(t.p, t.pad, c->vel, c->stream);
+    if (t.pad > 0 && t.halo && !c->dry) fill_planes(c, t.p, t.pad);
 }
 void tfree(nbe_ctx* c, Tensor& t) { if (t.off >= 0) c->arena.release(t.off); t.off = -1; }
 Tensor zview(const Tensor& t, int z0, int nz) {
@@ -76,6 +80,11 @@
 
 bool wino_f16_layer(int prec, bool vel, int cin_pad) { return prec == PREC_F16 && vel && cin_pad % 32 == 0 && cin_pad / 32 <= 8; }
 bool wino_env_off() { return getenv("NBE_WINO") && atoi(getenv("NBE_WINO")) == 0; }
+bool wrap_env_on() { return !(getenv("NBE_WRAP") && atoi(getenv("NBE_WRAP")) == 0); }
+bool wrap_mode(const nbe_ctx* c) {
+    return c->vel && c->prec == PREC_F16X3 && c->gauge_active && c->wino_ok && !wino_env_off() && wrap_env_on();
+}
+static bool wraps_layer(const nbe_ctx* c, const Layer& L) { return wrap_mode(c) && L.kind == 0 && L.g6 && L.pw.ww && !L.pwn.w; }
 bool up8_launch(const nbe_ctx* c, const Layer& L, bool has_dx) { return prec_is_half(c->prec) && (!c->vel || has_dx) && L.pw.cin_pad <= 64; }
 
 int run_conv(nbe_ctx* c, const Layer& L, const ConvLaunch& cl_in, bool has_dx) {
@@ -91,6 +100,13 @@
     const PackedW& pw = (g6 && L.kind == 0 && L.pwn.w) ? L.pwn : L.pw;
     cl.wino = (g6 || nov) && c->wino_ok && &pw == &L.pw && pw.ww && (!cl.skw || cl.skw->ww) && (c->prec == PREC_F16 || !(cl.flags & F_RES)) &&
               (cl.Dv & 1) == 0 && cl.in_off == 0 && cl.osz == 1 && !wino_env_off();
+    const bool reads_halo = L.kind == 0 && cl.pad1;
+    cl.wrap = reads_halo && cl.wino && g6 && c->vel && c->prec == PREC_F16X3 && pw.cout_t != 16 && wrap_env_on();
+    auto fill_inputs = [&] {
+        fill_planes(c, cl.in, 1);
+        if (cl.csplit_ch) fill_planes(c, cl.in2, 1);
+    };
+    if (reads_halo && !cl.wrap && cl.halo_missing) fill_inputs();
     if (c->paths)
         *c->paths |= (cl.skw ? NBE_PATH_SKIP_FUSED : 0) | (cl.skw && (cl.flags & F_SKIP_NODX) ? NBE_PATH_SKIP_NODX : 0) |
                      (cl.csplit_ch ? NBE_PATH_TWO_SOURCE : 0) | (cl.skw && cl.sk_split_ch ? NBE_PATH_TWO_SOURCE_SKIP : 0) |
@@ -106,7 +122,14 @@
         ea = get_event(c); eb = get_event(c);
         (void)hipEventRecord(ea, c->stream);
     }
-    if (launch_conv(pw, cl, c->vel, has_dx, c->stream))
+    int lrc = launch_conv(pw, cl, c->vel, has_dx, c->stream);
+    if (lrc == 2) {
+        if (cl.halo_missing) fill_inputs();
+        cl.wrap = false;
+        lrc = launch_conv(pw, cl, c->vel, has_dx, c->stream);
+    }
+    if (c->paths && cl.wrap) *c->paths |= NBE_PATH_WRAP_LOAD;
+    if (lrc)
         return fail("internal error: no kernel for layer %s/%s (mode %d, gauged %d, input tangent %d, crop offset %ld, output stride %d)",
                     L.block.c_str(), L.layer.c_str(), L.pw.mode, (int)g6, (int)has_dx, (long)cl.in_off, cl.osz);
     if (c->prof) {
@@ -162,14 +185,16 @@
     {
         ConvLaunch cl; cl.in = zview(x, jh, nh + 2).p; cl.Dv = nh; cl.Hv = H - 2; cl.Wv = W - 2; cl.out = inner(hv); cl.flags = F_ACT;
         if (x2) { cl.in2 = zview(*x2, jh, nh + 2).p; cl.csplit_ch = c->mid; }
+        cl.pad1 = pad == 1; cl.halo_missing = !x.halo || (x2 && !x2->halo);
         if (run_conv(c, *L0, cl, has_dx)) return 1;
         org_conv(x, 1, og); og[0] += jh;
         const int zh[3] = {zr ? zr[0] : 0, zr ? zr[1] + 2 : 0, zr ? zr[2] : 0};
         probe_act(c, *L0, cl.out, 0, og, cl.Dv, cl.Hv, cl.Wv, pad != 0, zr ? zh : nullptr);
     }
-    fill_halo(c, hv);
+    const bool h_halo = h.halo && !wraps_layer(c, *L1);
+    if (h_halo) fill_halo(c, hv);
     {
-        ConvLaunch cl; cl.in = zview(h, js, ns + 2).p; cl.Dv = ns; cl.Hv = s.p.H - 2 * pad; cl.Wv = s.p.W - 2 * pad; cl.out = inner(sv);
+        ConvLaunch cl; cl.in = zview(h, js, ns + 2).p; cl.pad1 = pad == 1; cl.halo_missing = !h_halo; cl.Dv = ns; cl.Hv = s.p.H - 2 * pad; cl.Wv = s.p.W - 2 * pad; cl.out = inner(sv);
         if (fused) { cl.sk = xs.p; cl.sk_off = sk_off; cl.skw = L1->pwn.w ? &Ls->pwn : &Ls->pw; cl.flags = (final_act ? F_ACT : 0) | (has_dx ? 0 : F_SKIP_NODX);
                      if (x2) { cl.sk2 = zview(*x2, js, ns + 4).p; cl.sk_split_ch = c->mid; } }
         else { cl.res = inner(sv); cl.flags = F_RES | (final_act ? F_ACT : 0); }
@@ -182,7 +207,7 @@
 }
 
 int resblock(nbe_ctx* c, const char* name, const Tensor& x, bool has_dx, bool final_act, int cout, int cmid, Tensor* out,
-                    Tensor* hidden_out) {
+                    Tensor* hidden_out, bool out_halo, const int* zr) {
     const Layer* L1 = find_layer(c, name, "conv_1");
     if (!L1) return fail("missing layers of block %s", name);
     const int D = x.p.D, pad = x.pad;
@@ -190,7 +215,8 @@
     Tensor s = tallocp(c, cout, D - 4, x.p.H - 2 * pad - 2 * sy, x.p.W - 2 * pad - 2 * sy, pad);
     Tensor h = alloc_hidden(c, cmid, D - 2, x, block_fused(c, L1, D - 4));
     if (s.off < 0 || h.off < 0) return fail("workspace exhausted in block %s", name);
-    if (resblock_part(c, name, x, h, s, 0, D - 4, 0, D - 2, has_dx, final_act, nullptr)) return 1;
+    s.halo = out_halo;
+    if (resblock_part(c, name, x, h, s, 0, D - 4, 0, D - 2, has_dx, final_act, zr)) return 1;
     tfree(c, h);
     if (hidden_out) *hidden_out = h;
     int og[3];
@@ -204,12 +230,16 @@
     if (c->dry || n <= 0) return;
     launch_crop(zview(t, src, n).p, 0, zview(t, dst, n).p, 0, c->vel, c->stream, 0);
 }
-
-int down_conv(nbe_ctx* c, const Layer& L, const Tensor& x, Tensor& o, bool probe) {
+static void wrap_planes_z(nbe_ctx* c, const Tensor& t, int lo, int h, int n) {
+    for (int b = lo; b > lo - n;) { const int k = std::min(h, b - (lo - n)); carry_planes(c, t, b - k + h, b - k, k); b -= k; }
+    for (int a = lo + h; a < lo + h + n;) { const int k = std::min(h, lo + h + n - a); carry_planes(c, t, a - h, a, k); a += k; }
+}
+
+int down_conv(nbe_ctx* c, const Layer& L, const Tensor& x, Tensor& o, bool probe, const int* zr) {
     ConvLaunch cl; cl.in = inner(x); cl.Dv = o.p.D; cl.Hv = o.p.H; cl.Wv = o.p.W; cl.out = o.p; cl.flags = F_ACT;
     if (run_conv(c, L, cl, true)) return 1;
     set_org(o, x.org[0] / 2, x.org[1] / 2, x.org[2] / 2);
-    if (probe) probe_act(c, L, cl.out, 0, o.org, cl.Dv, cl.Hv, cl.Wv, x.pad != 0);
+    if (probe) probe_act(c, L, cl.out, 0, o.org, cl.Dv, cl.Hv, cl.Wv, x.pad != 0, zr);
     return 0;
 }
 
@@ -279,10 +309,18 @@
     const int Y = D - 8;
     const bool zx = pad && c->zx;
     const bool pz = pad && (c->pz || zx);
-    const int zlo = pz ? (zx ? 44 : 40) : 0, zhi = pz ? (zx ? Y - 44 : Y - 40) : Y;
+    const bool zcopy = pz && !zx;
+    const int zlo = pz ? (zx ? 44 : 40) : 0, zhi = pz ? (zx ? Y - 44 : Y - 48) : Y;
+    bool zcopied = false;
     Tensor skip0 = pad ? tallocp(c, m, Y - 80, Hi, Wi, pad) : talloc(c, m, Y - 80, H - 88, W - 88);
-    Tensor td = pad ? talloc(c, m, pz ? (D - 96) / 2 : Y / 2, Hi / 2, Wi / 2) : talloc(c, m, Y / 2, (H - 8) / 2, (W - 8) / 2);
+    const bool inpl = pad && !zx;
+    const int zc1 = (inpl && pz) ? 6 : 0;
+    Tensor td = inpl ? tallocp(c, m, pz ? (D - 96) / 2 + 2 * zc1 : Y / 2, Hi / 2, Wi / 2, 1)
+              : pad ? talloc(c, m, (D - 96) / 2, Hi / 2, Wi / 2) : talloc(c, m, Y / 2, (H - 8) / 2, (W - 8) / 2);
     if (skip0.off < 0 || td.off < 0) return fail("workspace exhausted (level 0)");
+    const bool halos = !wrap_mode(c);
+    skip0.halo = halos;
+    if (inpl) td.halo = halos;
     const Layer* Ld = find_layer(c, "down_l0", "conv_0");
     if (!Ld) return fail("missing layer down_l0/conv_0");
     const int sy = pad ? 0 : 2;
@@ -294,6 +332,7 @@
     Tensor h1 = alloc_hidden(c, m, S + 2, a, block_fused(c, L01, S));
     Tensor y0r = pz ? Tensor() : tallocp(c, m, S, Hi - 4 * sy, Wi - 4 * sy, pad);
     if (h0.off < 0 || a.off < 0 || h1.off < 0 || (!pz && y0r.off < 0)) return fail("workspace exhausted (level-0 encoder slabs)");
+    a.halo = halos; y0r.halo = halos;
     const int zr00[3] = {zlo, zhi + 4, pz ? D - 96 : 0}, zr01[3] = {zlo, zhi, pz ? D - 96 : 0};
     for (int z = zlo, n = 0; z < zhi; z += n) {
         n = std::min(((c->pipe.active || c->pipe.slabwise) && z == zlo) ? std::min(S, PIPE_EDGE) : S, zhi - z);
@@ -315,14 +354,18 @@
             carry_planes(c, a, n, 0, 4);
             carry_planes(c, h1, n, 0, 2);
         }
+        if (zcopy && !zcopied && z + n - 40 >= 8) {
+            carry_planes(c, skip0, 0, D - 96, 8);
+            zcopied = true;
+        }
         const int i0 = std::max(0, 40 - z), i1 = std::min(n, Y - 40 - z);
         if (!pz && i1 > i0) crop_into(c, y0, pad ? 0 : 40, zview(skip0, z + i0 - 40, i1 - i0), i0);
         {
-            const int d0 = pz ? std::max(z, 44) : z, d1 = pz ? std::min(z + n, Y - 44) : z + n;
+            const int d0 = pz ? std::max(z, 44) : z, d1 = pz ? ((zcopy && z + n == zhi) ? Y - 44 : std::min(z + n, Y - 44)) : z + n;
             if (d1 > d0) {
-                const Tensor tv = zview(td, (d0 - (pz ? 44 : 0)) / 2, (d1 - d0) / 2);
+                const Tensor tv = zview(td, zc1 + (d0 - (pz ? 44 : 0)) / 2, (d1 - d0) / 2);
                 Tensor yv = zview(y0, d0 - z, d1 - d0);
-                ConvLaunch cl; cl.in = inner(yv); cl.Dv = tv.p.D; cl.Hv = tv.p.H; cl.Wv = tv.p.W; cl.out = tv.p; cl.flags = F_ACT;
+                ConvLaunch cl; cl.in = inner(yv); cl.Dv = tv.p.D; cl.Hv = tv.p.H - 2 * tv.pad; cl.Wv = tv.p.W - 2 * tv.pad; cl.out = inner(tv); cl.flags = F_ACT;
                 if (run_conv(c, *Ld, cl, true)) return 1;
                 const int og[3] = {yv.org[0] / 2, yv.org[1] / 2, yv.org[2] / 2};
                 const int zd[3] = {22, 22 + (D - 96) / 2, pz ? (D - 96) / 2 : 0};
@@ -333,38 +376,42 @@
     tfree(c, h0); tfree(c, a); tfree(c, h1);
     if (!pz) tfree(c, y0r);
     set_org(skip0, 0, pad ? 4 : 0, pad ? 4 : 0);
-    set_org(td, pz ? 22 : 0, pad ? 22 : 0, pad ? 22 : 0);
+    set_org(td, pz ? 22 - zc1 : 0, pad ? 22 : 0, pad ? 22 : 0);
     *skip0_out = skip0; *td_out = td;
     return 0;
 }
 
-static int stream_level1(nbe_ctx* c, int pad, bool pz, Tensor td, Tensor* cat1_out, Tensor* t_out) {
+static int stream_level1(nbe_ctx* c, int pad, bool pz, Tensor t, Tensor* cat1_out, Tensor* t_out) {
     const int m = c->mid;
-    Tensor t = td;
+    const int own = t.p.D - (pz ? 12 : 0);
     if (pad) {
-        t = tallocp(c, m, td.p.D + (pz ? 44 : 0), td.p.H, td.p.W, 1);
-        if (t.off < 0) return fail("workspace exhausted (level 1 input)");
-        if (!c->dry) launch_wrap_pad(td.p, t.p, 1, c->vel, c->stream, pz ? 22 : 0);
-        set_org(t, pz ? td.org[0] - 22 : td.org[0], td.org[1], td.org[2]);
-        tfree(c, td);
+        if (pz) wrap_planes_z(c, t, 6, own, 6);
+        fill_halo(c, t);
     }
 
     Tensor y1, cat1;
-    if (resblock(c, "conv_l1", t, true, true, m, m, &y1)) return 1;
+    const bool halos = !wrap_mode(c);
+    const int zr1[3] = {t.org[0], t.org[0] + own + 8, own};
+    if (resblock(c, "conv_l1", t, true, true, m, m, &y1, nullptr, halos, pz ? zr1 : nullptr)) return 1;
     tfree(c, t);
     if (pad) {
-        cat1 = tallocp(c, 2 * m, y1.p.D - 32, y1.p.H - 2, y1.p.W - 2, 1);
+        const int zc = pz ? 0 : 16;
+        cat1 = tallocp(c, 2 * m, y1.p.D - 2 * zc, y1.p.H - 2, y1.p.W - 2, 1);
         if (cat1.off < 0) return fail("workspace exhausted (cat1)");
-        crop_into(c, y1, 0, cat1, 16);
-        set_org(cat1, y1.org[0], y1.org[1] - 16, y1.org[2] - 16);
-        Tensor t2 = talloc(c, m, y1.p.D / 2, (y1.p.H - 2) / 2, (y1.p.W - 2) / 2);
+        cat1.halo = halos;
+        crop_into(c, y1, 0, cat1, zc);
+        set_org(cat1, y1.org[0] - 16 + zc, y1.org[1] - 16, y1.org[2] - 16);
+        const Tensor y1v = pz ? zview(y1, 4, own) : y1;
+        Tensor t2 = talloc(c, m, y1v.p.D / 2, (y1.p.H - 2) / 2, (y1.p.W - 2) / 2);
         const Layer* Ld1 = find_layer(c, "down_l1", "conv_0");
         if (t2.off < 0 || !Ld1) return fail("workspace exhausted or missing layer (down_l1)");
-        if (down_conv(c, *Ld1, y1, t2, true)) return 1;
-        t = talloc(c, m, t2.p.D, t2.p.H + 20, t2.p.W + 20);
+        const int zr2[3] = {y1v.org[0] / 2, y1v.org[0] / 2 + own / 2, own / 2};
+        if (down_conv(c, *Ld1, y1v, t2, true, pz ? zr2 : nullptr)) return 1;
+        const int pz2 = pz ? 10 : 0;
+        t = talloc(c, m, t2.p.D + 2 * pz2, t2.p.H + 20, t2.p.W + 20);
         if (t.off < 0) return fail("workspace exhausted (level 2 input)");
-        if (!c->dry) launch_wrap_pad(t2.p, t.p, 10, c->vel, c->stream, 0);
-        set_org(t, t2.org[0], t2.org[1] - 10, t2.org[2] - 10);
+        if (!c->dry) launch_wrap_pad(t2.p, t.p, 10, c->vel, c->stream, pz2);
+        set_org(t, t2.org[0] - pz2, t2.org[1] - 10, t2.org[2] - 10);
         tfree(c, t2);
     } else {
         cat1 = talloc(c, 2 * m, y1.p.D - 32, y1.p.H - 32, y1.p.W - 32);
@@ -399,7 +446,7 @@
     if (upblock(c, "up_r1", r, cat1, cat1.pad ? 2 : 0)) return 1;
     fill_halo(c, cat1);
     tfree(c, r);
-    if (resblock(c, "conv_r1", cat1, true, true, m, 2 * m, r_out)) return 1;
+    if (resblock(c, "conv_r1", cat1, true, true, m, 2 * m, r_out, nullptr, !(cat1.pad && wrap_mode(c)))) return 1;
     tfree(c, cat1);
     return 0;
 }
@@ -448,8 +495,10 @@
     const bool two = block_fused(c, Lr00, S + 4) && two_source_width(c);
     Tensor cat = tallocp(c, two ? m : 2 * m, S + 8, Hs, Ws, pad), hq = alloc_hidden(c, 2 * m, S + 6, cat, block_fused(c, Lr00, S + 4));
     Tensor q = tallocp(c, m, S + 4, Hs - 2 * sy, Ws - 2 * sy, pad), hy = alloc_hidden(c, m, S + 2, q, block_fused(c, Lr01, S));
-    Tensor y = tallocp(c, c->out_chan, S, Hs - 4 * sy, Ws - 4 * sy, pad);
+    Tensor y = tallocp(c, c->out_chan, S, Hs - 4 * sy, Ws - 4 * sy, pad, false);
     if (cat.off < 0 || hq.off < 0 || q.off < 0 || hy.off < 0 || y.off < 0) return fail("workspace exhausted (level-0 decoder slabs)");
+    cat.halo = q.halo = !wrap_mode(c);
+    y.halo = !wrap_env_on();
     for (int z = 0, n = 0; z < Yo; z += n) {
         n = std::min(S, Yo - z);
         if (c->pipe.active && c->pipe.out_async && Yo - z > PIPE_EDGE && Yo - z - n < PIPE_EDGE)
diff --git a/jax_nbody_emulator_with_dj_amd/csrc/nbe_kernels.h b/jax_nbody_emulator_with_dj_amd/csrc/nbe_kernels.h
--- a/jax_nbody_emulator_with_dj_amd/csrc/nbe_kernels.h
+++ b/jax_nbody_emulator_with_dj_amd/csrc/nbe_kernels.h
@@ -66,6 +66,7 @@
     int64_t sk_off = 0;
     const PackedW* skw = nullptr;
     bool wino = false;
+    bool pad1 = false, halo_missing = false, wrap = false;
 };
 
 int launch_conv(const PackedW& pw, const ConvLaunch& L, bool vel, bool has_dx, hipStream_t s);
diff --git a/jax_nbody_emulator_with_dj_amd/csrc/nbe_kernels.hip b/jax_nbody_emulator_with_dj_amd/csrc/nbe_kernels.hip
--- a/jax_nbody_emulator_with_dj_amd/csrc/nbe_kernels.hip
+++ b/jax_nbody_emulator_with_dj_amd/csrc/nbe_kernels.hip
@@ -146,6 +146,12 @@
         long o;
         if (MODE == MODE_DOWN) {
             o = q;
+            if (a.Ho != a.Hv || a.Wo != a.Wv) {
+                const int hw = a.Hv * a.Wv;
+                const int zo = (int)(q / hw), rem = (int)(q - (long)zo * hw);
+                const int yo = rem / a.Wv, xo = rem - yo * a.Wv;
+                o = ((long)zo * a.Ho + yo) * a.Wo + xo;
+            }
         } else {
             const int z = (int)(q / HW), rem = (int)(q - (long)z * HW);
             const int yy = rem / a.W, xx = rem - yy * a.W;
@@ -223,6 +229,7 @@
     ka.up8 = L.set < 0 ? 1 : 0; ka.set_stride = (long)pw.floats * 4;
     ka.stem_w = pw.stem;
     ka.ww = L.wino ? pw.ww : nullptr;
+    ka.wrap = L.wrap ? 1 : 0;
     ka.wws = (L.wino && L.skw) ? L.skw->ww : nullptr; ka.wws_set_floats = L.skw ? L.skw->floats : 0;
     ka.w = pw.w + (size_t)set * pw.floats;
     ka.dw = pw.dw ? pw.dw + (size_t)set * pw.floats : nullptr;
@@ -244,6 +251,7 @@
     }
     ka.ntiles = (int)((ka.Q + TILE_VOX - 1) / TILE_VOX);
     if (prec_is_half(pw.prec)) return launch_conv_h3(pw, ka, vel, has_dx, s);
+    if (ka.wrap) return 2;
     const int ct = pw.ctiles;
     if (ka.beta) {
         if (!(pw.mode == MODE_FLAT3 && vel && has_dx)) return 1;
diff --git a/jax_nbody_emulator_with_dj_amd/csrc/nbe_kernels_h3.hip b/jax_nbody_emulator_with_dj_amd/csrc/nbe_kernels_h3.hip
--- a/jax_nbody_emulator_with_dj_amd/csrc/nbe_kernels_h3.hip
+++ b/jax_nbody_emulator_with_dj_amd/csrc/nbe_kernels_h3.hip
@@ -288,6 +288,12 @@
         ok[jt] = q < a.Q;
         if (MODE == MODE_DOWN) {
             o[jt] = q;
+            if (a.Ho != a.Hv || a.Wo != a.Wv) {
+                const int hw = a.Hv * a.Wv;
+                const int zo = (int)(q / hw), rem = (int)(q - (long)zo * hw);
+                const int yo = rem / a.Wv, xo = rem - yo * a.Wv;
+                o[jt] = ((long)zo * a.Ho + yo) * a.Wo + xo;
+            }
         } else {
             const int z = (int)(q / HW), rem = (int)(q - (long)z * HW);
             const int yy = rem / a.W, xx = rem - yy * a.W;
@@ -1794,6 +1800,10 @@
 int launch_conv_h3(const PackedW& pw, const ConvKArgs& ka, bool vel, bool has_dx, hipStream_t s) {
     const int ct = pw.ctiles;
     const bool split = pw.prec == PREC_F16X3;
+    if (ka.wrap) {
+        const bool form = split && vel && has_dx && ka.beta && ka.ww && pw.mode == MODE_FLAT3 && pw.cout_t != 16 && ka.in_off == 0 && ka.osz == 1;
+        return form && launch_h3w(ka, ka.ww, ka.wws, ka.wws_set_floats, ct, s) == 0 ? 0 : 2;
+    }
     if (ka.stem_w && !(vel && has_dx) && pw.mode == MODE_FLAT3 && ka.in_off == 0 && ka.osz == 1 &&
         !(ka.flags & F_RES) && ka.nskip == 0 && !ka.beta) {
         if (split) return vel ? launch_stem<true>(ka, s) : launch_stem<false>(ka, s);
diff --git a/jax_nbody_emulator_with_dj_amd/csrc/nbe_kernels_internal.h b/jax_nbody_emulator_with_dj_amd/csrc/nbe_kernels_internal.h
--- a/jax_nbody_emulator_with_dj_amd/csrc/nbe_kernels_internal.h
+++ b/jax_nbody_emulator_with_dj_amd/csrc/nbe_kernels_internal.h
@@ -36,6 +36,7 @@
     int up8; long set_stride;
     const float* wws; long wws_set_floats;
     const float* ww;
+    int wrap;
     const float* stem_w;
     ConvGroupSrc gs[NBE_MAX_GROUPS];
 };
diff --git a/jax_nbody_emulator_with_dj_amd/csrc/nbe_kernels_wino.h b/jax_nbody_emulator_with_dj_amd/csrc/nbe_kernels_wino.h
--- a/jax_nbody_emulator_with_dj_amd/csrc/nbe_kernels_wino.h
+++ b/jax_nbody_emulator_with_dj_amd/csrc/nbe_kernels_wino.h
@@ -22,6 +22,7 @@
     int H, W, Dv, Hv, Wv, Ho, Wo;
     int nchunk, cout_groups, flags, ntiles, tny, tnx;
     int zblock;
+    int wrap;
     float* y; float* dy; long out_pstride; int out_g0;
     const float* bias; const float* gout; const float* beta;
     const float* r; const float* dr; long res_pstride;
@@ -68,12 +69,24 @@
     const int nst = 4 * a.nchunk;
 
     const long to = (((long)z0 * a.H + y0) * a.W + x0) * 16;
+    constexpr bool ABSOFF = !F16;
+    const long tz = (long)z0 * a.H * a.W * 16;
+    auto unit_off = [&](int row, int col) {
+        if (!ABSOFF) return (unsigned)(row * a.W + col) * 16u;
+        int Y = y0 + row, X = x0 + col;
+        if (a.wrap) {
+            Y = Y == 0 ? a.H - 2 : Y == a.H - 1 ? 1 : Y;
+            X = X == 0 ? a.W - 2 : X == a.W - 1 ? 1 : X;
+        }
+        return (unsigned)(Y * a.W + X) * 16u;
+    };
     const long wcm = (long)ct * nst * WGU * 16, wcs = (long)ct * a.nskip * TAPU * 16;
 
     struct Nxt { const char *xa, *xb, *w0; long dxd, psb; float sb; } nx;
-    auto set_next = [&](int s) {
+    auto set_next = [&](int s, bool raw) {
         const WinoSrc e = a.st[s];
-        nx.xa = e.xa + to; nx.xb = e.xb + to; nx.dxd = e.dxd; nx.psb = e.psb; nx.w0 = e.w + (SKIP && s >= nst ? wcs : wcm); nx.sb = e.sb;
+        const long tb = (raw || !ABSOFF) ? to : tz;
+        nx.xa = e.xa + tb; nx.xb = e.xb + tb; nx.dxd = e.dxd; nx.psb = e.psb; nx.w0 = e.w + (SKIP && s >= nst ? wcs : wcm); nx.sb = e.sb;
     };
     unsigned lane16 = (unsigned)lane << 4;
     asm volatile("" : "+v"(lane16));
@@ -108,7 +121,7 @@
             const int u = ((wave + NW * j) % 6) * 64 + lane;
             it_uu[j] = u < HP_PL ? u : HP_PL - 1;
             const int row = (it_uu[j] * 241) >> 13, col = it_uu[j] - row * HP_RS;
-            it_go[j] = (unsigned)(row * a.W + col) * 16u;
+            it_go[j] = unit_off(row, col);
         }
 #pragma unroll
         for (int j = 0; j < 3; ++j) asm volatile("" : "+v"(it_uu[j]), "+v"(it_go[j]));
@@ -129,7 +142,7 @@
         bool v;
         const int uu = item_unit(j, v);
         const int row = (uu * 241) >> 13, col = uu - row * HP_RS;
-        return (unsigned)(row * a.W + col) * 16u;
+        return unit_off(row, col);
     };
     typedef unsigned int u32x4 __attribute__((ext_vector_type(4)));
     struct Stg { half8 ah, al, bh, bl; float sb; };
@@ -329,7 +342,7 @@
         constexpr int NXT = decltype(nxt)::value;
         constexpr bool px = NXT == 1;
         const bool pre = px && s + 1 != 2 * a.nchunk;
-        if (NXT) set_next(s + 1);
+        if (NXT) set_next(s + 1, NXT == 2);
         int par = s & 1;
         asm volatile("" : "+s"(par));
         int nb = 1 - par;
@@ -394,7 +407,7 @@
     };
 
     auto raw_stage = [&](f32x4 (&Y)[NTILE], f32x4 (&DY)[NTILE], int s, bool px) {
-        if (px) set_next(s + 1);
+        if (px) set_next(s + 1, true);
         int par = s & 1;
         asm volatile("" : "+s"(par));
         int nb = 1 - par;
@@ -439,7 +452,7 @@
 
     {
         if (NBE_WINO_ZROW && !F16 && tid < 64) L8w[ZROW + tid] = half8{0, 0, 0, 0, 0, 0, 0, 0};
-        set_next(0);
+        set_next(0, false);
 #pragma unroll
         for (int k = 0; k < G::NWS; ++k) dma_w(0, k);
         {
@@ -660,7 +673,8 @@
     if (!ww || (!f16 && (ka.flags & F_RES)) || (ka.Dv & 1) || 4 * ka.nchunk > NBE_MAX_WSTAGES || (!novel && !ka.beta)) return 1;
     if (ka.nskip > 0 && (!wws || 2 * ka.nskip > NBE_MAX_WSKIP)) return 1;
     if (ctiles != (ka.cout_groups + 7) / 8) return 1;
-    if (std::max(ka.in_pstride, ka.csplit < ka.nchunk ? ka.in2_pstride : 0L) * 16 + 16L * (HP_ROWS + 2) * ka.W >= (1L << 32) - (1L << 20)) return 1;
+    if (std::max(ka.in_pstride, ka.csplit < ka.nchunk ? ka.in2_pstride : 0L) * 16 + 16L * ((f16 ? 0 : ka.H) + HP_ROWS + 2) * ka.W >= (1L << 32) - (1L << 20)) return 1;
+    if (ka.wrap && (novel || f16 || ka.Hv != ka.H - 2 || ka.Wv != ka.W - 2)) return 1;
     WinoKArgs wa;
     wa.H = ka.H; wa.W = ka.W; wa.Dv = ka.Dv; wa.Hv = ka.Hv; wa.Wv = ka.Wv; wa.Ho = ka.Ho; wa.Wo = ka.Wo;
     wa.nchunk = ka.nchunk; wa.cout_groups = ka.cout_groups; wa.flags = ka.flags;
@@ -674,6 +688,7 @@
     wa.inv_scale = 1.0f / (f16 ? WINO_WSCALE_F16 : WINO_WSCALE);
     wa.r = ka.r; wa.dr = ka.dr; wa.res_pstride = ka.res_pstride;
     wa.zblock = std::min(8, ka.Dv / 2);
+    wa.wrap = ka.wrap ? 1 : 0;
     wa.nskip = ka.nskip; wa.dws_delta = wws_set_floats * 4;
     static const int XI[2][2] = {{1, 2}, {0, 3}};
     static const int PA[4] = {0, 1, 2, 1}, PB[4] = {2, 2, 1, 3};
diff --git a/jax_nbody_emulator_with_dj_amd/engine.py b/jax_nbody_emulator_with_dj_amd/engine.py
--- a/jax_nbody_emulator_with_dj_amd/engine.py
+++ b/jax_nbody_emulator_with_dj_amd/engine.py
@@ -169,7 +169,7 @@
         check(self._l.nbe_synchronize(self._h))
 
     QUERY = {"gauge_active": 0, "slab": 1, "periodic_yx": 2, "periodic_z": 3, "range_shift": 4, "workspace_bytes": 5,
-             "host_pipe": 6, "graph_replays": 7, "plan_tiles": 8, "plan_short_gb": 9}
+             "host_pipe": 6, "graph_replays": 7, "plan_tiles": 8, "plan_short_gb": 9, "halo_fills": 10}
 
     def query(self, what):
         out = C.c_double()
@@ -343,7 +343,7 @@
         return y, dy
 
     PATHS = {"skip_fused": 1, "two_source": 2, "wino_0": 4, "wino_1": 8, "narrow": 16, "up8": 32, "skip_nodx": 64,
-             "two_source_skip": 128}
+             "two_source_skip": 128, "wrap_load": 256}
 
     def test_block(self, block, x, dx=None, x2=None, dx2=None, pad=0, two_source=False):
         x = _f32(x)
```

Result: no change. 99.40 million, median of 6 (+1.0%).
